# NicolaDM/MAPLE

Measured on AMD Instinct MI355X. Metric: candidate SPR placements/sec, higher is better.
Workload: dtype f64

## Files before the change

### __graft_entry__.py

```python
import os
import subprocess
import sys

ROOT = os.path.dirname(os.path.abspath(__file__))
if ROOT not in sys.path:
    sys.path.insert(0, ROOT)

CSRC = os.path.join(ROOT, "maple_amd", "csrc")
HIP_UNITS = ["maple_hip.hip", "append_queries.hip", "placement.hip", "update.hip", "spr_batch.hip", "frontier.hip", "frontier_upd.hip",
             "frontier_updw128.hip", "witness.hip", "em.hip"]
DEBUG_UNIT = "debug_abi.hip"
HIP_LIB = os.path.join(ROOT, "maple_amd", "libmaple_hip.so")
HIP_LIB_DEBUG = os.path.join(ROOT, "maple_amd", "libmaple_hip_debug.so")
HIP_FLAGS = ["--offload-arch=gfx950", "-O3", "-std=c++17", "-ffp-contract=off", "-fPIC"]
HIPCC = "hipcc" if subprocess.call(["which", "hipcc"], stdout=subprocess.DEVNULL) == 0 else "/opt/rocm/bin/hipcc"


def _stale(target, sources):
    if not os.path.exists(target):
        return True
    t = os.path.getmtime(target)
    return any(os.path.getmtime(s) > t for s in sources)


def compile_units(out_dir, extra_flags=(), only=None, force=True):
    sources = [os.path.join(CSRC, f) for f in os.listdir(CSRC) if not f.endswith((".o", ".c"))]
    sources.append(os.path.join(ROOT, "include", "maple_hip.h"))
    sources.append(os.path.join(ROOT, "include", "maple_hip_debug.h"))
    objs, jobs = [], []
    for unit in HIP_UNITS + [DEBUG_UNIT]:
        mine = only is None or unit in only
        obj = os.path.join(out_dir if mine else CSRC, unit[:-4] + ".o")
        objs.append(obj)
        deps = [x for x in sources if not (x.endswith(".hip") and os.path.basename(x) != unit)]
        if mine and (force or _stale(obj, deps)):
            jobs.append((unit, subprocess.Popen([HIPCC] + HIP_FLAGS + list(extra_flags) + ["-c", os.path.join(CSRC, unit), "-o", obj])))
    for unit, job in jobs:
        if job.wait() != 0:
            raise RuntimeError(f"hipcc failed on {unit}")
    return objs


def link(lib, objs):
    subprocess.check_call([HIPCC, "--offload-arch=gfx950", "-shared", "-fPIC"] + objs + ["-o", lib])


def build(force=False):
    extra = os.environ.get("MAPLE_HIP_EXTRA_FLAGS", "").split()
    objs = compile_units(CSRC, extra, force=force)
    for lib, parts in ((HIP_LIB, objs[:-1]), (HIP_LIB_DEBUG, objs)):
        if force or _stale(lib, parts):
            link(lib, parts)
    synth_src, synth_lib = os.path.join(CSRC, "synth_gen.c"), os.path.join(ROOT, "maple_amd", "libmaple_synth.so")
    if force or _stale(synth_lib, [synth_src]):
        subprocess.check_call(["gcc", "-O2", "-shared", "-fPIC", "-o", synth_lib, synth_src, "-lm"])
    subprocess.check_call(["make", "-C", os.path.join(ROOT, "oracle"), "-s"])
    import maple_amd
    from maple_amd import runtime
    runtime.load_library()


def smoke():
    import math
    import numpy as np
    from maple_amd.runtime import Device
    from maple_amd.synth import make_dataset
    from maple_amd.host import tip_genome_list, reference_tables
    from oracle.oracle_py import Oracle

    d = make_dataset(n_samples=64, l_ref=3000, seed=5, mean_diffs=12.0, frac_with_n=0.3, frac_ambig=0.3,
                     n_run_len=(5, 80))
    ref_idx, root_freqs = reference_tables(d.ref)
    lists = [tip_genome_list(x, ref_idx) for x in d.diffs]
    Q = [[-0.9, 0.2, 0.5, 0.2], [0.3, -1.4, 0.1, 1.0], [0.8, 0.1, -1.3, 0.4], [0.1, 0.6, 0.1, -0.8]]
    dev = Device(ref_idx, root_freqs, arena_bytes=64 << 20)
    orc = Oracle(ref_idx, root_freqs)
    dev.set_model(Q)
    orc.set_model(Q)
    ids = dev.upload(lists)
    n = len(lists)
    a = np.arange(n, dtype=np.int32)
    b = (a * 7 + 3) % n
    merged = dev.merge_batch(ids[a], 1e-4, True, ids[b], 2e-4, True, False)
    got_lists = dev.download(merged)
    ok_ids = [m for m in merged if m >= 0]
    scores = dev.append_batch(ok_ids, ids[: len(ok_ids)], True, 1.0 / dev.lRef)
    k = 0
    for i in range(n):
        want = orc.mergeVectors(lists[a[i]], 1e-4, True, lists[b[i]], 2e-4, True)
        if want is None:
            assert got_lists[i] is None
            continue
        assert len(want) == len(got_lists[i]) and all(x[0] == y[0] and x[1] == y[1] for x, y in zip(want, got_lists[i]))
        ws = orc.appendProbNode(want, lists[k], True, 1.0 / dev.lRef)
        gs = float(scores[k])
        assert (math.isinf(ws) and math.isinf(gs)) or abs(ws - gs) <= 1e-9 * max(1.0, abs(ws)), (ws, gs)
        k += 1
    import torch
    cu = torch.device("cuda", 0)
    t_q = torch.from_numpy(ids[:8].astype(np.int32)).to(cu)
    t_c = torch.from_numpy(np.asarray(ok_ids, dtype=np.int32)).to(cu)
    out = torch.empty(8 * len(ok_ids), dtype=torch.float64, device=cu)
    torch.cuda.synchronize()
    dev.append_queries_dev(8, t_q.data_ptr(), len(ok_ids), t_c.data_ptr(), True, 1.0 / dev.lRef, out.data_ptr(),
                           torch.cuda.current_stream().cuda_stream)
    torch.cuda.synchronize()
    got = out.cpu().numpy().reshape(8, len(ok_ids))
    ok_lists = [g for g in got_lists if g is not None]
    for qi in range(8):
        for ci in range(0, len(ok_ids), 5):
            ws = orc.appendProbNode(ok_lists[ci], lists[qi], True, 1.0 / dev.lRef)
            gs = float(got[qi, ci])
            assert (math.isinf(ws) and math.isinf(gs)) or abs(ws - gs) <= 1e-9 * max(1.0, abs(ws)), (qi, ci, ws, gs)
    dev.close()
    print(f"smoke ok: {n} merges, {k} + {8 * len(range(0, len(ok_ids), 5))} placements scored on the GPU and matched "
          "against the oracle")


if __name__ == "__main__":
    build()
    if len(sys.argv) > 1 and sys.argv[1] == "smoke":
        smoke()
```

### include/maple_hip_debug.h

```cpp
#ifndef MAPLE_HIP_DEBUG_H
#define MAPLE_HIP_DEBUG_H
#include "maple_hip.h"

#ifdef __cplusplus
extern "C" {
#endif

int maple_debug_frontier_levels(maple_ctx *ctx, int32_t cap, int64_t *itemsUpdating, int64_t *itemsCached, float *msUpdating,
                                float *msCached, int32_t *n, int64_t *waveItemsSmall , int64_t *waveItemsBig );

int maple_debug_wave_append_batch(maple_ctx *ctx, int32_t n, const int32_t *parentList, const int32_t *childList,
                                  const uint8_t *isTipC, const double *bLen, double *outLK, float *ms);
int maple_debug_trace_query(maple_ctx *ctx, int32_t query);
int maple_debug_calib_walk(maple_ctx *ctx, uint64_t bytes, int32_t repeats, float *ms);
int maple_debug_calib_write(maple_ctx *ctx, uint64_t bytes, int32_t mode, int32_t repeats, float *ms);
int maple_debug_trace_read(maple_ctx *ctx, int32_t *n, int32_t *items4 , double *vals2 );
int maple_debug_live_resources(int64_t *allocs, int64_t *bytes, int64_t *handles);
int maple_debug_gpv_batch(maple_ctx *ctx, int32_t n, const int32_t *i12, const double *totLen, const double *M16,
                          const double *errorRate, const double *vect4, const uint8_t *upNode, const uint8_t *flag,
                          double *out4);
int maple_debug_simplify_batch(maple_ctx *ctx, int32_t n, const double *vec4, const int32_t *refA, int32_t *out);
int maple_debug_frontier_pass_batch(maple_ctx *ctx, int32_t n, const int32_t *list, const int32_t *mutList, const uint8_t *dirIsUp,
                                    int32_t waveForm, int32_t *outList, uint8_t *grade, uint8_t *sameHandle);
int maple_debug_score_rows(maple_ctx *ctx, int32_t form, int32_t nQ, const int32_t *qList, const uint8_t *qTip, const double *qBLen,
                           int32_t nC, const int32_t *cand, const int32_t *outCol , int64_t ldOut, double fill, double *out,
                           uint64_t *finMask, int32_t *prefix, int64_t *pairsWalked );

#ifdef __cplusplus
}
#endif
#endif
```

### maple_amd/csrc/debug_abi.hip

```cpp
#include "../../include/maple_hip_debug.h"
#include "genome_dev.h"
#include "ctx_host.h"
#include "batch_host.h"
#include "frontier.h"
#include "frontier_dev.h"
#include "witness.h"

#include <algorithm>

using namespace frt;

__global__ __launch_bounds__(MAPLE_BLOCK) void k_calib_walk(const unsigned long long *buf, long long nLists, unsigned long long *sink)
{
    unsigned long long acc = 0;
    for (long long l = (long long)blockIdx.x * blockDim.x + threadIdx.x; l < nLists; l += (long long)gridDim.x * blockDim.x) {
        const unsigned long long *p = buf + l * 64;
        unsigned idx = 0;
        for (int k = 0; k < 64; k++) {
            unsigned long long w = p[idx];
            acc += w;
            idx = (idx + 1 + (unsigned)(w & 0)) & 63;
        }
    }
    if (acc == 0x123456789abcdefull) *sink = acc;
// ... 21 lines not shown
        hipLaunchKernelGGL(k_calib_write, dim3(4096), dim3(MAPLE_BLOCK), 0, c->stream, buf.p, (long long)(bytes / 8), mode == 1 ? 1 : 8);
    HIPCK(c, hipEventRecord(e1, c->stream));
    HIPCK(c, hipEventSynchronize(e1));
    if (ms) HIPCK(c, hipEventElapsedTime(ms, e0, e1));
    return MAPLE_OK;
}

extern "C" int maple_debug_calib_walk(maple_ctx *c, uint64_t bytes, int32_t repeats, float *ms)
{
    if (!c || bytes < 512 || repeats <= 0) return MAPLE_ERR_ARG;
    HIPCK(c, hipSetDevice(c->device));
    DevBuf<unsigned long long> buf, sink;
    HIPCK(c, buf.reserve_exact((size_t)((bytes + 7) / 8)));
    HIPCK(c, sink.reserve_exact(1));
    HIPCK(c, hipMemset(buf, 1, bytes));
    HIPCK(c, hipDeviceSynchronize());
    Event e0, e1;
    HIPCK(c, e0.create());
    HIPCK(c, e1.create());
    HIPCK(c, hipEventRecord(e0, c->stream));
    for (int r = 0; r < repeats; r++)
        hipLaunchKernelGGL(k_calib_walk, dim3(2048), dim3(MAPLE_BLOCK), 0, c->stream, buf.p, (long long)(bytes / 512), sink.p);
    HIPCK(c, hipEventRecord(e1, c->stream));
    HIPCK(c, hipEventSynchronize(e1));
    if (ms) HIPCK(c, hipEventElapsedTime(ms, e0, e1));
    return MAPLE_OK;
}

struct MatCtx {
    const double *M;
    __device__ inline double q(double, int i, int j) const { return M[i * 4 + j]; }
};
struct ThrCtx { struct { double thresholdProb, thresholdProb4; } m; };

__global__ __launch_bounds__(MAPLE_BLOCK) void k_debug_gpv(int n, int usingErrorRate, const int32_t *i12, const double *totLen,
                                                           const double *M16, const double *errorRate, const double *vect,
                                                           const uint8_t *upNode, const uint8_t *flag, double *out)
{
    for (int i = blockIdx.x * blockDim.x + threadIdx.x; i < n; i += gridDim.x * blockDim.x) {
        MatCtx c{M16 + 16 * (size_t)i};
        double o[4];
        if (i12[i] == 6) gpv_vec(c, 1.0, vect + 4 * (size_t)i, totLen[i], upNode[i] != 0, o);
        else if (usingErrorRate) gpv_nuc<MatCtx, true>(c, 1.0, i12[i], totLen[i], errorRate[i], upNode[i] != 0, flag[i] != 0, o);
        else gpv_nuc<MatCtx, false>(c, 1.0, i12[i], totLen[i], errorRate[i], upNode[i] != 0, false, o);
        for (int k = 0; k < 4; k++) out[4 * (size_t)i + k] = o[k];
    }
}

__global__ __launch_bounds__(MAPLE_BLOCK) void k_debug_simplify(int n, double thresholdProb, double thresholdProb4, const double *vec,
                                                                const int32_t *refA, int32_t *out)
{
    for (int i = blockIdx.x * blockDim.x + threadIdx.x; i < n; i += gridDim.x * blockDim.x) {
        ThrCtx c;
        c.m.thresholdProb = thresholdProb; c.m.thresholdProb4 = thresholdProb4;
        out[i] = simplify(c, vec + 4 * (size_t)i, refA[i]);
    }
}

extern "C" int maple_debug_gpv_batch(maple_ctx *c, int32_t n, const int32_t *i12, const double *totLen, const double *M16,
                                     const double *errorRate, const double *vect4, const uint8_t *upNode, const uint8_t *flag,
                                     double *out4)
{
    if (!c || n < 0 || !i12 || !totLen || !M16 || !errorRate || !vect4 || !upNode || !flag || !out4) return MAPLE_ERR_ARG;
    if (n == 0) return MAPLE_OK;
    HIPCK(c, hipSetDevice(c->device));
    TRY(need_model(c));
    TRY(h2d(c, c->s_i32[0], i12, (size_t)n));
    TRY(h2d(c, c->s_f64[0], totLen, (size_t)n));
    TRY(h2d(c, c->s_f64[1], M16, (size_t)16 * n));
    TRY(h2d(c, c->s_f64[2], errorRate, (size_t)n));
    TRY(h2d(c, c->s_f64[3], vect4, (size_t)4 * n));
    TRY(h2d(c, c->s_u8[0], upNode, (size_t)n));
    TRY(h2d(c, c->s_u8[1], flag, (size_t)n));
    HIPCK(c, c->s_aux.reserve((size_t)4 * n));
    hipLaunchKernelGGL(k_debug_gpv, dim3(grid_for(n)), dim3(MAPLE_BLOCK), 0, c->stream, n, c->dm.usingErrorRate, c->s_i32[0].p,
                       c->s_f64[0].p, c->s_f64[1].p, c->s_f64[2].p, c->s_f64[3].p, c->s_u8[0].p, c->s_u8[1].p, c->s_aux.p);
    HIPCK(c, hipGetLastError());
    HIPCK(c, hipMemcpyAsync(out4, c->s_aux.p, (size_t)4 * n * sizeof(double), hipMemcpyDeviceToHost, c->stream));
    HIPCK(c, hipStreamSynchronize(c->stream));
    return MAPLE_OK;
}

extern "C" int maple_debug_simplify_batch(maple_ctx *c, int32_t n, const double *vec4, const int32_t *refA, int32_t *out)
{
    if (!c || n < 0 || !vec4 || !refA || !out) return MAPLE_ERR_ARG;
    if (n == 0) return MAPLE_OK;
    HIPCK(c, hipSetDevice(c->device));
    TRY(h2d(c, c->s_f64[0], vec4, (size_t)4 * n));
    TRY(h2d(c, c->s_i32[0], refA, (size_t)n));
    HIPCK(c, c->s_i32[1].reserve(n));
    hipLaunchKernelGGL(k_debug_simplify, dim3(grid_for(n)), dim3(MAPLE_BLOCK), 0, c->stream, n, c->dm.thresholdProb,
                       c->dm.thresholdProb4, c->s_f64[0].p, c->s_i32[0].p, c->s_i32[1].p);
    HIPCK(c, hipGetLastError());
    HIPCK(c, hipMemcpyAsync(out, c->s_i32[1].p, n * sizeof(int32_t), hipMemcpyDeviceToHost, c->stream));
    HIPCK(c, hipStreamSynchronize(c->stream));
    return MAPLE_OK;
}

extern "C" int maple_debug_wave_append_batch(maple_ctx *c, int32_t n, const int32_t *pl, const int32_t *cl, const uint8_t *tip,
                                             const double *bl, double *out, float *ms)
{
    if (!c || n < 0 || !pl || !cl || !tip || !bl || !out) return MAPLE_ERR_ARG;
    if (n == 0) return MAPLE_OK;
    HIPCK(c, hipSetDevice(c->device));
    TRY(need_model(c));
    TRY(check_ids(c, n, pl, false, "parentList"));
    TRY(check_ids(c, n, cl, false, "childList"));
    TRY(stage_begin(c, (size_t)n * 32 + 256));
    STAGE(dpl, c, pl, n); STAGE(dcl, c, cl, n); STAGE(dtip, c, tip, n); STAGE(dbl, c, bl, n);
    TRY(stage_flush(c));
    HIPCK(c, c->s_f64[1].reserve(n));
    hipEvent_t e0, e1;
    TRY(ev_pair(c, &e0, &e1, MAPLE_K_OTHER, (double)n, 0.0));
    HIPCK(c, hipEventRecord(e0, c->stream));
    launch_wave_append(c, std::min(n, 256 * 16), n, dpl, dcl, dtip, dbl, c->s_f64[1].p);
    HIPCK(c, hipGetLastError());
    HIPCK(c, hipEventRecord(e1, c->stream));
    HIPCK(c, hipMemcpyAsync(out, c->s_f64[1].p, n * sizeof(double), hipMemcpyDeviceToHost, c->stream));
    HIPCK(c, hipStreamSynchronize(c->stream));
    if (ms) HIPCK(c, hipEventElapsedTime(ms, e0, e1));
    return MAPLE_OK;
}

extern "C" int maple_debug_live_resources(int64_t *allocs, int64_t *bytes, int64_t *handles)
{
    if (!allocs || !bytes || !handles) return MAPLE_ERR_ARG;
    const DevBufStats &s = devbuf_stats();
    *allocs = s.live_allocs; *bytes = s.live_bytes; *handles = s.live_handles;
    return MAPLE_OK;
}

extern "C" int maple_debug_trace_query(maple_ctx *c, int32_t query)
{
    if (!c) return MAPLE_ERR_ARG;
    c->trace_query = query;
    if (query >= 0) {
        HIPCK(c, c->s_trace_i.reserve(4 * 4096 + 4));
        HIPCK(c, c->s_trace_d.reserve(2 * 4096));
        HIPCK(c, hipMemset(c->s_trace_i.p, 0, (4 * 4096 + 4) * sizeof(int32_t)));
    }
    return MAPLE_OK;
}

extern "C" int maple_debug_trace_read(maple_ctx *c, int32_t *n, int32_t *items4, double *vals2)
{
    if (!c || !n || !items4 || !vals2 || !c->s_trace_i.p) return MAPLE_ERR_ARG;
    HIPCK(c, hipMemcpy(n, c->s_trace_i.p + 4 * 4096, sizeof(int32_t), hipMemcpyDeviceToHost));
    HIPCK(c, hipMemcpy(items4, c->s_trace_i.p, 4 * 4096 * sizeof(int32_t), hipMemcpyDeviceToHost));
    HIPCK(c, hipMemcpy(vals2, c->s_trace_d.p, 2 * 4096 * sizeof(double), hipMemcpyDeviceToHost));
    return MAPLE_OK;
}

extern "C" int maple_debug_frontier_levels(maple_ctx *c, int32_t cap, int64_t *itemsUpdating, int64_t *itemsCached, float *msUpdating,
                                           float *msCached, int32_t *n, int64_t *waveItemsSmall, int64_t *waveItemsBig)
{
    if (!c || cap < 0 || !itemsUpdating || !itemsCached || !msUpdating || !msCached || !n) return MAPLE_ERR_ARG;
    HIPCK(c, hipSetDevice(c->device));
    int nn = 0;
    const int rc = frontier_level_profile(c, cap, (long long *)itemsUpdating, (long long *)itemsCached, msUpdating, msCached, &nn,
                                          (long long *)waveItemsSmall, (long long *)waveItemsBig);
    *n = nn;
    return rc;
}

template <bool RV, bool U, bool SS>
__global__ __launch_bounds__(FR_BLOCK) void k_debug_fpass_lane(const DevModel *__restrict__ mp, ArenaViewS av, FPools fp, int n, const int32_t *l,
                                                               const int32_t *ml, const uint8_t *up, int32_t *handle)
{
    __shared__ Lds lds;
    const DevModel &m = *mp;
    stage_model(m, lds);
    Ctx<RV, U, SS> c(m, lds);
    const long long laneId = (long long)blockIdx.x * blockDim.x + threadIdx.x;
    for (long long i = laneId; i < n; i += (long long)gridDim.x * blockDim.x)
        handle[i] = fpass_removed(c, fp, av, laneId, ftree(l[i]), ml[i], up[i] != 0);
}

template <bool RV, bool U, bool SS>
__global__ __launch_bounds__(FR_BLOCK) void k_debug_fpass_wave(const DevModel *__restrict__ mp, ArenaViewS av, FPools fp, int n, const int32_t *l,
                                                               const int32_t *ml, const uint8_t *up, int32_t *handle)
{
    __shared__ Lds lds;
    const DevModel &m = *mp;
    stage_model(m, lds);
    Ctx<RV, U, SS> c(m, lds);
    const long long wave = ((long long)blockIdx.x * blockDim.x + threadIdx.x) >> 6, nWaves = ((long long)gridDim.x * blockDim.x) >> 6;
    const int lane = threadIdx.x & 63;
    for (long long i = wave; i < n; i += nWaves) {
        const int h = wave_pass(c, fp, av, ftree(l[i]), ml[i], up[i] != 0, true);
        if (lane == 0) handle[i] = h;
    }
}

__global__ __launch_bounds__(FR_BLOCK) void k_debug_fpass_out(FPools fp, int n, const int32_t *handle, int64_t *woff, int64_t *aoff, int32_t *nEnt,
                                                              int32_t *nAux, uint8_t *grade)
{
    for (int i = blockIdx.x * blockDim.x + threadIdx.x; i < n; i += gridDim.x * blockDim.x) {
        const int h = handle[i];
        if (h >= 0 && h < fp.capL) {
            const LRec r = fp.trec[h];
            woff[i] = LREC_OFF(r.x); aoff[i] = LREC_OFF(r.y); nEnt[i] = LREC_N(r.x); nAux[i] = LREC_N(r.y); grade[i] = fp.tflag[h];
        } else { woff[i] = 0; aoff[i] = 0; nEnt[i] = -1; nAux[i] = 0; grade[i] = 0; }
    }
}

extern "C" int maple_debug_frontier_pass_batch(maple_ctx *c, int32_t n, const int32_t *list, const int32_t *mutList, const uint8_t *dirIsUp,
                                               int32_t waveForm, int32_t *outList, uint8_t *grade, uint8_t *sameHandle)
{
    if (!c || n < 0 || n > (1 << 20) || !list || !mutList || !dirIsUp || !outList || !grade || !sameHandle) return MAPLE_ERR_ARG;
    if (n == 0) return MAPLE_OK;
    HIPCK(c, hipSetDevice(c->device));
    TRY(need_model(c));
    TRY(check_ids(c, n, list, false, "list"));
    TRY(settle(c));
    const int32_t nml = (int32_t)c->h_mut_cnt.size();
    long long capW = 0, capA = 0;
    int capE = 1;
    for (int i = 0; i < n; i++) {
        if (mutList[i] < -1 || mutList[i] >= nml) return fail(c, MAPLE_ERR_ARG, "mutList[%d] = %d is not a mutation-list id", i, mutList[i]);
        const long long cnt = mutList[i] < 0 ? 0 : c->h_mut_cnt[mutList[i]];
        const long long ne = c->h_n_ent[list[i]] + 2 * cnt, na = c->h_n_aux[list[i]] + 4 * cnt;
        capW += ne; capA += na;
        capE = std::max(capE, (int)ne);
    }
    const int threads = waveForm ? 64 * std::min(n, 1024) : std::min(1024, (n + FR_BLOCK - 1) / FR_BLOCK * FR_BLOCK);
    const int grid = (threads + FR_BLOCK - 1) / FR_BLOCK;
    const long long lanes = (long long)grid * FR_BLOCK;
    HIPCK(c, c->s_words.reserve((size_t)capW));
    HIPCK(c, c->s_aux.reserve((size_t)capA));
    auto up16 = [](size_t x) { return (x + 255) & ~(size_t)255; };
    const size_t oRec = 0, oCtr = up16(oRec + (size_t)n * sizeof(LRec)), oSw = up16(oCtr + sizeof(FCtr)),
                 oSa = up16(oSw + (waveForm ? 0 : (size_t)lanes * capE * sizeof(uint2))),
                 oWoff = up16(oSa + (waveForm ? 0 : (size_t)lanes * 5 * capE * sizeof(double))), oAoff = up16(oWoff + (size_t)n * 8),
                 oHandle = up16(oAoff + (size_t)n * 8), oNe = up16(oHandle + (size_t)n * 4), oNa = up16(oNe + (size_t)n * 4),
                 oFlag = up16(oNa + (size_t)n * 4), oGrade = up16(oFlag + (size_t)n), total = up16(oGrade + (size_t)n);
    DevBuf<uint8_t> own;
    HIPCK(c, own.reserve_exact(total));
    uint8_t *const buf = own.p;
    int rc = MAPLE_OK;
    std::vector<int32_t> handle(n);
    do {
        if (hipMemsetAsync(buf, 0, oSw, c->stream) != hipSuccess) { rc = fail(c, MAPLE_ERR_HIP, "hipMemsetAsync"); break; }
        FPools fp;
        memset(&fp, 0, sizeof fp);
        fp.tw = c->s_words.p; fp.ta = c->s_aux.p;
        fp.trec = (LRec *)(buf + oRec); fp.tflag = buf + oFlag;
        fp.capW = capW; fp.capA = capA; fp.capL = n;
        fp.sw = (uint2 *)(buf + oSw); fp.sa = (double *)(buf + oSa); fp.capE = capE;
        fp.ctr = (FCtr *)(buf + oCtr);
        fp.mat = 1;
        fp.mv = MutViewS{c->d_mut3, c->d_mut_off, c->d_mut_cnt};
        const ArenaViewS av{c->d_words, c->d_aux, c->d_ent_off, c->d_aux_off, c->d_n_ent, c->d_n_aux};
        if ((rc = stage_begin(c, (size_t)n * 64 + 256)) != MAPLE_OK) break;
        auto *dl = stage_put(c, list, (size_t)n);
        auto *dml = stage_put(c, mutList, (size_t)n);
        auto *dup = stage_put(c, dirIsUp, (size_t)n);
        if (!dl || !dml || !dup) { rc = fail(c, MAPLE_ERR_NOMEM, "argument staging overflow"); break; }
        if ((rc = stage_flush(c)) != MAPLE_OK) break;
        int32_t *dHandle = (int32_t *)(buf + oHandle), *dNe = (int32_t *)(buf + oNe), *dNa = (int32_t *)(buf + oNa);
        int64_t *dWoff = (int64_t *)(buf + oWoff), *dAoff = (int64_t *)(buf + oAoff);
        if (waveForm) DISPATCH3(c, k_debug_fpass_wave, <<<grid, FR_BLOCK, 0, c->stream>>>(c->d_model, av, fp, n, dl, dml, dup, dHandle));
        else DISPATCH3(c, k_debug_fpass_lane, <<<grid, FR_BLOCK, 0, c->stream>>>(c->d_model, av, fp, n, dl, dml, dup, dHandle));
        hipLaunchKernelGGL(k_debug_fpass_out, dim3(grid_for(n)), dim3(FR_BLOCK), 0, c->stream, fp, n, dHandle, dWoff, dAoff, dNe, dNa, buf + oGrade);
        if (hipGetLastError() != hipSuccess || hipMemcpyAsync(handle.data(), dHandle, (size_t)n * 4, hipMemcpyDeviceToHost, c->stream) != hipSuccess
            || hipMemcpyAsync(grade, buf + oGrade, (size_t)n, hipMemcpyDeviceToHost, c->stream) != hipSuccess
            || hipStreamSynchronize(c->stream) != hipSuccess) { rc = fail(c, MAPLE_ERR_HIP, "the frontier pass hook's launch failed"); break; }
        for (int i = 0; i < n && rc == MAPLE_OK; i++) {
            sameHandle[i] = handle[i] == -(list[i] + 10);
            if (!sameHandle[i] && handle[i] < 0) rc = fail(c, MAPLE_ERR_NOMEM, "item %d: no room for the new list (%d)", i, handle[i]);
        }
        if (rc != MAPLE_OK) break;
        if ((rc = commit_lists(c, n, dWoff, dAoff, dNe, dNa, outList, fp.tw, fp.ta)) != MAPLE_OK) break;
        if (hipStreamSynchronize(c->stream) != hipSuccess) { rc = fail(c, MAPLE_ERR_HIP, "hipStreamSynchronize"); break; }
        for (int i = 0; i < n; i++) if (sameHandle[i]) outList[i] = list[i];
    } while (0);
    return rc;
}

__global__ __launch_bounds__(MAPLE_BLOCK) void k_debug_fill(long long n, double v, double *out)
{
    for (long long i = (long long)blockIdx.x * blockDim.x + threadIdx.x; i < n; i += (long long)gridDim.x * blockDim.x) out[i] = v;
}

extern "C" int maple_debug_score_rows(maple_ctx *c, int32_t form, int32_t nQ, const int32_t *qList, const uint8_t *qTip, const double *qBLen,
                                      int32_t nC, const int32_t *cand, const int32_t *outCol, int64_t ldOut, double fill, double *out,
                                      uint64_t *finMask, int32_t *prefix, int64_t *pairsWalked)
{
    if (!c || form < 0 || form > 1 || nQ <= 0 || nC <= 0 || !qList || !qTip || !qBLen || !cand || ldOut < nC || !out || !finMask || !prefix)
        return MAPLE_ERR_ARG;
    if ((long long)nQ * ldOut > (1ll << 28)) return fail(c, MAPLE_ERR_ARG, "maple_debug_score_rows: a table of %lld scores", (long long)nQ * ldOut);
    HIPCK(c, hipSetDevice(c->device));
    TRY(need_model(c));
    TRY(check_ids(c, nQ, qList, false, "qList"));
    TRY(check_ids(c, nC, cand, true, "cand"));
    for (int k = 0; k < nC; k++) {
        if (cand[k] < -1) return fail(c, MAPLE_ERR_ARG, "cand[%d] = %d", k, cand[k]);
        if (outCol && (outCol[k] < 0 || outCol[k] >= ldOut)) return fail(c, MAPLE_ERR_ARG, "outCol[%d] = %d is outside a row of %lld", k, outCol[k], (long long)ldOut);
    }
    TRY(settle(c));
    const int nWords = (nC + 63) / 64;
    const size_t nOut = (size_t)nQ * (size_t)ldOut, nMask = (size_t)nQ * nWords, nPre = (size_t)nQ * (nWords + 1);
    DevBuf<double> dOut;
    DevBuf<unsigned long long> dMask;
    DevBuf<int32_t> dPre;
    HIPCK(c, dOut.reserve_exact(nOut));
    HIPCK(c, dMask.reserve_exact(nMask));
    HIPCK(c, dPre.reserve_exact(nPre));
    TRY(stage_begin(c, (size_t)nQ * 16 + (size_t)nC * 8 + 256));
    STAGE(dq, c, qList, nQ); STAGE(dtip, c, qTip, nQ); STAGE(dbl, c, qBLen, nQ); STAGE(dcand, c, cand, nC);
    const int32_t *dcol = nullptr;
    if (outCol) { STAGE(dc, c, outCol, nC); dcol = dc; }
    TRY(stage_flush(c));
    hipLaunchKernelGGL(k_debug_fill, dim3(grid_for((int)nOut)), dim3(MAPLE_BLOCK), 0, c->stream, (long long)nOut, fill, dOut.p);
    HIPCK(c, hipGetLastError());
    HIPCK(c, hipMemsetAsync(dMask.p, 0xA5, nMask * sizeof(unsigned long long), c->stream));
// ... 16 lines not shown
```

### maple_amd/csrc/fr_wave_items_body.inc

```
    __shared__ Lds lds;
    __shared__ WaveUpdLds<Class::wuIn> L;
    typedef WaveLds<Class::capW> WaveLdsC;
    const DevModel &m = *mp;
    stage_model(m, lds);
    Ctx<RV, U, SS> c(m, lds);
    const int lane = threadIdx.x;
    WaveLdsC &W = *reinterpret_cast<WaveLdsC *>(L.baux);
    static_assert(sizeof(WaveLdsC) <= sizeof(L.baux), "LDS alias");
    const long long lo = (long long)fp.ctr->loU;
    const long long nHeavy = (long long)(fp.ctr->*Class::count);
    (void)heavyMin;
    unsigned long long nU = 0, bU = 0;
    for (long long kk = blockIdx.x; kk < nHeavy; kk += gridDim.x) {
        nU++;
#ifdef MAPLE_SPR_PROFILE
        const long long tItem0 = wall_clock64();
        int profCls = Class::profCls;
        struct ProfEnd {
            const FPools &fp; const long long t0; int &cls;
            __device__ ~ProfEnd() {
                if ((threadIdx.x & 63) == 0) {
                    const unsigned long long dt = (unsigned long long)(wall_clock64() - t0);
                    atomicAdd(&fp.ctr->dbgWCnt[cls], 1ull); atomicAdd(&fp.ctr->dbgWT[cls], dt); atomicMax(&fp.ctr->dbgWMax[cls], dt);
                }
            }
        } profEnd{fp, tItem0, profCls};
#endif
        {
            const long long i = lo + (fp.*Class::perm)[kk];
            FItem &it = fp.U[i];
            FSearch &S = fp.S[it.q];
            if (!fs_live(S.state)) { if (lane == 0) it.flags |= FI_DEAD; continue; }
            const int q = it.q, t1 = it.t1, dir = it.dir;
            const NodeRec r1 = T.nd[t1];
            const int hPassed = it.hPassed, hRpr = it.hRpr;
            const double distance = it.distance, lastLK = it.lastLK;
            const bool rt = S.isRemovedTip != 0;
            const double rbl = S.removedBLen;
            const int other = dir == 0 ? -1 : (dir == 1 ? r1.c1 : r1.c0);
            const int upT = r1.up;
            const FList lp = fvalid(hPassed) ? flist(av, fp, hPassed) : FList{nullptr, nullptr, 0, 0};
            const FList lr = flist(av, fp, hRpr);
            const bool fits = fr_wave_fits(av, T, fp, it, Class::wuIn, Class::capW);
            if (!fits) {
#ifdef MAPLE_SPR_PROFILE
                profCls += 2;
#endif
                if (lane == 0) fr_upd_item_lane_call(c, av, T, P, fp, budget, laneBase + blockIdx.x, i, &bU);
                wave_sync();
                continue;
            }
            bool upd = true;
            double midProb = lastLK;
            int flagsAdd = 0;
            int nM = 0, naM = 0;
            auto merge = [&](const FList &l1, double b1, bool tp1, const FList &l2, double b2, bool tp2, bool upDown) -> int {
                if (l1.n > L.wuIn || l2.n > L.wuIn) return -2;
                wave_sync();
                const int r = wave_merge(c, fref(l1), l1.n, b1, tp1, fref(l2), l2.n, b2, tp2, upDown, L, naM);
                bU += 8ull * (unsigned long long)(l1.n + l1.na + l2.n + l2.na + (r > 0 ? r + naM : 0));
                if (r < 0) return r == -1 ? -1 : -2;
                nM = r;
                return 0;
            };
            auto differs = [&](int listId) -> bool {
                const FList tu = flist(av, fp, ftree(listId));
                const unsigned long long *tw = (const unsigned long long *)tu.w;
                for (int k = lane; k < tu.n; k += 64) L.old[k] = tw[k];
                wave_sync();
                return wave_differ(c, L.m, L.maux, nM, L.old, tu.aux, tu.n);
            };
            auto score = [&]() -> double {
                wave_sync();
                return wave_append(c, ListRef{(const uint2 *)L.m, L.maux}, nM, fref(lr), lr.n, rt, rbl, W);
            };
            auto push1 = [&](bool u, int node, int d, int h, double dst, double mp, int fails, double pb, int hr, bool needPass) -> int {
                int ref = FR_NONE;
                if (lane == 0) ref = fpush(fp, budget, q, u, node, d, h, dst, mp, fails, hr, pb, needPass);
                return __shfl(ref, 0, 64);
            };
            const bool matAdj = fp.mat && (r1.c0Frame != r1.frameOf || r1.c1Frame != r1.frameOf || r1.upFrame != r1.frameOf);
            auto passW = [&](int h, int mutId, bool up, bool removed) -> int {
                if (!matAdj) return h;
                return wave_pass(c, fp, av, h, mutId, up, removed);
            };
            bool dead = false, fallback = false;
            int child0 = FR_NONE, child1 = FR_NONE, hA = -1, hB = -1, hMid = -1;
            double recDist = 0.0;
            if (dir == 0) {
                const bool scored = !(upT == S.parent || upT < 0) && (r1.dist > P.effNon0 || r1.upIsRoot);
                if (scored) {
                    const FList ll = flist(av, fp, ftree(r1.lower));
                    if (merge(lp, distance / 2, false, ll, distance / 2, r1.isTip != 0, true) != 0) dead = true;
                    else {
                        if (r1.totUp >= 0 && !differs(r1.totUp)) upd = false;
                        midProb = score();
                        flagsAdd |= FI_SCORED;
                        if (upd && midProb >= it.pathBest - P.thrOptTopo) {
                            wave_sync();
                            hMid = fstore_wave(fp, L.m, L.maux, nM, naM);
                            if (hMid < 0) { fallback = true; dead = true; }
                            else { hA = hPassed; hB = ftree(r1.lower); recDist = distance; flagsAdd |= FI_REC_UPD; }
                        }
                    }
                }
                if (!dead) {
                    const PRule pr = p_rule(P, scored, midProb, lastLK, it.failsP, it.pathBest);
                    if (pr.go && r1.c0 >= 0) {
                        for (int k = 0; k < 2 && !fallback; k++) {
                            const int ch = k == 0 ? r1.c0 : r1.c1, oth = k == 0 ? r1.c1 : r1.c0;
                            int ref = FR_NONE;
                            const bool cross = matAdj && (k == 0 ? r1.c0Frame : r1.c1Frame) != r1.frameOf;
                            if (upd) {
                                const NodeRec ro = T.nd[oth];
                                const int hOther = passW(ftree(ro.lower), ro.mutId, true, false);
                                const FList lo2 = fvalid(hOther) ? flist(av, fp, hOther) : FList{nullptr, nullptr, 0, 0};
                                const int r = fvalid(hOther) ? merge(lp, distance, false, lo2, ro.dist, ro.isTip != 0, true) : -2;
                                if (r == -2) { fallback = true; break; }
                                if (r == 0) {
                                    wave_sync();
                                    int hv = fstore_wave(fp, L.m, L.maux, nM, naM), hr = hRpr;
                                    if (hv >= 0 && cross) {
                                        const int mId = T.nd[ch].mutId;
                                        hv = passW(hv, mId, false, false); hr = passW(hRpr, mId, false, true);
                                    }
                                    if (hv < 0 || !fvalid(hr)) { fallback = true; break; }
                                    ref = push1(true, ch, 0, hv, T.nd[ch].dist, midProb, pr.fails, pr.pathBest, hr, false);
                                }
                            } else if ((k == 0 ? r1.upRight : r1.upLeft) >= 0)
                                ref = push1(false, ch, 0, -1, 0.0, midProb, pr.fails, pr.pathBest, hRpr, cross);
                            if (k == 0) child0 = ref; else child1 = ref;
                        }
                    }
                }
            } else {
                const NodeRec ro = T.nd[other];
                const int vectUp = upT >= 0 ? passW(ftree(r1.whichChild ? T.nd[upT].upLeft : T.nd[upT].upRight), r1.mutId, false, false) : -1;
                const int hOther = passW(ftree(ro.lower), ro.mutId, true, false);
                const bool crossO = matAdj && ((dir == 1) ? r1.c1Frame : r1.c0Frame) != r1.frameOf, crossU = matAdj && r1.upFrame != r1.frameOf;
                const bool scored = upT >= 0 && (r1.dist > P.effNon0 || r1.upIsRoot);
                int hBottom = -1;
                if (vectUp == -2 || hOther == -2 || !fvalid(hOther)) {
                    if (lane == 0) { S.state = FS_FALLBACK; it.flags |= FI_DEAD; }
                    wave_sync();
                    continue;
                }
                const FList lo2 = flist(av, fp, hOther);
                const FList lvu = fvalid(vectUp) ? flist(av, fp, vectUp) : FList{nullptr, nullptr, 0, 0};
                if (scored) {
                    if (!fvalid(vectUp) || r1.totUp < 0) {
                        if (lane == 0) fr_upd_item_lane_call(c, av, T, P, fp, budget, laneBase + blockIdx.x, i, &bU);
                        wave_sync();
                        continue;
                    }
                    int r = merge(lp, distance, false, lo2, ro.dist, ro.isTip != 0, false);
                    if (r == -2) { fallback = true; dead = true; }
                    else if (r != 0) dead = true;
                    else {
                        wave_sync();
                        hBottom = fstore_wave(fp, L.m, L.maux, nM, naM);
                        if (hBottom < 0) { fallback = true; dead = true; }
                        else {
                            const FList lb = flist(av, fp, hBottom);
                            r = merge(lvu, r1.dist / 2, false, lb, r1.dist / 2, false, true);
                            if (r == -2) { fallback = true; dead = true; }
                            else if (r != 0) dead = true;
                            else {
                                if (!differs(r1.totUp)) upd = false;
                                midProb = score();
                                flagsAdd |= FI_SCORED;
                                if (upd && midProb >= it.pathBest - P.thrOptTopo) {
                                    wave_sync();
                                    hMid = fstore_wave(fp, L.m, L.maux, nM, naM);
                                    if (hMid < 0) { fallback = true; dead = true; }
                                    else { hA = vectUp; hB = hBottom; recDist = r1.dist; flagsAdd |= FI_REC_UPD; }
                                }
                            }
                        }
                    }
                }
                if (!dead) {
                    const PRule pr = p_rule(P, scored, midProb, lastLK, it.failsP, it.pathBest);
                    if (pr.go) {
                        if (upT >= 0) {
                            int hUp = -1;
                            bool stop = false;
                            if (upd) {
                                const int r = fvalid(vectUp) ? merge(lvu, r1.dist, false, lp, distance, false, true) : -2;
                                if (r == -2) { fallback = true; stop = true; }
                                else if (r == 0) { wave_sync(); hUp = fstore_wave(fp, L.m, L.maux, nM, naM); if (hUp < 0) { fallback = true; stop = true; } }
                            } else hUp = ftree(dir == 1 ? r1.upLeft : r1.upRight);
                            int hrO = hRpr, hrU = hRpr;
                            if (upd && crossO && !stop && hUp >= 0) {
                                hUp = passW(hUp, ro.mutId, false, false); hrO = passW(hRpr, ro.mutId, false, true);
                                if (hUp == -2 || !fvalid(hrO)) { fallback = true; stop = true; }
                            }
                            if (!stop && fvalid(hUp)) {
                                child0 = upd ? push1(true, other, 0, hUp, ro.dist, midProb, pr.fails, pr.pathBest, hrO, false)
                                             : push1(false, other, 0, -1, 0.0, midProb, pr.fails, pr.pathBest, hRpr, crossO);
// ... 32 lines not shown
```

### maple_amd/csrc/frontier.h

```cpp
#pragma once
#include "ctx_host.h"

#define FR_STATUS_FALLBACK (-8)

struct FrontierStats {
    int levels = 0, overflow = 0;
    long long itemsUpdating = 0, itemsCached = 0, tempLists = 0, tempWords = 0, tempAux = 0, records = 0;
};

struct FrontierWide {
    const int32_t *rowOf;
    const double *cacheS;
    FiniteRows fin;
    hipEvent_t rowsReady;
    int forceWide;
    const int32_t *frameParent = nullptr, *frameNode = nullptr;
    int nFrames = 0;
};

__attribute__((visibility("hidden")))
int frontier_search(maple_ctx *c, const SearchParams &P, int m, const int32_t *nodes, int budget, int zeroBudget, SearchOut *hostOut,
                    uint2 *poolW, double *poolA, unsigned long long *poolUsed, long long poolCapW, long long poolCapA,
                    FrontierStats *stats, long long itemsHint, const FrontierWide *wide = nullptr,
                    const uint8_t *overHint = nullptr);
__attribute__((visibility("hidden"))) int frontier_export(maple_ctx *c, long long cap, int32_t *q, int32_t *node, long long *n);
__attribute__((visibility("hidden")))
int frontier_level_profile(maple_ctx *c, int cap, long long *itemsU, long long *itemsC, float *msU, float *msC, int *n,
                           long long *waveSmall = nullptr, long long *waveBig = nullptr);
```

### maple_amd/csrc/frontier.hip

```cpp
#include "ctx_host.h"
#include "frontier_dev.h"
#include "search_plan.h"

#include <chrono>

using namespace frt;
namespace plan = maple::plan;

namespace {

__global__ __launch_bounds__(FR_BLOCK) void k_fr_arena_recs(ArenaViewS av, int n, LRec *out)
{
    for (int i = blockIdx.x * blockDim.x + threadIdx.x; i < n; i += gridDim.x * blockDim.x)
        out[i] = lrec_make(av.ent_off[i], av.n_ent[i], av.aux_off[i], av.n_aux[i]);
}

template <bool RV, bool U, bool SS>
__global__ __launch_bounds__(FR_BLOCK) void k_fr_begin(const DevModel *__restrict__ mp, ArenaViewS av, DevTree T, SearchParams P, int n,
                                                       const int32_t *nodes, FPools fp, SearchOut *out, int budget, int zeroBudget,
                                                       const int32_t *rowOf, int forceWide, const uint8_t *overHint)
{
    __shared__ Lds lds;
    const DevModel &m = *mp;
    stage_model(m, lds);
    Ctx<RV, U, SS> c(m, lds);
    for (int q = blockIdx.x * blockDim.x + threadIdx.x; q < n; q += gridDim.x * blockDim.x) {
        const int node = nodes[q];
        SearchOut &o = out[q];
        o.bestNode = -1; o.placement = -1; o.status = 0; o.nAppend = 0;
        o.bestScore = 0.0; o.improvement = 0.0; o.currentLK = 0.0;
        o.blen[0] = o.blen[1] = o.blen[2] = 0.0;
        o.rprWoff = o.rprAoff = -1; o.rprN = o.rprNA = 0;
        o.nShortList = o.nSteps = 0; o.tStep = o.tReplay = o.tRefine = 0;
        FSearch &S = fp.S[q];
        S.node = node; S.parent = -1; S.sibling = -1; S.hRpr0 = -1; S.seed0 = S.seed1 = FR_NONE; S.nItems = 0; S.state = FS_FINAL;
        S.slHead = FR_NONE; S.nApp = 0; S.recBase = 0; S.recCount = 0; S.isRemovedTip = 0; S.removedBLen = 0.0; S.curLK = 0.0;
        const NodeRec rn = T.nd[node];
        const int parent = rn.up;
        if (parent < 0) { o.status = 1; continue; }
        const NodeRec rp = T.nd[parent];
        const int childIdx = (rp.c0 == node) ? 0 : 1;
        const int vectUp = ftree(childIdx == 0 ? rp.upRight : rp.upLeft);
        if (!fvalid(vectUp) || rn.lower < 0) { o.status = -1; continue; }
        const FList lu = flist(av, fp, vectUp), ll = flist(av, fp, ftree(rn.lower));
        const long long laneId = (long long)blockIdx.x * blockDim.x + threadIdx.x;
        double curLK;
        if (fp.mat && rn.mutId >= 0 && fp.mv.cnt[rn.mutId] > 0) {
            const int cnt = fp.mv.cnt[rn.mutId];
            FScr scr{nullptr, nullptr};
            if (!fscratch(fp, laneId, lu.n + 2 * cnt, scr)) { S.state = FS_FALLBACK; continue; }
            Writer wr;
            wr.init(scr.w, scr.a);
            pass_walk(c.m.lRef, fref(lu), fp.mv.mut3 + 3 * fp.mv.off[rn.mutId], cnt, false, wr);
            curLK = append_walk(c, ListRef{scr.w, scr.a}, fref(ll), rn.isTip != 0, rn.dist);
        } else
        curLK = append_walk(c, fref(lu), fref(ll), rn.isTip != 0, rn.dist);
        o.currentLK = curLK;
        if (!(curLK < P.thrPlacement || rn.dist != 0.0)) { o.status = 2; continue; }
        if (overHint && overHint[q]) { S.state = FS_OVER; o.status = -5; continue; }
        S.parent = parent; S.sibling = childIdx == 0 ? rp.c1 : rp.c0;
        S.isRemovedTip = rn.isTip; S.removedBLen = rn.dist; S.curLK = curLK;
        const NodeRec rs = T.nd[S.sibling];
        int rpr = ftree(rn.lower);
        const int mergeLevel = shorten_would_merge(c, fref(ll), ll.n);
        const bool wouldMerge = mergeLevel != 0;
        S.rprMerge0 = mergeLevel;
        int hBest = rpr;
        if (fp.mat) {
            rpr = fpass_removed(c, fp, av, laneId, rpr, rn.mutId, true);
            hBest = fvalid(rpr) ? fpass_removed(c, fp, av, laneId, rpr, rs.mutId, false) : rpr;
            if (!fvalid(rpr) || !fvalid(hBest)) { S.state = FS_FALLBACK; continue; }
        }
        S.hRpr0 = hBest;
        bool wide = false;
        if (forceWide && rowOf && rowOf[q] >= 0) {
            if (wouldMerge) { S.state = FS_OVER; o.status = -5; o.nAppend = -1; continue; }
            wide = true;
        } else if (!U && budget > zeroBudget && rn.dist == 0.0) {
            wide = rowOf && rowOf[q] >= 0 && !wouldMerge;
            if (!wide) { S.state = FS_OVER; o.status = -5; o.nAppend = -1; continue; }
        } else if (U && rowOf && rowOf[q] >= 0) {
            if (wouldMerge) { S.state = FS_OVER; o.status = -5; o.nAppend = -1; continue; }
            wide = true;
        }
        S.state = wide ? FS_WIDE : FS_ACTIVE;
        if (rp.up < 0) {
            S.seed0 = fpush(fp, budget, q, true, S.sibling, 3, -1, 0.0, curLK, 0, S.hRpr0, curLK);
            continue;
        }
        const int pp = rp.up;
        const NodeRec rpp = T.nd[pp];
        const bool first = rpp.c0 == parent;
        const double d = rs.dist + rp.dist;
        int pv1 = ftree(rs.lower), rprUp = rpr, vUpUp = ftree(first ? rpp.upRight : rpp.upLeft), rprDown = rpr;
        if (fp.mat) {
            pv1 = fpass_store(fp, av, c.m.lRef, laneId, pv1, rs.mutId, true);
            if (rp.mutId >= 0) {
                pv1 = fvalid(pv1) ? fpass_store(fp, av, c.m.lRef, laneId, pv1, rp.mutId, true) : pv1;
                rprUp = fpass_removed(c, fp, av, laneId, rpr, rp.mutId, true);
            }
            vUpUp = fpass_store(fp, av, c.m.lRef, laneId, vUpUp, rp.mutId, false);
            if (rs.mutId >= 0) {
                vUpUp = fvalid(vUpUp) ? fpass_store(fp, av, c.m.lRef, laneId, vUpUp, rs.mutId, false) : vUpUp;
                rprDown = hBest;
            }
            if (pv1 == -2 || vUpUp == -2 || !fvalid(rprUp) || !fvalid(rprDown)) { S.state = FS_FALLBACK; continue; }
        }
        S.seed0 = fpush(fp, budget, q, true, pp, first ? 1 : 2, pv1, d, curLK, 0, rprUp, curLK);
        S.seed1 = fpush(fp, budget, q, true, S.sibling, 0, vUpUp, d, curLK, 0, rprDown, curLK);
    }
}

#define FR_LVL 8
__global__ void k_fr_snap_u(FCtr *ctr, long long capU, long long capR, long long capPassR, unsigned long long *lvl, int maxLevels)
{
    if (threadIdx.x == 0 && blockIdx.x == 0) {
        ctr->loU = ctr->hiU; ctr->hiU = min(ctr->usedU, (unsigned long long)capU);
        atomicExch(&ctr->safePassR, min(ctr->nPassR, (unsigned long long)capPassR));
        __threadfence();
        atomicExch(&ctr->safeR, min(ctr->usedR, (unsigned long long)capR));
        ctr->bigUsed = 0;
        const unsigned long long heavySmall = ctr->permHeavy, heavyBig = ctr->permHeavy2;
        ctr->permDown = ctr->permUp = ctr->permDownB = ctr->permUpB = ctr->permHeavy = ctr->permHeavy2 = 0;
        if (lvl) {
            const int l = ctr->nLevels++;
            if (l < maxLevels) { lvl[FR_LVL * l] = ctr->loU; lvl[FR_LVL * l + 1] = ctr->hiU; lvl[FR_LVL * l + 6] = lvl[FR_LVL * l + 7] = 0; }
            if (l > 0 && l - 1 < maxLevels) { lvl[FR_LVL * (l - 1) + 6] = heavySmall; lvl[FR_LVL * (l - 1) + 7] = heavyBig; }
        }
    }
}
__global__ void k_fr_snap_c(FCtr *ctr, long long capCC, long long capPass, long long capDeferred, unsigned long long *lvl, int maxLevels)
{
    if (threadIdx.x == 0 && blockIdx.x == 0) {
        ctr->loC = ctr->hiC; ctr->hiC = min(ctr->usedC, (unsigned long long)capCC);
        ctr->loR = ctr->hiR; ctr->hiR = atomicAdd(&ctr->safeR, 0ull);
        __threadfence();
        ctr->loP = ctr->hiP; ctr->hiP = min(ctr->nPass, (unsigned long long)capPass);
        ctr->loPR = ctr->hiPR; ctr->hiPR = atomicAdd(&ctr->safePassR, 0ull);
        ctr->bigUsedC = 0;
        ctr->loD = ctr->hiD; ctr->hiD = min(ctr->nDeferred, (unsigned long long)capDeferred);
        if (lvl) {
            const int k = ctr->nLevelsC++;
            if (k < maxLevels) {
                lvl[FR_LVL * k + 2] = ctr->loC; lvl[FR_LVL * k + 3] = ctr->hiC;
                lvl[FR_LVL * k + 4] = (unsigned long long)capCC + ctr->loR; lvl[FR_LVL * k + 5] = (unsigned long long)capCC + ctr->hiR;
            }
        }
    }
}

#define FR_PASS_WAVE_BELOW 8192
template <bool RV, bool U, bool SS>
__global__ __launch_bounds__(FR_BLOCK) void k_fr_pass_wave(const DevModel *__restrict__ mp, ArenaViewS av, DevTree T, FPools fp)
{
    __shared__ Lds lds;
    const DevModel &m = *mp;
    stage_model(m, lds);
    Ctx<RV, U, SS> c(m, lds);
    const long long wave = ((long long)blockIdx.x * blockDim.x + threadIdx.x) >> 6, nWaves = ((long long)gridDim.x * blockDim.x) >> 6;
    const int lane = threadIdx.x & 63;
    const long long loA = (long long)fp.ctr->loP, nA = (long long)fp.ctr->hiP - loA, loB = (long long)fp.ctr->loPR, nB = (long long)fp.ctr->hiPR - loB;
    if (nA + nB > FR_PASS_WAVE_BELOW) return;
    for (long long i = wave; i < nA + nB; i += nWaves) {
        FItem &it = item_of(fp, i < nA ? fp.passList[loA + i] : fp.passListR[loB + (i - nA)]);
        FSearch &S = fp.S[it.q];
        if (!fs_live(S.state)) continue;
        const NodeRec r1 = T.nd[it.t1];
        const int mutId = it.dir == 0 ? r1.mutId : T.nd[it.dir == 1 ? r1.c0 : r1.c1].mutId;
        const int h = wave_pass(c, fp, av, it.hRpr, mutId, it.dir != 0, true);
        if (lane == 0) {
            if (!fvalid(h)) S.state = FS_FALLBACK;
            else {
                it.hRpr = h;
                const unsigned long long k = atomicAdd(&fp.ctr->nDeferred, 1ull);
                if ((long long)k < fp.capDeferred) fp.deferred[k] = (int32_t)(&it - fp.C);
                else { S.state = FS_FALLBACK; fp.ctr->overflow = 1; }
            }
        }
    }
}

template <bool RV, bool U, bool SS>
__global__ __launch_bounds__(FR_BLOCK) void k_fr_pass(const DevModel *__restrict__ mp, ArenaViewS av, DevTree T, FPools fp, long long slabBase)
{
    __shared__ Lds lds;
    const DevModel &m = *mp;
    stage_model(m, lds);
    Ctx<RV, U, SS> c(m, lds);
    const long long laneId = (long long)blockIdx.x * blockDim.x + threadIdx.x;
    const long long slab = slabBase + laneId;
    const long long loA = (long long)fp.ctr->loP, nA = (long long)fp.ctr->hiP - loA, loB = (long long)fp.ctr->loPR, nB = (long long)fp.ctr->hiPR - loB;
    if (nA + nB <= FR_PASS_WAVE_BELOW) return;
    for (long long i = laneId; i < nA + nB; i += (long long)gridDim.x * blockDim.x) {
        FItem &it = item_of(fp, i < nA ? fp.passList[loA + i] : fp.passListR[loB + (i - nA)]);
        FSearch &S = fp.S[it.q];
        if (!fs_live(S.state)) continue;
        const NodeRec r1 = T.nd[it.t1];
        const int mutId = it.dir == 0 ? r1.mutId : T.nd[it.dir == 1 ? r1.c0 : r1.c1].mutId;
        const int h = fpass_removed(c, fp, av, slab, it.hRpr, mutId, it.dir != 0);
        if (!fvalid(h)) { S.state = FS_FALLBACK; continue; }
        it.hRpr = h;
        const unsigned long long k = atomicAdd(&fp.ctr->nDeferred, 1ull);
        if ((long long)k < fp.capDeferred) fp.deferred[k] = (int32_t)(&it - fp.C);
        else { S.state = FS_FALLBACK; fp.ctr->overflow = 1; }
    }
}

__global__ __launch_bounds__(FR_BLOCK) void k_fr_sort_level(ArenaViewS av, DevTree T, FPools fp, int heavyMin, int bigMin)
{
    const long long lo = (long long)fp.ctr->loU, hi = (long long)fp.ctr->hiU;
    const long long n = hi - lo;
    const int lane = threadIdx.x & 63;
    heavyMin = fr_level_heavy_min(fp, heavyMin);
    auto bc = [](unsigned long long x) {
        return ((unsigned long long)(uint32_t)__shfl((int)(x >> 32), 0, 64) << 32) | (uint32_t)__shfl((int)x, 0, 64);
    };
    for (long long base = (long long)blockIdx.x * blockDim.x; base < n; base += (long long)gridDim.x * blockDim.x) {
        const long long i = base + threadIdx.x;
        int kind = -1;
        bool small = false;
        if (i < n) {
            const FItem &it = fp.U[lo + i];
            const int sz = fr_upd_size(av, T, fp, it);
            if (!(heavyMin > 0 && it.dir != 3 && sz >= heavyMin)) kind = (it.dir == 0 ? 0 : 1) + (sz >= bigMin ? 2 : 0);
            else {
                small = fr_wave_fits(av, T, fp, it, WaveSmall::wuIn, WaveSmall::capW);
                if (!small && !fr_wave_fits(av, T, fp, it, WaveBig::wuIn, WaveBig::capW)) kind = (it.dir == 0 ? 2 : 3);
            }
        }
        const unsigned long long below = (1ull << lane) - 1ull;
        {
            const bool hv = i < n && kind == -1;
            for (int cls = 0; cls < 2; cls++) {
                const bool mine = hv && (small == (cls == 0));
                const unsigned long long mh = __ballot(mine);
                if (!mh) continue;
                unsigned long long b0 = 0;
                if (lane == 0) b0 = atomicAdd(cls == 0 ? &fp.ctr->permHeavy : &fp.ctr->permHeavy2, (unsigned long long)__popcll(mh));
                b0 = bc(b0);
                if (mine) (cls == 0 ? fp.perm3 : fp.perm4)[(long long)(b0 + __popcll(mh & below))] = (int32_t)i;
            }
        }
        for (int k = 0; k < 4; k++) {
            const unsigned long long mk = __ballot(kind == k);
            if (!mk) continue;
            unsigned long long *ctr = k == 0 ? &fp.ctr->permDown : (k == 1 ? &fp.ctr->permUp : (k == 2 ? &fp.ctr->permDownB : &fp.ctr->permUpB));
            unsigned long long b0 = 0;
            if (lane == 0) b0 = atomicAdd(ctr, (unsigned long long)__popcll(mk));
            b0 = bc(b0);
            if (kind == k) {
                int32_t *pm = k < 2 ? fp.perm : fp.perm2;
                const long long at = (long long)(b0 + __popcll(mk & below));
                pm[(k & 1) ? n - 1 - at : at] = (int32_t)i;
            }
        }
    }
}

#ifndef FR_CACHED_WAVES
#define FR_CACHED_WAVES 4
#endif
template <bool RV, bool U, bool SS>
__global__ __launch_bounds__(FR_BLOCK) __attribute__((amdgpu_waves_per_eu(FR_CACHED_WAVES, FR_CACHED_WAVES)))
void k_fr_cached(const DevModel *__restrict__ mp, ArenaViewS av, DevTree T, SearchParams P, FPools fp, int budget,
                 const int32_t *rowOf, FiniteRows fin)
{
    __shared__ Lds lds;
    const DevModel &m = *mp;
    stage_model(m, lds);
    Ctx<RV, U, SS> c(m, lds);
    const int lane = threadIdx.x & 63;
    const long long loC = (long long)fp.ctr->loC, nC = (long long)fp.ctr->hiC - loC, loR = fp.capCC + (long long)fp.ctr->loR,
                    nCR = nC + (long long)fp.ctr->hiR - (long long)fp.ctr->loR, loD = (long long)fp.ctr->loD,
                    hi = nCR + (long long)fp.ctr->hiD - loD;
    unsigned long long nSc = 0, bSc = 0;
    for (long long i0 = (long long)blockIdx.x * blockDim.x; i0 < hi; i0 += (long long)gridDim.x * blockDim.x) {
        const long long i = i0 + threadIdx.x;
#ifdef MAPLE_SPR_PROFILE
        const long long tp0 = wall_clock64();
#endif
        int mode = 0;
        FItem *itp = nullptr;
        const FSearch *Sp = nullptr;
        NodeRec r1{};
        FList lp{nullptr, nullptr, 0, 0}, lr{nullptr, nullptr, 0, 0};
        bool rt = false;
        double rbl = 0.0;
        if (i < hi) {
            FItem &it = fp.C[i < nC ? loC + i : (i < nCR ? loR + (i - nC) : (long long)fp.deferred[loD + (i - nCR)])];
            FSearch &S = fp.S[it.q];
            itp = &it; Sp = &S;
            const int st = S.state;
            if (i < nCR && (it.flags & FI_NEEDPASS)) { }
            else if (!fs_live(st)) it.flags |= FI_DEAD;
            else if (st == FS_WIDE && it.dir == 0) {
                int fl = FI_SEED;
                if (fin.mask && rowOf) {
                    const NodeRec r1s = T.nd[it.t1];
                    const SScan rec = T.scan[r1s.preRank];
                    const size_t row = (size_t)rowOf[it.q];
                    const unsigned long long *fm = fin.mask + row * fin.nWords;
                    const int32_t *fpx = fin.prefix + row * (fin.nWords + 1);
                    const int clo = T.candBefore[r1s.preRank], chi = T.candBefore[r1s.preRank + rec.size];
                    if (fin_count_before(fm, fpx, chi) == fin_count_before(fm, fpx, clo)) {
                        const bool firstScored = !(r1s.up == S.parent || r1s.up < 0) && (r1s.dist > P.effNon0 || r1s.upIsRoot);
                        const bool dropped = firstScored && !(rec.ff & SS_TOTUP);
                        fl |= FI_SEED_EMPTY;
                        it.hA = (firstScored && !dropped) ? 1 : 0;
                        it.hB = T.cladeVisits[r1s.preRank];
                        it.hMid = ((rec.ff & SS_INNER) && !dropped) ? 1 : 0;
                    }
                }
                it.flags |= (uint8_t)fl;
            } else {
                r1 = T.nd[it.t1];
                const int upT = r1.up;
                const bool scored = (it.dir == 0) ? (!(upT == S.parent || upT < 0) && (r1.dist > P.effNon0 || r1.upIsRoot))
                                                  : (upT >= 0 && (r1.dist > P.effNon0 || r1.upIsRoot));
                mode = 1;
                if (scored) {
                    if (r1.totUp < 0) { it.flags |= FI_DEAD; mode = 0; }
                    else {
                        lp = flist(av, fp, ftree(r1.totUp)); lr = flist(av, fp, it.hRpr);
                        rt = S.isRemovedTip != 0; rbl = S.removedBLen;
                        mode = 2;
                    }
                }
            }
        }
#ifdef MAPLE_SPR_PROFILE
        __builtin_amdgcn_s_waitcnt(0);
        const long long tp1 = wall_clock64();
#endif
        double scoreV = 0.0;
        if (mode == 2) scoreV = append_walk(c, fref(lp), fref(lr), rt, rbl);
        const int nS = __popcll(__ballot(mode == 2));
        (void)nS;
#ifdef MAPLE_SPR_PROFILE
        const long long tp2 = wall_clock64();
#endif
        if (mode != 0) {
            FItem &it = *itp;
            const FSearch &S = *Sp;
            const int q = it.q, hRpr = it.hRpr, upT = r1.up;
            const double lastLK = it.lastLK;
            double midProb = lastLK;
            const bool scored = mode == 2;
            if (scored) {
                midProb = scoreV;
                it.flags |= FI_SCORED;
                nSc++; bSc += 8ull * (unsigned long long)(lp.n + lp.na) + 8ull;
            }
            it.midProb = midProb;
            const PRule pr = p_rule(P, scored, midProb, lastLK, it.failsP, it.pathBest);
            if (pr.go) {
                const bool x0 = fp.mat && r1.c0Frame != r1.frameOf, x1 = fp.mat && r1.c1Frame != r1.frameOf, xu = fp.mat && r1.upFrame != r1.frameOf;
                if (it.dir == 0) {
                    if (r1.c0 >= 0) {
                        if (r1.upRight >= 0) it.child0 = fpush(fp, budget, q, false, r1.c0, 0, -1, 0.0, midProb, pr.fails, hRpr, pr.pathBest, x0, true);
                        if (r1.upLeft >= 0) it.child1 = fpush(fp, budget, q, false, r1.c1, 0, -1, 0.0, midProb, pr.fails, hRpr, pr.pathBest, x1, true);
                    }
                } else {
                    const int other = (it.dir == 1) ? r1.c1 : r1.c0;
                    const bool xo = (it.dir == 1) ? x1 : x0;
                    if (upT >= 0) {
                        if (((it.dir == 1) ? r1.upLeft : r1.upRight) >= 0) {
                            it.child0 = fpush(fp, budget, q, false, other, 0, -1, 0.0, midProb, pr.fails, hRpr, pr.pathBest, xo, true);
                            it.child1 = fpush(fp, budget, q, false, upT, (int)r1.whichChild + 1, -1, 0.0, midProb, pr.fails, hRpr, pr.pathBest, xu, true);
                        }
                    } else
                        it.child0 = fpush(fp, budget, q, false, other, 0, -1, 0.0, midProb, pr.fails, hRpr, pr.pathBest, xo, true);
                }
            }
            (void)S;
        }
#ifdef MAPLE_SPR_PROFILE
        {
            __builtin_amdgcn_s_waitcnt(0);
            const long long tp3 = wall_clock64();
            int len = mode == 2 ? lp.n + lr.n : 0, tot = len;
            for (int off = 32; off > 0; off >>= 1) { len = max(len, __shfl_down(len, off, 64)); tot += __shfl_down(tot, off, 64); }
            if (lane == 0) {
                atomicAdd(&fp.ctr->dbgC[0], 1ull); atomicAdd(&fp.ctr->dbgC[1], (unsigned long long)(tp1 - tp0));
                atomicAdd(&fp.ctr->dbgC[2], (unsigned long long)(tp2 - tp1)); atomicAdd(&fp.ctr->dbgC[3], (unsigned long long)(tp3 - tp2));
                atomicAdd(&fp.ctr->dbgC[4], (unsigned long long)len); atomicAdd(&fp.ctr->dbgC[5], (unsigned long long)nS);
                atomicAdd(&fp.ctr->dbgC[6], (unsigned long long)tot);
            }
        }
#endif
    }
    for (int off = 32; off > 0; off >>= 1) {
        nSc += ((unsigned long long)(uint32_t)__shfl_down((int)(nSc >> 32), off, 64) << 32) | (uint32_t)__shfl_down((int)nSc, off, 64);
        bSc += ((unsigned long long)(uint32_t)__shfl_down((int)(bSc >> 32), off, 64) << 32) | (uint32_t)__shfl_down((int)bSc, off, 64);
// ... 416 lines not shown
    }
}

template <bool RV, bool U, bool SS>
__global__ __launch_bounds__(FR_BLOCK) __attribute__((amdgpu_waves_per_eu(4, 4)))
void k_fr_refine(const DevModel *__restrict__ mp, ArenaViewS av, DevTree T, FPools fp)
{
    __shared__ Lds lds;
    const DevModel &m = *mp;
    stage_model(m, lds);
    Ctx<RV, U, SS> c(m, lds);
    const long long laneId = (long long)blockIdx.x * blockDim.x + threadIdx.x;
    double *ais = fp.sais + laneId * 2ll * fp.capE;
    const long long nRecs = min((long long)fp.ctr->nRecs, fp.capRecs);
    for (long long i = laneId; i < nRecs; i += (long long)gridDim.x * blockDim.x) {
        FRec &R = fp.recs[i];
        const FItem &it = item_of(fp, R.ref);
        FSearch &S = fp.S[R.q];
        R.ok = 0;
        if (!fs_live(S.state)) continue;
        const int t1 = it.t1;
        const NodeRec r1 = T.nd[t1];
        int hUp, hDown, hMid;
        double distance;
        if (it.flags & FI_REC_UPD) { hUp = it.hA; hDown = it.hB; hMid = it.hMid; distance = it.recDist; }
        else {
            hUp = r1.up >= 0 ? ftree(r1.whichChild ? T.nd[r1.up].upLeft : T.nd[r1.up].upRight) : -1;
            if (fp.mat && fvalid(hUp)) {
                hUp = fpass_store(fp, av, c.m.lRef, laneId, hUp, r1.mutId, false);
                if (hUp == -2) { S.state = FS_FALLBACK; continue; }
            }
            hDown = ftree(r1.lower); hMid = ftree(r1.totUp); distance = r1.dist;
        }
        if (!fvalid(hUp) || !fvalid(hDown) || !fvalid(hMid)) { R.ok = -1; continue; }
        int hRem = it.hRpr;
        if (R.hRprS == FR_SHORTEN) {
            const FList l0 = flist(av, fp, hRem);
            FScr scrS;
            if (!fscratch(fp, laneId, l0.n, scrS)) { S.state = FS_FALLBACK; continue; }
            Writer ws;
            ws.init(scrS.w, scrS.a);
            shorten_walk(c, fref(l0), l0.n, ws);
            hRem = fstore(fp, ws);
            if (hRem < 0) { S.state = FS_FALLBACK; continue; }
            R.hRprS = hRem;
        }
        const FList lUp = flist(av, fp, hUp), lDown = flist(av, fp, hDown), lMid = flist(av, fp, hMid), lRem = flist(av, fp, hRem);
        const bool ft = r1.isTip != 0, rt = S.isRemovedTip != 0;
        const int need = max(lDown.n + lRem.n, max(lUp.n + lRem.n, lUp.n + lDown.n));
        FScr scr0;
        if (lMid.n + lRem.n > 2 * fp.capE || lUp.n + need > 2 * fp.capE || !fscratch(fp, laneId, need, scr0)) { S.state = FS_FALLBACK; continue; }
        uint2 *sw = scr0.w;
        double *sa = scr0.a;
        bool f;
        Writer w;
        const double app = blen_walk(c, fref(lMid), fref(lRem), rt, ais, 1, &f);
        w.init(sw, sa);
        int r = merge_walk(c, fref(lDown), distance / 2, ft, fref(lRem), app, rt, false, false, 0, 0, w, nullptr);
        if (r < 0) { R.ok = -1; continue; }
        const ListRef scr{sw, sa};
        double top = blen_walk(c, fref(lUp), scr, false, ais, 1, &f);
        w.init(sw, sa);
        r = merge_walk(c, fref(lUp), top, false, fref(lRem), app, rt, true, false, 0, 0, w, nullptr);
        if (r == -1) {
            top = m.defaultBLen * 0.1;
            w.init(sw, sa);
            r = merge_walk(c, fref(lUp), top, false, fref(lRem), app, rt, true, false, 0, 0, w, nullptr);
        }
        if (r < 0) { R.ok = -1; continue; }
        const double bottom = blen_walk(c, scr, fref(lDown), ft, ais, 1, &f);
        w.init(sw, sa);
        r = merge_walk(c, fref(lUp), top, false, fref(lDown), bottom, ft, true, false, 0, 0, w, nullptr);
        if (r < 0) { R.ok = -1; continue; }
        const double cost = append_walk(c, scr, fref(lRem), rt, app);
        const double initialCost = append_walk(c, fref(lUp), fref(lDown), ft, distance);
        const double newPartialCost = append_walk(c, fref(lUp), fref(lDown), ft, bottom + top);
        R.optimized = cost + newPartialCost - initialCost;
        R.top = top; R.bottom = bottom; R.app = app;
        R.ok = 1;
    }
}

__global__ __launch_bounds__(FR_BLOCK) void k_fr_finish(ArenaViewS av, DevTree T, SearchParams P, int n, FPools fp, SearchOut *out,
                                                        uint2 *poolW, double *poolA, unsigned long long *poolUsed, long long poolCapW,
                                                        long long poolCapA)
{
    for (int q = blockIdx.x * blockDim.x + threadIdx.x; q < n; q += gridDim.x * blockDim.x) {
        FSearch &S = fp.S[q];
        SearchOut &o = out[q];
        if (S.state == FS_FALLBACK) { o.status = FR_STATUS_FALLBACK; continue; }
        if (!fs_live(S.state)) continue;
        const int node = S.node;
        const NodeRec rp = T.nd[S.parent];
        double bestScore = S.curLK;
        int bestNode = S.sibling, hBestRpr = S.hRpr0, nApp = S.nApp;
        double bl0 = rp.up >= 0 ? rp.dist : 0.0, bl1 = T.nd[S.sibling].dist, bl2 = S.removedBLen;
        bool failed = false;
        for (int k = 0; k < S.recCount; k++) {
            const FRec &R = fp.recs[S.recBase + k];
            if (R.ok != 1) { failed = true; break; }
            nApp += 3;
            if (R.optimized >= bestScore) {
                const FItem &it = item_of(fp, R.ref);
                bestNode = it.t1; bestScore = R.optimized; bl0 = R.top; bl1 = R.bottom; bl2 = R.app; hBestRpr = R.hRprS >= 0 ? R.hRprS : it.hRpr;
            }
        }
        o.nAppend = nApp;
        o.nShortList = S.recCount;
        if (failed) { o.status = -1; continue; }
        o.bestNode = bestNode; o.bestScore = bestScore;
        o.blen[0] = bl0; o.blen[1] = bl1; o.blen[2] = bl2;
        if (poolW) {
            const FList rp2 = flist(av, fp, hBestRpr);
            const long long ow = (long long)atomicAdd(&poolUsed[0], (unsigned long long)rp2.n);
            const long long oa = (long long)atomicAdd(&poolUsed[1], (unsigned long long)rp2.na);
            if (ow + rp2.n <= poolCapW && oa + rp2.na <= poolCapA) {
                for (int k = 0; k < rp2.n; k++) poolW[ow + k] = rp2.w[k];
                for (int k = 0; k < rp2.na; k++) poolA[oa + k] = rp2.aux[k];
                o.rprWoff = ow; o.rprAoff = oa; o.rprN = rp2.n; o.rprNA = rp2.na;
            } else o.status = -4;
        }
        const double curLK = S.curLK;
        if (bestScore + P.thrPlacement > curLK) {
            bool updated = true;
            int topNode = T.nd[node].up;
            if (bestNode == topNode) updated = false;
            while (T.nd[topNode].dist == 0.0 && T.nd[topNode].up >= 0) topNode = T.nd[topNode].up;
            if (bestNode == topNode && bl1 == 0.0) updated = false;
            if (bestNode == S.sibling) updated = false;
            if (T.nd[bestNode].up == S.sibling && bl0 == 0.0) updated = false;
            if (updated) { o.improvement = bestScore - curLK; o.placement = bestNode; }
        }
    }
}

__global__ __launch_bounds__(FR_BLOCK) void k_fr_export(FPools fp, long long nU, long long nC, long long nR, int32_t *outQ, int32_t *outNode)
{
    const long long n = nU + nC + nR;
    for (long long i = (long long)blockIdx.x * blockDim.x + threadIdx.x; i < n; i += (long long)gridDim.x * blockDim.x) {
        const FItem &it = i < nU ? fp.U[i] : (i < nU + nC ? fp.C[i - nU] : fp.C[fp.capCC + (i - nU - nC)]);
        outQ[i] = it.q; outNode[i] = it.t1;
    }
}

struct FrontierScratch : ScratchBase {
    Stream side, side2;
    Event evFork, evJoin, evFork2, evJoin2;
    DevBuf<uint8_t> itemsU, itemsC, srch, recs, ctr;
    DevBuf<uint2> tw, sw, bw;
    DevBuf<double> ta, sa, sais, ba;
    DevBuf<LRec> trec, arec;
    DevBuf<int32_t> nodes, expQ, expNode;
    DevBuf<uint8_t> out, wideBr, tflag, overHint;
    DevBuf<int32_t> wideRow, wideQ, wideCtr, perm, perm2, perm3, perm4, tot, lsize, lpos, lpar, passList, passListR, deferred;
    DevBuf<uint2> bw2; DevBuf<double> ba2;
    DevBuf<uint8_t> visit;
    DevBuf<unsigned long long> lvl;
    DevBuf<long long> vbase;
    std::vector<unsigned long long> lastLvl;
    std::vector<size_t> lastSlotsU, lastSlotsC;
    long long lastU = -1, lastC = -1, lastR = 0;
    plan::FrontierNeeds need;
    FPools lastPools{};
    int capE = 0;
    plan::FrontierCaps caps() const
    {
        plan::FrontierCaps k;
        k.itemsU = itemsU.cap; k.itemsC = itemsC.cap; k.tw = tw.cap; k.ta = ta.cap; k.trec = trec.cap; k.tflag = tflag.cap; k.arec = arec.cap;
        k.sw = sw.cap; k.sa = sa.cap; k.sais = sais.cap; k.bw = bw.cap; k.bw2 = bw2.cap; k.recs = recs.cap;
        k.perm = perm.cap; k.perm2 = perm2.cap; k.perm3 = perm3.cap; k.perm4 = perm4.cap; k.visit = visit.cap; k.lsize = lsize.cap;
        k.lpos = lpos.cap; k.lpar = lpar.cap; k.passList = passList.cap; k.passListR = passListR.cap;
        return k;
    }
};

struct QuiesceOnExit {
    hipStream_t s[3];
    bool armed = true;
    ~QuiesceOnExit() { if (armed) for (hipStream_t x : s) (void)hipStreamSynchronize(x); }
    void disarm() { armed = false; }
};

}

int frontier_search(maple_ctx *c, const SearchParams &P, int m, const int32_t *nodes, int budget, int zeroBudget, SearchOut *hostOut,
                    uint2 *poolW, double *poolA, unsigned long long *poolUsed, long long poolCapW, long long poolCapA,
                    FrontierStats *stats, long long itemsHint, const FrontierWide *wide, const uint8_t *overHint)
{
    if (!c->frontier) c->frontier.reset(new FrontierScratch());
    FrontierScratch &F = *static_cast<FrontierScratch *>(c->frontier.get());
    if (budget < 1) budget = 1 << 30;
    const auto tEnter = std::chrono::steady_clock::now();
    auto sinceEnter = [&] { return std::chrono::duration_cast<std::chrono::microseconds>(std::chrono::steady_clock::now() - tEnter).count() * 1e-3; };
    const bool dbgTime = c->tuning.verbose != 0;
    plan::FrontierPlanIn in;
    size_t totalB = 0;
    if (hipMemGetInfo(&in.freeBytes, &totalB) != hipSuccess) in.freeBytes = (size_t)8 << 30;
    const size_t allocs0 = devbuf_stats().allocs, allocBytes0 = devbuf_stats().bytes;
    struct PoolCap { const char *name; const size_t *cap; size_t elem, before; };
    PoolCap poolCaps[] = {{"itemsU", &F.itemsU.cap, 1, 0}, {"itemsC", &F.itemsC.cap, 1, 0}, {"tw", &F.tw.cap, 8, 0}, {"ta", &F.ta.cap, 8, 0},
                          {"trec", &F.trec.cap, 16, 0}, {"sw", &F.sw.cap, 8, 0}, {"sa", &F.sa.cap, 8, 0}, {"sais", &F.sais.cap, 8, 0},
                          {"bw", &F.bw.cap, 8, 0}, {"bw2", &F.bw2.cap, 8, 0}, {"visit", &F.visit.cap, 1, 0}, {"recs", &F.recs.cap, 1, 0},
                          {"perm", &F.perm.cap, 4, 0}, {"passList", &F.passList.cap, 4, 0}};
    for (PoolCap &pc : poolCaps) pc.before = *pc.cap;
    in.m = m; in.budget = budget; in.itemsHint = itemsHint;
    in.usingErrorRate = c->dm.usingErrorRate; in.forceWide = wide && wide->forceWide; in.matTree = c->tree_has_mut;
    in.nLists = c->h_n_ent.size(); in.usedEnt = c->used_ent; in.treeMaxEnt = c->tree_max_ent; in.waveAllBelow = c->tuning.waveAllBelow;
    static_assert(sizeof(FItem) == 96 && sizeof(FVisit) == 32 && sizeof(FRec) == 48 && FR_BLOCK == 256, "tests/search_plan_main.cpp");
    in.szItem = sizeof(FItem); in.szVisit = sizeof(FVisit); in.szRec = sizeof(FRec);
    in.frBlock = FR_BLOCK; in.heavyMult = FR_HEAVY_MULT; in.bigMin = FR_BIG_MIN;
    in.cap = F.caps(); in.capE = F.capE; in.need = F.need;
    const plan::FrontierPlan pl = plan::plan_frontier(in);
    F.capE = pl.capE;
    HIPCK(c, F.itemsU.reserve_exact(pl.resItemsU));
    HIPCK(c, F.itemsC.reserve_exact(pl.resItemsC));
    HIPCK(c, F.srch.reserve((size_t)m * sizeof(FSearch)));
    HIPCK(c, F.recs.reserve_exact(pl.resRecs));
    HIPCK(c, F.ctr.reserve(sizeof(FCtr)));
    HIPCK(c, F.tw.reserve_exact(pl.resTw));
    HIPCK(c, F.ta.reserve_exact(pl.resTa));
    HIPCK(c, F.trec.reserve_exact(pl.resTrec));
    HIPCK(c, F.arec.reserve_exact(pl.resArec));
    HIPCK(c, F.tflag.reserve_exact(pl.resTflag));
    HIPCK(c, F.sw.reserve_exact(pl.resSw));
    HIPCK(c, F.sa.reserve_exact(pl.resSa));
    HIPCK(c, F.sais.reserve_exact(pl.resSais));
    HIPCK(c, F.bw.reserve_exact(pl.resBw));
    HIPCK(c, F.ba.reserve_exact(pl.resBa));
    HIPCK(c, F.bw2.reserve_exact(pl.resBw2));
    HIPCK(c, F.ba2.reserve_exact(pl.resBa2));
    HIPCK(c, F.nodes.reserve((size_t)m));
    HIPCK(c, F.out.reserve((size_t)m * sizeof(SearchOut)));
    const plan::FrontierBound bd = plan::bind_frontier(in, pl, F.caps());
    FPools fp;
    fp.U = (FItem *)F.itemsU.p; fp.C = (FItem *)F.itemsC.p;
    fp.capU = bd.capU; fp.capC = bd.capC; fp.capCC = bd.capCC;
    fp.tw = F.tw.p; fp.ta = F.ta.p; fp.trec = F.trec.p; fp.arec = F.arec.p; fp.nArec = (int32_t)c->h_n_ent.size();
    fp.capW = bd.capW; fp.capA = bd.capA;
    fp.tflag = F.tflag.p;
    fp.capL = bd.capL;
    HIPCK(c, F.perm.reserve_exact(bd.resPerm));
    HIPCK(c, F.perm2.reserve_exact(bd.resPerm2));
    HIPCK(c, F.perm3.reserve_exact(bd.resPerm3));
    HIPCK(c, F.perm4.reserve_exact(bd.resPerm4));
    fp.perm = F.perm.p; fp.perm2 = F.perm2.p; fp.perm3 = F.perm3.p; fp.perm4 = F.perm4.p;
    fp.waveAllBelow = pl.waveAllBelow;
    fp.maxLevels = 4096;
    fp.capVisit = bd.capVisit;
    HIPCK(c, F.visit.reserve_exact(bd.resVisit));
    HIPCK(c, F.lsize.reserve_exact(bd.resLsize));
    HIPCK(c, F.lpos.reserve_exact(bd.resLpos));
    HIPCK(c, F.lpar.reserve_exact(bd.resLpar));
    fp.lsize = F.lsize.p; fp.lpos = F.lpos.p; fp.lpar = F.lpar.p;
    HIPCK(c, F.lvl.reserve((size_t)fp.maxLevels * FR_LVL));
    HIPCK(c, F.tot.reserve((size_t)m));
    HIPCK(c, F.vbase.reserve((size_t)m + 1));
    fp.visit = bd.layoutOK ? (FVisit *)F.visit.p : nullptr; fp.lvl = F.lvl.p; fp.tot = F.tot.p; fp.vbase = F.vbase.p;
    fp.sw = F.sw.p; fp.sa = F.sa.p; fp.sais = F.sais.p; fp.capE = pl.capE;
    fp.bw = F.bw.p; fp.ba = F.ba.p; fp.capBig = bd.capBig; fp.bigSide = 0;
    fp.ctr = (FCtr *)F.ctr.p; fp.S = (FSearch *)F.srch.p; fp.recs = (FRec *)F.recs.p;
    fp.capRecs = bd.capRecs;
    fp.mat = c->tree_has_mut ? 1 : 0;
    fp.mv = mview(c);
    fp.passList = nullptr; fp.capPass = 0; fp.passListR = nullptr; fp.capPassR = 0; fp.deferred = nullptr; fp.capDeferred = 0;
    if (fp.mat) {
        HIPCK(c, F.passList.reserve_exact(bd.resPassList));
        fp.passList = F.passList.p; fp.capPass = (long long)F.passList.cap;
        HIPCK(c, F.passListR.reserve_exact(bd.resPassListR));
        fp.passListR = F.passListR.p; fp.capPassR = (long long)F.passListR.cap;
        HIPCK(c, F.deferred.reserve_exact(bd.resDeferred));
        fp.deferred = F.deferred.p; fp.capDeferred = (long long)F.deferred.cap;
    }
    if (dbgTime) fprintf(stderr, "[maple]   frontier +%.1f ms: pools reserved (%zu allocations, %.2f GB; free %.1f GB, room %.1f GB; per-lane scratch %lld x %d entries, shared %lld + %lld)\n", sinceEnter(),
                         devbuf_stats().allocs - allocs0, 1e-9 * (double)(devbuf_stats().bytes - allocBytes0), 1e-9 * (double)in.freeBytes, 1e-9 * pl.room,
                         pl.scratchLanes + pl.extraSlabs, pl.capE, pl.capBig, pl.capBig2);
    if (dbgTime)
        for (const PoolCap &pc : poolCaps)
            if (*pc.cap != pc.before) fprintf(stderr, "[maple]     %s: %.3f -> %.3f GB\n", pc.name, 1e-9 * (double)(pc.before * pc.elem), 1e-9 * (double)(*pc.cap * pc.elem));
    hipStream_t s = c->stream;
    const bool dbgSync = c->tuning.verbose > 2;
    auto stage = [&](const char *what) -> int {
        if (!dbgSync) return MAPLE_OK;
        HIPCK(c, hipDeviceSynchronize());
        fprintf(stderr, "[maple] frontier: %s done\n", what);
        return MAPLE_OK;
    };
    HIPCK(c, hipMemsetAsync(fp.ctr, 0, sizeof(FCtr), s));
    HIPCK(c, hipMemcpyAsync(F.nodes.p, nodes, (size_t)m * sizeof(int32_t), hipMemcpyHostToDevice, s));
    if (overHint) {
        HIPCK(c, F.overHint.reserve((size_t)m));
        HIPCK(c, hipMemcpyAsync(F.overHint.p, overHint, (size_t)m, hipMemcpyHostToDevice, s));
    }
    SearchOut *dout = (SearchOut *)F.out.p;
    DevTree T = c->dtree;
    const ArenaViewS av = view(c);
    hipEvent_t e0, e1, er0, er1;
    size_t slotEv;
    TRY(maple_internal_ev_pair(c, &e0, &e1, MAPLE_K_SPR_SEARCH, (double)m, 0.0, &slotEv));
    HIPCK(c, hipEventRecord(e0, s));
    std::vector<int32_t> wideIdx;
    const bool useWide = wide && wide->rowOf && wide->cacheS && (wide->forceWide || budget > zeroBudget) && c->scan_valid && !c->tuning.noCladeScan
                         && (size_t)(c->tree_max_depth + 2) * 16 <= (48u << 10);
    DevTree Tw = T;
    if (useWide) {
        Tw.scan = c->t_scan.p; Tw.scanParent = c->t_scan_parent.p; Tw.scanDepthCap = c->tree_max_depth + 2;
        Tw.candBefore = c->t_cand_before.p; Tw.cladeVisits = c->t_clade_visits.p;
    }
    if (useWide) {
        for (int k = 0; k < m; k++) if (wide->rowOf[k] >= 0) wideIdx.push_back(k);
        if ((int)c->h_clade.size() == T.n)
            std::stable_sort(wideIdx.begin(), wideIdx.end(), [&](int a, int b) { return c->h_clade[nodes[a]] > c->h_clade[nodes[b]]; });
        HIPCK(c, F.wideRow.reserve((size_t)m));
        HIPCK(c, F.wideQ.reserve(std::max<size_t>(1, wideIdx.size())));
        HIPCK(c, F.wideCtr.reserve(4));
        HIPCK(c, hipMemcpyAsync(F.wideRow.p, wide->rowOf, (size_t)m * sizeof(int32_t), hipMemcpyHostToDevice, s));
        if (!wideIdx.empty())
            HIPCK(c, hipMemcpyAsync(F.wideQ.p, wideIdx.data(), wideIdx.size() * sizeof(int32_t), hipMemcpyHostToDevice, s));
        HIPCK(c, hipMemsetAsync(F.wideCtr.p, 0, 4 * sizeof(int32_t), s));
        HIPCK(c, hipStreamSynchronize(s));
    }
    const bool anyWide = useWide && !wideIdx.empty();
    if (fp.nArec > 0) {
        k_fr_arena_recs<<<std::min(4096, (fp.nArec + FR_BLOCK - 1) / FR_BLOCK), FR_BLOCK, 0, s>>>(av, fp.nArec, F.arec.p);
        HIPCK(c, hipGetLastError());
    }
    DISPATCH3(c, k_fr_begin, <<<std::min(pl.gridN, pl.gridUpd), FR_BLOCK, 0, s>>>(c->d_model, av, T, P, m, F.nodes.p, fp, dout, budget, zeroBudget,
                                                            anyWide ? F.wideRow.p : nullptr, anyWide ? wide->forceWide : 0,
                                                            overHint ? F.overHint.p : nullptr));
    HIPCK(c, hipGetLastError());
    FCtr hc;
    std::memset(&hc, 0, sizeof hc);
    int levels = 0;
    std::vector<size_t> slotsC, slotsU;
    if (!F.side) {
        {
            int prLow = 0, prHigh = 0;
            if (hipDeviceGetStreamPriorityRange(&prLow, &prHigh) != hipSuccess) prLow = 0;
            HIPCK(c, F.side.create(&prLow));
            HIPCK(c, F.side2.create(&prLow));
        }
        HIPCK(c, F.evFork2.create(hipEventDisableTiming));
        HIPCK(c, F.evJoin2.create(hipEventDisableTiming));
        HIPCK(c, F.evFork.create(hipEventDisableTiming));
        HIPCK(c, F.evJoin.create(hipEventDisableTiming));
    }
    const hipStream_t s2 = F.side, s3 = F.side2;
    FPools fpC = fp;
    fpC.bw = F.bw2.p; fpC.ba = F.ba2.p; fpC.capBig = (long long)F.bw2.cap; fpC.bigSide = 1;
    int launchesC = 0;
    auto u_level = [&]() -> int {
        hipEvent_t a0, a1;
        size_t slot;
        TRY(maple_internal_ev_pair(c, &a0, &a1, MAPLE_K_FR_UPDATING, 0.0, 0.0, &slot));
        slotsU.push_back(slot);
        HIPCK(c, hipEventRecord(a0, s));
        k_fr_sort_level<<<512, FR_BLOCK, 0, s>>>(av, T, fp, pl.heavyMin, pl.bigMin);
        TRY(stage("k_fr_sort_level"));
        TRY(fr_launch_updating(c, s, pl.gridUpd, av, T, P, fp, budget, pl.heavyMin));
        TRY(stage("k_fr_updating"));
        if (pl.heavyMin > 0) {
            TRY(fr_launch_updating_wave_small(c, s, pl.gridWaveSmall, av, T, P, fp, budget, pl.heavyMin, pl.scratchLanes + 256));
            TRY(fr_launch_updating_wave(c, s, pl.gridWave, av, T, P, fp, budget, pl.heavyMin, pl.scratchLanes));
        }
        TRY(stage("k_fr_updating_wave"));
        HIPCK(c, hipEventRecord(a1, s));
        k_fr_snap_u<<<1, 64, 0, s>>>(fp.ctr, fp.capU, fp.capC - fp.capCC, fp.capPassR, fp.lvl, fp.maxLevels);
        HIPCK(c, hipEventRecord(F.evFork, s));
        HIPCK(c, hipStreamWaitEvent(s2, F.evFork, 0));
        levels++;
        return MAPLE_OK;
    };
    bool passQueued = false;
    auto c_launch = [&]() -> int {
        hipEvent_t b0, b1;
        size_t slot;
        TRY(maple_internal_ev_pair(c, &b0, &b1, MAPLE_K_FR_CACHED, 0.0, 0.0, &slot));
        slotsC.push_back(slot);
        if (fp.mat && passQueued) HIPCK(c, hipStreamWaitEvent(s2, F.evJoin2, 0));
        k_fr_snap_c<<<1, 64, 0, s2>>>(fp.ctr, fp.capCC, fp.capPass, fp.capDeferred, fp.lvl, fp.maxLevels);
        HIPCK(c, hipEventRecord(b0, s2));
        if (fp.mat) {
            HIPCK(c, hipEventRecord(F.evFork2, s2));
            HIPCK(c, hipStreamWaitEvent(s3, F.evFork2, 0));
            DISPATCH3(c, k_fr_pass_wave, <<<1024, FR_BLOCK, 0, s3>>>(c->d_model, av, T, fp));
            DISPATCH3(c, k_fr_pass, <<<256, FR_BLOCK, 0, s3>>>(c->d_model, av, T, fpC, pl.scratchLanes + 2048));
            HIPCK(c, hipEventRecord(F.evJoin2, s3));
            passQueued = true;
            TRY(stage("k_fr_pass"));
        }
        DISPATCH3(c, k_fr_cached, <<<pl.gridCached, FR_BLOCK, 0, s2>>>(c->d_model, av, anyWide ? Tw : T, P, fp, budget,
                                                                        anyWide ? F.wideRow.p : nullptr,
                                                                        anyWide ? wide->fin : FiniteRows{nullptr, nullptr, 0}));
        HIPCK(c, hipEventRecord(b1, s2));
        TRY(stage("k_fr_cached"));
        launchesC++;
        return MAPLE_OK;
    };
    QuiesceOnExit quiesce{{s, s2, s3}};
    k_fr_snap_u<<<1, 64, 0, s>>>(fp.ctr, fp.capU, fp.capC - fp.capCC, fp.capPassR, fp.lvl, fp.maxLevels);
    HIPCK(c, hipGetLastError());
    HIPCK(c, hipEventRecord(F.evFork, s));
    HIPCK(c, hipStreamWaitEvent(s2, F.evFork, 0));
    if (anyWide && wide->rowsReady) HIPCK(c, hipStreamWaitEvent(s2, wide->rowsReady, 0));
    for (;;) {
        for (int g = 0; g < pl.groupLevels; g++) {
            TRY(u_level());
            for (int k2 = 0; k2 < 2; k2++) TRY(c_launch());
        }
        HIPCK(c, hipGetLastError());
        HIPCK(c, hipMemcpyAsync(&hc, fp.ctr, sizeof(FCtr), hipMemcpyDeviceToHost, s));
        HIPCK(c, hipStreamSynchronize(s));
        if (hc.hiU == hc.loU) break;
        if (levels > 100000) return fail(c, MAPLE_ERR_FATAL, "frontier search did not terminate");
    }
    for (;;) {
        for (int g = 0; g < pl.groupLevels; g++) TRY(c_launch());
        if (passQueued) HIPCK(c, hipStreamWaitEvent(s2, F.evJoin2, 0));
        HIPCK(c, hipGetLastError());
        HIPCK(c, hipMemcpyAsync(&hc, fp.ctr, sizeof(FCtr), hipMemcpyDeviceToHost, s2));
        HIPCK(c, hipStreamSynchronize(s2));
        const unsigned long long haveC = std::min<unsigned long long>(hc.usedC, (unsigned long long)fp.capCC),
                                 haveR = std::min<unsigned long long>(hc.usedR, (unsigned long long)(fp.capC - fp.capCC));
        if (hc.hiC == haveC && hc.hiR == haveR && hc.hiD == std::min<unsigned long long>(hc.nDeferred, (unsigned long long)fp.capDeferred)) break;
        if (launchesC > 200000) return fail(c, MAPLE_ERR_FATAL, "frontier search did not terminate");
    }
    HIPCK(c, hipEventRecord(F.evJoin, s2));
    HIPCK(c, hipStreamWaitEvent(s, F.evJoin, 0));
    if (dbgTime) fprintf(stderr, "[maple]   frontier +%.1f ms: expansion done (%d updating levels, %d cached launches)\n", sinceEnter(), levels, launchesC);
    size_t slotWide = (size_t)-1;
    if (anyWide) {
        hipEvent_t w0, w1;
        TRY(maple_internal_ev_pair(c, &w0, &w1, MAPLE_K_FR_WIDE, 0.0, 0.0, &slotWide));
        const int capB = 512, gridW = (int)std::min<size_t>(8192, wideIdx.size());
        HIPCK(c, F.wideBr.reserve_exact(std::max(F.wideBr.cap, (size_t)gridW * capB * sizeof(BestRec))));
        HIPCK(c, hipEventRecord(F.evFork, s));
        HIPCK(c, hipStreamWaitEvent(s2, F.evFork, 0));
        HIPCK(c, hipEventRecord(w0, s2));
        const size_t dyn = (size_t)Tw.scanDepthCap * (sizeof(double) + sizeof(int) + sizeof(unsigned));
        k_fr_replay_wide<<<gridW, 64, dyn, s2>>>(Tw, P, (int)wideIdx.size(), F.wideQ.p, F.wideRow.p, wide->cacheS, wide->fin, fp, dout,
                                                  (BestRec *)F.wideBr.p, capB, F.wideCtr.p);
        HIPCK(c, hipGetLastError());
        HIPCK(c, hipEventRecord(w1, s2));
        HIPCK(c, hipEventRecord(F.evJoin, s2));
    }
    TRY(maple_internal_ev_pair(c, &er0, &er1, MAPLE_K_FR_REPLAY, (double)m, 0.0));
    HIPCK(c, hipEventRecord(er0, s));
    if (levels <= fp.maxLevels && launchesC <= fp.maxLevels && fp.visit) {
        HIPCK(c, hipMemsetAsync(fp.lpos, 0xFF, (size_t)fp.capVisit * sizeof(int32_t), s));
        for (int l = launchesC - 1; l >= 0; l--) k_fr_layout_sizes<<<pl.gridLayout, FR_BLOCK, 0, s>>>(fp, l, 1);
        for (int l = levels - 1; l >= 0; l--) k_fr_layout_sizes<<<pl.gridLayout, FR_BLOCK, 0, s>>>(fp, l, 0);
        k_fr_layout_totals<<<pl.gridN, FR_BLOCK, 0, s>>>(m, fp);
        k_fr_layout_scan<<<1, 1024, 0, s>>>(m, fp.tot, fp.vbase);
        k_fr_layout_seeds<<<pl.gridN, FR_BLOCK, 0, s>>>(m, fp);
        for (int l = 0; l < levels; l++) k_fr_layout_place<<<pl.gridLayout, FR_BLOCK, 0, s>>>(fp, l, 0);
        for (int l = 0; l < launchesC; l++) k_fr_layout_place<<<pl.gridLayout, FR_BLOCK, 0, s>>>(fp, l, 1);
        HIPCK(c, hipGetLastError());
        TRY(stage("k_fr_layout"));
    } else fp.visit = nullptr;
    k_fr_replay<<<pl.gridN, FR_BLOCK, 0, s>>>(P, m, fp, dout);
    TRY(stage("k_fr_replay"));
    if (anyWide) HIPCK(c, hipStreamWaitEvent(s, F.evJoin, 0));
    if (anyWide && fp.mat && wide->nFrames > 0) {
        DISPATCH3(c, k_fr_wide_frames, <<<std::min(pl.gridUpd, 512), FR_BLOCK, 0, s>>>(c->d_model, av, T, fp, wide->frameParent, wide->frameNode));
        TRY(stage("k_fr_wide_frames"));
    }
    DISPATCH3(c, k_fr_refine, <<<pl.gridUpd, FR_BLOCK, 0, s>>>(c->d_model, av, T, fp));
    TRY(stage("k_fr_refine"));
    k_fr_finish<<<pl.gridN, FR_BLOCK, 0, s>>>(av, T, P, m, fp, dout, poolW, poolA, poolUsed, poolCapW, poolCapA);
    HIPCK(c, hipGetLastError());
    HIPCK(c, hipEventRecord(er1, s));
    HIPCK(c, hipEventRecord(e1, s));
    HIPCK(c, hipMemcpyAsync(hostOut, dout, (size_t)m * sizeof(SearchOut), hipMemcpyDeviceToHost, s));
    HIPCK(c, hipMemcpyAsync(&hc, fp.ctr, sizeof(FCtr), hipMemcpyDeviceToHost, s));
    HIPCK(c, hipStreamSynchronize(s));
    quiesce.disarm();
    if (dbgTime) fprintf(stderr, "[maple]   frontier +%.1f ms: replay, refinement, final selection done; results on the host\n", sinceEnter());
    if (dbgTime && (hc.fbReason[0] | hc.fbReason[1] | hc.fbReason[2] | hc.fbReason[3] | hc.fbReason[4] | hc.fbReason[5] | hc.fbReason[6] | hc.fbReason[7]))
        fprintf(stderr, "[maple]   exact walk handed searches to the one-lane kernel: %d a merge within tolerance, %d a list re-expressed from a shortened one, "
                        "%d a fifth shortened list, %d the search's own first list shortened, %d marked list without a layout, %d other; whole-tree searches: "
                        "%d short list / scan slots / marked item list, %d a scanned branch whose list shorten() would change\n",
                hc.fbReason[1], hc.fbReason[2], hc.fbReason[3], hc.fbReason[4], hc.fbReason[5], hc.fbReason[0], hc.fbReason[6], hc.fbReason[7]);
    if (dbgTime && hc.overflow)
        fprintf(stderr, "[maple]   frontier pools, asked / capacity: updating items %llu / %lld, cached items %llu / %lld, roots %llu / %lld, temporary lists %llu / %lld "
                        "(words %llu / %lld, aux %llu / %lld), pass entries %llu / %lld, of roots %llu / %lld, records %llu / %lld\n",
                hc.usedU, fp.capU, hc.usedC, fp.capCC, hc.usedR, fp.capC - fp.capCC, hc.nLists, fp.capL, hc.usedW, fp.capW, hc.usedA, fp.capA,
                hc.nPass, fp.capPass, hc.nPassR, fp.capPassR, hc.nRecs, fp.capRecs);
    {
        const double meanCand = c->n_scored ? c->scored_bytes_total / c->n_scored : 0.0;
        double units = 0.0, bytes = 0.0;
        double unitsW = 0.0, bytesW = 0.0;
        for (int k = 0; k < m; k++) {
            if (hostOut[k].status != 0 && hostOut[k].status != -1) continue;
            if (anyWide && wide->rowOf[k] >= 0) {
                const int32_t l = c->h_tree_lower[nodes[k]];
                unitsW += hostOut[k].nAppend;
                bytesW += 8.0 * hostOut[k].nAppend + (l >= 0 ? 8.0 * c->h_n_ent[l] + 8.0 * c->h_n_aux[l] : 0.0);
                continue;
            }
            units += hostOut[k].nAppend;
            const int32_t l = c->h_tree_lower[nodes[k]];
            bytes += meanCand * hostOut[k].nAppend + (l >= 0 ? 8.0 * c->h_n_ent[l] + 8.0 * c->h_n_aux[l] : 0.0);
        }
        c->ev_units[slotEv] = units; c->ev_bytes[slotEv] = bytes;
        if (slotWide != (size_t)-1) { c->ev_units[slotWide] = unitsW; c->ev_bytes[slotWide] = bytesW; }
        if (!slotsC.empty()) { c->ev_units[slotsC[0]] = (double)hc.scoredC; c->ev_bytes[slotsC[0]] = (double)hc.bytesC; }
        if (!slotsU.empty()) { c->ev_units[slotsU[0]] = (double)hc.itemsU; c->ev_bytes[slotsU[0]] = (double)hc.bytesU; }
    }
#ifdef MAPLE_SPR_PROFILE
    {
        const char *nm[8] = {"<64", "<96", "<128", "<192", "<256", "<384", "<512", ">=512"};
        for (int b = 0; b < 8; b++)
            if (hc.dbgCnt[b]) fprintf(stderr, "[maple] one-lane updating items, lists of %s entries: %llu items, mean %.3f ms, slowest %.3f ms\n", nm[b],
                                      hc.dbgCnt[b], hc.dbgT[b] * 1e-5 / hc.dbgCnt[b], hc.dbgMax[b] * 1e-5);
    }
    if (hc.dbgC[0])
        fprintf(stderr, "[maple] k_fr_cached, per wavefront-iteration (%llu of them, %.1f scored items each): %.2f us before the scores (item, search, node, "
                        "list table), %.2f us in the scores (%.1f entries per scored item in its two lists, the longest of an iteration %.1f), %.2f us "
                        "after them (rule, pushes)\n",
                hc.dbgC[0], (double)hc.dbgC[5] / hc.dbgC[0], hc.dbgC[1] * 1e-2 / hc.dbgC[0], hc.dbgC[2] * 1e-2 / hc.dbgC[0],
                (double)hc.dbgC[6] / std::max(1.0, (double)hc.dbgC[5]), (double)hc.dbgC[4] / hc.dbgC[0], hc.dbgC[3] * 1e-2 / hc.dbgC[0]);
    {
        const char *nm[4] = {"small class", "512 class", "small class, one lane (a list does not fit)", "512 class, one lane (a list does not fit)"};
        for (int b = 0; b < 4; b++)
            if (hc.dbgWCnt[b]) fprintf(stderr, "[maple] wavefront-wide updating items, %s: %llu items, mean %.3f ms, slowest %.3f ms\n", nm[b],
                                       hc.dbgWCnt[b], hc.dbgWT[b] * 1e-5 / hc.dbgWCnt[b], hc.dbgWMax[b] * 1e-5);
    }
    if (anyWide) {
        double tw = 0, ts = 0, mw = 0, ms = 0; long long ns = 0, mxn = 0;
        for (int k : wideIdx) {
            tw += hostOut[k].tStep * 1e-5; ts += hostOut[k].tReplay * 1e-5; ns += hostOut[k].nSteps;
            mw = std::max(mw, hostOut[k].tStep * 1e-5); ms = std::max(ms, hostOut[k].tReplay * 1e-5); mxn = std::max<long long>(mxn, hostOut[k].nSteps);
        }
        fprintf(stderr, "[maple] wide replay profile over %zu searches: item walk %.1f ms total (max %.2f), scans %.1f ms total (max %.2f), %lld scans (max %lld)\n",
                wideIdx.size(), tw, mw, ts, ms, ns, mxn);
    }
#endif
    F.need = plan::remember_frontier(F.need, m, anyWide && wide->forceWide, hc.usedU, hc.usedC, hc.usedR, hc.nLists, hc.usedW, hc.usedA, hc.overflow != 0);
    F.lastU = std::min((long long)hc.usedU, fp.capU); F.lastC = std::min((long long)hc.usedC, fp.capCC);
    F.lastR = std::min((long long)hc.usedR, fp.capC - fp.capCC); F.lastPools = fp;
    {
        const int nl = std::min(std::max(levels, launchesC), fp.maxLevels);
        F.lastLvl.assign((size_t)nl * FR_LVL, 0ull);
        if (nl) HIPCK(c, hipMemcpy(F.lastLvl.data(), fp.lvl, (size_t)nl * FR_LVL * sizeof(unsigned long long), hipMemcpyDeviceToHost));
        for (int l = 0; l < nl; l++) {
            unsigned long long *L = F.lastLvl.data() + (size_t)FR_LVL * l;
            if (l >= levels) L[0] = L[1] = L[6] = L[7] = 0;
            if (l >= launchesC) L[2] = L[3] = L[4] = L[5] = 0;
        }
        F.lastSlotsU = slotsU; F.lastSlotsC = slotsC;
    }
    if (hc.overflow) F.lastU = F.lastC = -1;
    if (stats) {
        stats->levels = levels; stats->itemsUpdating = (long long)hc.usedU; stats->itemsCached = (long long)(hc.usedC + hc.usedR);
        stats->tempLists = (long long)hc.nLists; stats->tempWords = (long long)hc.usedW; stats->tempAux = (long long)hc.usedA;
        stats->records = (long long)hc.nRecs; stats->overflow = hc.overflow;
    }
    return MAPLE_OK;
}

int frontier_export(maple_ctx *c, long long cap, int32_t *q, int32_t *node, long long *n)
{
    FrontierScratch *F = static_cast<FrontierScratch *>(c->frontier.get());
    if (!F || F->lastU < 0) return fail(c, MAPLE_ERR_STATE, "no complete frontier search to export");
    const long long tot = F->lastU + F->lastC + F->lastR;
    *n = tot;
    if (tot > cap) return fail(c, MAPLE_ERR_ARG, "%lld expanded items do not fit in %lld", tot, cap);
    if (tot == 0) return MAPLE_OK;
    HIPCK(c, F->expQ.reserve((size_t)tot));
    HIPCK(c, F->expNode.reserve((size_t)tot));
    k_fr_export<<<(int)std::min<long long>(1024, (tot + FR_BLOCK - 1) / FR_BLOCK), FR_BLOCK, 0, c->stream>>>(F->lastPools, F->lastU, F->lastC, F->lastR,
                                                                                                          F->expQ.p, F->expNode.p);
    HIPCK(c, hipGetLastError());
    HIPCK(c, hipMemcpyAsync(q, F->expQ.p, (size_t)tot * sizeof(int32_t), hipMemcpyDeviceToHost, c->stream));
    HIPCK(c, hipMemcpyAsync(node, F->expNode.p, (size_t)tot * sizeof(int32_t), hipMemcpyDeviceToHost, c->stream));
    HIPCK(c, hipStreamSynchronize(c->stream));
    return MAPLE_OK;
}

int frontier_level_profile(maple_ctx *c, int cap, long long *itemsU, long long *itemsC, float *msU, float *msC, int *n, long long *waveSmall,
                           long long *waveBig)
{
    FrontierScratch *F = static_cast<FrontierScratch *>(c->frontier.get());
    if (!F) return fail(c, MAPLE_ERR_STATE, "no frontier search to report on");
    const int nl = (int)(F->lastLvl.size() / FR_LVL);
    *n = nl;
    for (int l = 0; l < nl && l < cap; l++) {
        const unsigned long long *L = F->lastLvl.data() + (size_t)FR_LVL * l;
        itemsU[l] = (long long)(L[1] - L[0]);
        itemsC[l] = (long long)(L[3] - L[2]) + (long long)(L[5] - L[4]);
        if (waveSmall) waveSmall[l] = (long long)L[6];
        if (waveBig) waveBig[l] = (long long)L[7];
        msU[l] = msC[l] = 0.f;
        const size_t su = l < (int)F->lastSlotsU.size() ? F->lastSlotsU[l] : (size_t)-1 / 4, sc = l < (int)F->lastSlotsC.size() ? F->lastSlotsC[l] : (size_t)-1 / 4;
        if (2 * su + 1 < c->ev_used) { HIPCK(c, hipEventSynchronize(c->evs[2 * su + 1])); HIPCK(c, hipEventElapsedTime(&msU[l], c->evs[2 * su], c->evs[2 * su + 1])); }
        if (2 * sc + 1 < c->ev_used) { HIPCK(c, hipEventSynchronize(c->evs[2 * sc + 1])); HIPCK(c, hipEventElapsedTime(&msC[l], c->evs[2 * sc], c->evs[2 * sc + 1])); }
    }
    return MAPLE_OK;
}
```

### maple_amd/csrc/frontier_dev.h

```cpp
#pragma once
#include "ctx_host.h"
#include "frontier.h"

#include <algorithm>
#include <cstring>

namespace frt {

#define FR_BLOCK 256
#ifndef FR_HEAVY_MULT
#define FR_HEAVY_MULT 24
#endif
#ifndef FR_BIG_MIN
#define FR_BIG_MIN 176
#endif

enum { FI_UPD_IN = 1, FI_UPD_OUT = 2, FI_SCORED = 4, FI_DEAD = 8, FI_REC_UPD = 16, FI_SEED = 32, FI_SEED_EMPTY = 64,
       FI_NEEDPASS = 128 };
enum { FS_ACTIVE = 0, FS_FINAL = 1, FS_OVER = 2, FS_FALLBACK = 3, FS_WIDE = 4 };
__device__ __forceinline__ bool fs_live(int st) { return st == FS_ACTIVE || st == FS_WIDE; }
#define FR_NONE (-1)

typedef ulonglong2 LRec;
#define LREC_OFF(x) ((long long)((x) & ((1ull << 40) - 1)))
#define LREC_N(x) ((int32_t)((x) >> 40))
__device__ __host__ __forceinline__ LRec lrec_make(long long offW, int n, long long offA, int na)
{
    LRec r;
    r.x = (unsigned long long)offW | ((unsigned long long)(uint32_t)n << 40);
    r.y = (unsigned long long)offA | ((unsigned long long)(uint32_t)na << 40);
    return r;
}

struct alignas(32) FItem {
    int8_t dir;
    uint8_t flags;
    int16_t failsA;
    int32_t next;
    int32_t child0, child1;
    double midProb, lastLK;
    int32_t q, t1;
    int32_t hPassed, hRpr;
    double distance, pathBest;
    int16_t failsP, pad;
    int32_t hA, hB, hMid;
    double recDist;
    int32_t pad2[2];
};
static_assert(sizeof(FItem) == 96, "FItem");

struct alignas(32) FVisit {
    double midProb, lastLK;
    int32_t ref, size;
    int32_t parent;
    uint8_t flags; int8_t dir; int16_t failsOut;
};
static_assert(sizeof(FVisit) == 32, "FVisit");

struct FSearch {
    int32_t node, parent, sibling;
    int32_t hRpr0;
    int32_t seed0, seed1;
    int32_t nItems;
    int32_t state;
    int32_t slHead, nApp, recBase, recCount;
    int32_t isRemovedTip;
    int32_t rprMerge0;
    double removedBLen, curLK;
};

struct FRec { int32_t q, ref; double optimized, top, bottom, app; int32_t ok;
              int32_t hRprS; };
#define FR_SHORTEN (-3)
#define FR_FRAMES_EVENT (-4)
#define FR_FRAMES (-2)

struct FCtr {
    alignas(128) unsigned long long loU;
    unsigned long long hiU;
    alignas(128) unsigned long long loC;
    unsigned long long hiC, loR, hiR, loPR, hiPR;
    alignas(128) unsigned long long safeR;
    unsigned long long safePassR;
    alignas(128) unsigned long long usedU;
    alignas(128) unsigned long long usedC;
    alignas(128) unsigned long long usedR;
    alignas(128) unsigned long long nPassR;
    alignas(128) unsigned long long bigUsedC;
    alignas(128) unsigned long long nDeferred;
    unsigned long long loD, hiD;
    alignas(128) unsigned long long permDown;
    alignas(128) unsigned long long permUp;
    alignas(128) unsigned long long permDownB;
    alignas(128) unsigned long long permUpB;
    alignas(128) unsigned long long permHeavy;
    alignas(128) unsigned long long permHeavy2;
    alignas(128) unsigned long long nLists;
    alignas(128) unsigned long long usedW;
    alignas(128) unsigned long long usedA;
    alignas(128) unsigned long long nRecs;
    alignas(128) unsigned long long nPass;
    unsigned long long loP, hiP;
    unsigned long long bigUsed;
    alignas(128) unsigned long long itemsU;
    unsigned long long bytesU;
    alignas(128) unsigned long long scoredC;
    unsigned long long bytesC;
    int32_t overflow, nLevels, nLevelsC;
    int32_t fbReason[8];
#ifdef MAPLE_SPR_PROFILE
    unsigned long long dbgCnt[8], dbgT[8], dbgMax[8];
    unsigned long long dbgC[8];
    unsigned long long dbgWCnt[4], dbgWT[4], dbgWMax[4];
#endif
};

struct FPools {
    FItem *U, *C;
    long long capU, capC;
    long long capCC;
    uint2 *tw; double *ta;
    LRec *trec;
    const LRec *arec; int32_t nArec;
    uint8_t *tflag;
    long long capW, capA, capL;
    FVisit *visit; long long capVisit;
    int32_t *lsize, *lpos, *lpar;
    unsigned long long *lvl;
    int32_t maxLevels;
    int32_t *tot; long long *vbase;
    int32_t *perm, *perm2;
    int32_t *perm3, *perm4;
    int32_t waveAllBelow;
    uint2 *sw; double *sa; double *sais;
    int32_t capE;
    uint2 *bw; double *ba;
    long long capBig;
    int32_t bigSide;
    FCtr *ctr;
    FSearch *S;
    FRec *recs;
    long long capRecs;
    int32_t mat;
    MutViewS mv;
    int32_t *passList; long long capPass;
    int32_t *passListR; long long capPassR;
    int32_t *deferred; long long capDeferred;
};

__device__ __forceinline__ FItem &item_of(const FPools &fp, int ref) { return ref >= 0 ? fp.C[ref] : fp.U[-(ref + 2)]; }

struct FList { const uint2 *w; const double *aux; int32_t n, na; };

__device__ __forceinline__ bool fvalid(int h) { return h >= 0 || h <= -10; }
__device__ __forceinline__ int ftree(int listId) { return listId < 0 ? -1 : -(listId + 10); }
__device__ __forceinline__ FList flist(const ArenaViewS &av, const FPools &fp, int h)
{
    if (h >= 0) { const LRec r = fp.trec[h]; return FList{fp.tw + LREC_OFF(r.x), fp.ta + LREC_OFF(r.y), LREC_N(r.x), LREC_N(r.y)}; }
    const int id = -h - 10;
    if (id < fp.nArec) { const LRec r = fp.arec[id]; return FList{av.words + LREC_OFF(r.x), av.aux + LREC_OFF(r.y), LREC_N(r.x), LREC_N(r.y)}; }
    return FList{av.words + av.ent_off[id], av.aux + av.aux_off[id], av.n_ent[id], av.n_aux[id]};
}
__device__ __forceinline__ int flen(const ArenaViewS &av, const FPools &fp, int h)
{
    if (h >= 0) return LREC_N(fp.trec[h].x);
    const int id = -h - 10;
    return id < fp.nArec ? LREC_N(fp.arec[id].x) : av.n_ent[id];
}
__device__ __forceinline__ ListRef fref(const FList &l) { return ListRef{l.w, l.aux}; }

struct FScr { uint2 *w; double *a; };
__device__ inline bool fscratch(const FPools &fp, long long laneId, int need, FScr &o)
{
    if (need <= fp.capE) { o.w = fp.sw + laneId * fp.capE; o.a = fp.sa + laneId * 5ll * fp.capE; return true; }
    const unsigned long long off = atomicAdd(fp.bigSide ? &fp.ctr->bigUsedC : &fp.ctr->bigUsed, (unsigned long long)need);
    if ((long long)(off + need) > fp.capBig) return false;
    o.w = fp.bw + off; o.a = fp.ba + 5ull * off;
    return true;
}

__device__ inline int fstore(const FPools &fp, const Writer &wr)
{
    const unsigned long long act = __ballot(1);
    const int lane = threadIdx.x & 63, leader = (int)__ffsll((long long)act) - 1;
    int preN = 0, preA = 0, totN = 0, totA = 0, rank = 0, cnt = 0;
    for (unsigned long long mm = act; mm; mm &= mm - 1) {
        const int j = (int)__ffsll((long long)mm) - 1;
        const int nj = __builtin_amdgcn_readlane(wr.n, j), aj = __builtin_amdgcn_readlane(wr.na, j);
        if (j < lane) { preN += nj; preA += aj; rank++; }
        totN += nj; totA += aj; cnt++;
    }
    unsigned long long id0 = 0, ow0 = 0, oa0 = 0;
    if (lane == leader) {
        id0 = atomicAdd(&fp.ctr->nLists, (unsigned long long)cnt);
        ow0 = atomicAdd(&fp.ctr->usedW, (unsigned long long)totN);
        oa0 = atomicAdd(&fp.ctr->usedA, (unsigned long long)totA);
    }
    auto bc = [&](unsigned long long x) {
        return ((unsigned long long)(uint32_t)__builtin_amdgcn_readlane((int)(x >> 32), leader) << 32)
               | (uint32_t)__builtin_amdgcn_readlane((int)x, leader);
    };
    const unsigned long long id = bc(id0) + (unsigned long long)rank, ow = bc(ow0) + (unsigned long long)preN,
                             oa = bc(oa0) + (unsigned long long)preA;
    if ((long long)id >= fp.capL || (long long)(ow + wr.n) > fp.capW || (long long)(oa + wr.na) > fp.capA) {
        fp.ctr->overflow = 1;
        return -2;
    }
    uint2 *dw = fp.tw + ow;
    double *da = fp.ta + oa;
    for (int k = 0; k < wr.n; k++) dw[k] = wr.w[k];
    for (int k = 0; k < wr.na; k++) da[k] = wr.aux[k];
    fp.trec[id] = lrec_make((long long)ow, wr.n, (long long)oa, wr.na); fp.tflag[id] = 0;
    return (int)id;
}

__device__ inline int wave_excl_sum_f(int v, int lane, int &total)
{
    int incl = v;
    for (int off = 1; off < 64; off <<= 1) {
        const int t = __shfl_up(incl, off);
        incl += (lane >= off) ? t : 0;
    }
    total = __shfl(incl, 63);
    return incl - v;
}

template <class C> __device__ inline int shorten_would_merge(const C &c, ListRef L, int nEnt)
{
    const double thr = c.m.thresholdProb;
    Cursor a;
    a.init(L);
    Ent head = a.e;
    int level = 0;
    bool exact = true;
    for (int k = 1; k < nEnt; k++) {
        a.next();
        const Ent &nw = a.e;
        bool absorb = false;
        if (nw.type == 4 && head.type == 4 && nw.hasD0 == head.hasD0 && nw.hasD1 == head.hasD1) {
            if (!nw.hasD0) absorb = true;
            else if (fabs(nw.d0 - head.d0) > thr) absorb = false;
            else if (nw.hasD1 && fabs(nw.d1 - head.d1) > thr) absorb = false;
            else absorb = (nw.flag == head.flag);
        }
        if (absorb) {
            if (nw.hasD0 && (nw.d0 != head.d0 || (nw.hasD1 && nw.d1 != head.d1))) exact = false;
            level = max(level, exact ? 1 : 2);
        } else { head = nw; exact = true; }
    }
    return level;
}

__device__ inline int fpass_store(const FPools &fp, const ArenaViewS &av, const int lRef, const long long laneId, const int h, const int mutId,
                                  const bool dirUp)
{
    if (!fvalid(h) || mutId < 0) return h;
    const int cnt = fp.mv.cnt[mutId];
    if (cnt == 0) return h;
    const FList l = flist(av, fp, h);
    FScr scr{nullptr, nullptr};
    if (!fscratch(fp, laneId, l.n + 2 * cnt, scr)) return -2;
    Writer wr;
    wr.init(scr.w, scr.a);
    pass_walk(lRef, fref(l), fp.mv.mut3 + 3 * fp.mv.off[mutId], cnt, dirUp, wr);
    return fstore(fp, wr);
}
template <class C>
__device__ inline int fpass_removed(const C &c, const FPools &fp, const ArenaViewS &av, const long long laneId, const int h, const int mutId,
                                    const bool dirUp)
{
    const int r = fpass_store(fp, av, c.m.lRef, laneId, h, mutId, dirUp);
    if (r == h || r < 0) return r;
    const FList l = flist(av, fp, r);
    fp.tflag[r] = (uint8_t)shorten_would_merge(c, fref(l), l.n);
    return r;
}
template <class C>
__device__ inline int wave_pass(const C &c, const FPools &fp, const ArenaViewS &av, const int h, const int mutId, const bool dirUp, const bool removed)
{
    if (!fvalid(h) || mutId < 0) return h;
    const int cnt = fp.mv.cnt[mutId];
    if (cnt == 0) return h;
    const int lane = threadIdx.x & 63;
    const FList l = flist(av, fp, h);
    const int32_t *mut = fp.mv.mut3 + 3 * fp.mv.off[mutId];
// ... 48 lines not shown
        int idx = nOut + wave_excl_sum_f(cntOut, lane, totN);
        int ao = nAux + wave_excl_sum_f(auxOut, lane, totA);
        if (i < l.n) {
            auto put = [&](int type, int pos, int ref, bool tails, bool vec) {
                const uint32_t meta = (uint32_t)type | ((uint32_t)ref << 3) | ((tails && e.hasD0) ? 1u << 5 : 0u) | ((tails && e.hasD1) ? 1u << 6 : 0u)
                                      | ((tails && e.flag) ? 1u << 7 : 0u) | ((uint32_t)ao << 8);
                dw[idx++] = make_uint2((uint32_t)pos, meta);
                if (tails && e.hasD0) da[ao++] = e.d0;
                if (tails && e.hasD1) da[ao++] = e.d1;
                if (vec) { da[ao] = e.vec[0]; da[ao + 1] = e.vec[1]; da[ao + 2] = e.vec[2]; da[ao + 3] = e.vec[3]; ao += 4; }
            };
            if (e.type == 5) put(5, e.pos, 0, false, false);
            else if (e.type == 4) {
                int last = prevEnd;
                for (int k = a; k < b; k++) {
                    const int mp = mut[3 * k], from = mut[3 * k + 1], to = mut[3 * k + 2];
                    if (mp > last + 1) put(4, mp - 1, 0, true, false);
                    put(dirUp ? to : from, mp, dirUp ? from : to, true, false);
                    last = mp;
                }
                if (last < e.pos) put(4, e.pos, 0, true, false);
            } else if (a < b) {
                const int newRef = dirUp ? mut[3 * a + 1] : mut[3 * a + 2];
                if (e.type == 6) put(6, e.pos, newRef, true, true);
                else if (e.type == newRef) put(4, e.pos, 0, true, false);
                else put(e.type, e.pos, newRef, true, false);
            } else put(e.type, e.pos, e.ref, true, e.type == 6);
        }
        nOut += totN; nAux += totA;
    }
    __threadfence();
    sync();
    int level = 0;
    if (removed) {
        bool plain = false, tails = false;
        for (int j = 1 + lane; j < nOut; j += 64) {
            const uint32_t m1 = dw[j].y, m0 = dw[j - 1].y;
            if ((m1 & 7u) == 4u && (m0 & 7u) == 4u && ((m1 ^ m0) & 0x60u) == 0u) { if (m1 & 0x20u) tails = true; else plain = true; }
        }
        if (__ballot(tails)) {
            if (lane == 0) level = shorten_would_merge(c, ListRef{dw, da}, nOut);
            level = __shfl(level, 0, 64);
        } else level = __ballot(plain) ? 1 : 0;
    }
    if (lane == 0) {
        fp.trec[id] = lrec_make((long long)ow, nOut, (long long)oa, nAux); fp.tflag[id] = (uint8_t)level;
    }
    __threadfence();
    sync();
    return (int)id;
}

__device__ __forceinline__ int frpr_marked(const FPools &fp, const FSearch &S, const int h)
{
    return h >= 0 ? (int)fp.tflag[h] : (h <= -10 ? S.rprMerge0 : 0);
}

__device__ inline int fpush(const FPools &fp, const int budget, const int q, const bool upd, const int t1, const int dir,
                            const int hPassed, const double distance, const double lastLK, const int fails, const int hRpr,
                            const double pathBest, const bool needPass = false, const bool fromC = false)
{
    FSearch &S = fp.S[q];
    if (S.state != FS_WIDE && atomicAdd(&S.nItems, 1) >= budget) { S.state = FS_OVER; return FR_NONE; }
    FItem *it;
    int ref;
    unsigned long long *ctrp = upd ? &fp.ctr->usedU : (fromC ? &fp.ctr->usedC : &fp.ctr->usedR);
    const unsigned long long act = __ballot(1);
    const int lane = threadIdx.x & 63, leader = (int)__ffsll((long long)act) - 1;
    const unsigned long long same = __ballot(upd);
    const unsigned long long mine = upd ? (act & same) : (act & ~same);
    const int lead2 = (int)__ffsll((long long)mine) - 1;
    unsigned long long base = 0;
    if (lane == lead2) base = atomicAdd(ctrp, (unsigned long long)__popcll(mine));
    base = ((unsigned long long)(uint32_t)__shfl((int)(base >> 32), lead2, 64) << 32) | (uint32_t)__shfl((int)base, lead2, 64);
    (void)leader;
    const unsigned long long i = base + (unsigned long long)__popcll(mine & ((1ull << lane) - 1ull));
    if (upd) {
        if ((long long)i >= fp.capU) { S.state = FS_FALLBACK; fp.ctr->overflow = 1; return FR_NONE; }
        it = &fp.U[i]; ref = -((int)i + 2);
    } else if (fromC) {
        if ((long long)i >= fp.capCC) { S.state = FS_FALLBACK; fp.ctr->overflow = 1; return FR_NONE; }
        it = &fp.C[i]; ref = (int)i;
    } else {
        if ((long long)i >= fp.capC - fp.capCC) { S.state = FS_FALLBACK; fp.ctr->overflow = 1; return FR_NONE; }
        it = &fp.C[fp.capCC + i]; ref = (int)(fp.capCC + i);
    }
    it->q = q; it->t1 = t1; it->dir = (int8_t)dir; it->flags = upd ? FI_UPD_IN : 0; it->failsP = (int16_t)fails;
    it->hPassed = hPassed; it->hRpr = hRpr; it->distance = distance; it->lastLK = lastLK; it->pathBest = pathBest;
    it->child0 = it->child1 = FR_NONE; it->hA = it->hB = it->hMid = -1; it->next = FR_NONE; it->failsA = 0;
    it->midProb = lastLK; it->recDist = 0.0;
    if (needPass) {
        it->flags |= FI_NEEDPASS;
        const unsigned long long k = atomicAdd(fromC ? &fp.ctr->nPass : &fp.ctr->nPassR, 1ull);
        if ((long long)k >= (fromC ? fp.capPass : fp.capPassR)) { S.state = FS_FALLBACK; fp.ctr->overflow = 1; }
        else (fromC ? fp.passList : fp.passListR)[k] = ref;
    }
    return ref;
}

struct PRule { int fails; double pathBest; bool go; };
__device__ __forceinline__ PRule p_rule(const SearchParams &P, bool scored, double midProb, double lastLK, int fails, double pathBest)
{
    PRule r;
    r.fails = fails; r.pathBest = pathBest;
    if (scored) {
        if (midProb > pathBest) { r.pathBest = midProb; r.fails = 0; }
        else if (midProb < (lastLK - P.thrConsec)) r.fails = fails + 1;
    }
    const bool within = midProb > (r.pathBest - P.thrLKtopology);
    r.go = P.strict ? (r.fails <= P.allowedFails && within) : (r.fails <= P.allowedFails || within);
    return r;
}

__device__ __forceinline__ int fr_upd_size(const ArenaViewS &av, const DevTree &T, const FPools &fp, const FItem &it)
{
    if (it.dir == 3) return 0;
    const NodeRec &r1 = T.nd[it.t1];
    const int other = it.dir == 0 ? it.t1 : (it.dir == 1 ? r1.c1 : r1.c0);
    const int lw = T.nd[other].lower;
    const int nTree = lw >= 0 ? flen(av, fp, ftree(lw)) : 0;
    const int nPass = fvalid(it.hPassed) ? flen(av, fp, it.hPassed) : 0;
    return nPass + nTree;
}
__device__ __forceinline__ bool fr_upd_heavy(const ArenaViewS &av, const DevTree &T, const FPools &fp, const FItem &it, int heavyMin)
{
    return heavyMin > 0 && it.dir != 3 && fr_upd_size(av, T, fp, it) >= heavyMin;
}
__device__ inline bool fr_wave_fits(const ArenaViewS &av, const DevTree &T, const FPools &fp, const FItem &it, const int wuIn, const int capW)
{
    const int dir = it.dir;
    if (dir == 3 || !fvalid(it.hPassed)) return false;
    const NodeRec r1 = T.nd[it.t1];
    const int nP = flen(av, fp, it.hPassed), nR = flen(av, fp, it.hRpr);
    if (nP > wuIn || nR > capW) return false;
    const int other = dir == 0 ? -1 : (dir == 1 ? r1.c1 : r1.c0);
    const int upT = r1.up;
    const bool mat = fp.mat && (r1.c0Frame != r1.frameOf || r1.c1Frame != r1.frameOf || r1.upFrame != r1.frameOf);
    auto grow = [&](int mutId) { return (mat && mutId >= 0) ? 2 * fp.mv.cnt[mutId] : 0; };
    const int g0 = (dir == 0 && r1.c0 >= 0) ? grow(T.nd[r1.c0].mutId) : 0, g1 = (dir == 0 && r1.c1 >= 0) ? grow(T.nd[r1.c1].mutId) : 0;
    const int gO = other >= 0 ? grow(T.nd[other].mutId) : 0, gU = (dir != 0 && upT >= 0) ? grow(r1.mutId) : 0;
    const int ids[6] = {r1.lower, r1.totUp, dir == 0 && r1.c0 >= 0 ? T.nd[r1.c0].lower : -1, dir == 0 && r1.c1 >= 0 ? T.nd[r1.c1].lower : -1,
                        other >= 0 ? T.nd[other].lower : -1,
                        (dir != 0 && upT >= 0) ? (r1.whichChild ? T.nd[upT].upLeft : T.nd[upT].upRight) : -1};
    const int add[6] = {0, 0, g0, g1, gO, gU};
    for (int k = 0; k < 6; k++) if (ids[k] >= 0 && av.n_ent[ids[k]] + add[k] > wuIn) return false;
    if (dir != 0 && ids[4] >= 0 && nP + av.n_ent[ids[4]] + gO > wuIn) return false;
    return true;
}
struct WaveSmall {
    static constexpr int wuIn = 128, capW = 256, profCls = 0;
    static constexpr int32_t *FPools::*perm = &FPools::perm3;
    static constexpr unsigned long long FCtr::*count = &FCtr::permHeavy;
};
struct WaveBig {
    static constexpr int wuIn = 512, capW = 512, profCls = 1;
    static constexpr int32_t *FPools::*perm = &FPools::perm4;
    static constexpr unsigned long long FCtr::*count = &FCtr::permHeavy2;
};

__device__ __forceinline__ int fr_level_heavy_min(const FPools &fp, int heavyMin)
{
    const long long n = (long long)(fp.ctr->hiU - fp.ctr->loU);
    return (heavyMin > 0 && n <= fp.waveAllBelow) ? 1 : heavyMin;
}

}

__attribute__((visibility("hidden")))
int fr_launch_updating(maple_ctx *c, hipStream_t s, int grid, const ArenaViewS &av, const DevTree &T, const SearchParams &P, const frt::FPools &fp,
                       int budget, int heavyMin);
__attribute__((visibility("hidden")))
int fr_launch_updating_wave(maple_ctx *c, hipStream_t s, int grid, const ArenaViewS &av, const DevTree &T, const SearchParams &P,
                            const frt::FPools &fp, int budget, int heavyMin, long long laneBase);
__attribute__((visibility("hidden")))
int fr_launch_updating_wave_small(maple_ctx *c, hipStream_t s, int grid, const ArenaViewS &av, const DevTree &T, const SearchParams &P,
                                  const frt::FPools &fp, int budget, int heavyMin, long long laneBase);
```

### maple_amd/csrc/frontier_upd_wave.h

```cpp
#pragma once
#include "frontier_upd_lane.h"
#include "wave_dev.h"
#include "wave_update.h"

namespace frt {

__device__ inline int fstore_wave(const FPools &fp, const unsigned long long *w, const double *a, int n, int na)
{
    const int lane = threadIdx.x & 63;
    unsigned long long id = 0, ow = 0, oa = 0;
    if (lane == 0) {
        id = atomicAdd(&fp.ctr->nLists, 1ull);
        ow = atomicAdd(&fp.ctr->usedW, (unsigned long long)n);
        oa = atomicAdd(&fp.ctr->usedA, (unsigned long long)na);
    }
    auto bc = [](unsigned long long x) {
        return ((unsigned long long)(uint32_t)__shfl((int)(x >> 32), 0, 64) << 32) | (uint32_t)__shfl((int)x, 0, 64);
    };
    id = bc(id); ow = bc(ow); oa = bc(oa);
    if ((long long)id >= fp.capL || (long long)(ow + n) > fp.capW || (long long)(oa + na) > fp.capA) {
        if (lane == 0) fp.ctr->overflow = 1;
        return -2;
    }
    unsigned long long *dw = (unsigned long long *)(fp.tw + ow);
    double *da = fp.ta + oa;
    for (int k = lane; k < n; k += 64) dw[k] = w[k];
    for (int k = lane; k < na; k += 64) da[k] = a[k];
    if (lane == 0) { fp.trec[id] = lrec_make((long long)ow, n, (long long)oa, na); fp.tflag[id] = 0; }
    __threadfence();
    wave_sync();
    return (int)id;
}

static_assert(sizeof(WaveUpdLds<WaveSmall::wuIn>) == 27680 && sizeof(WaveUpdLds<WaveBig::wuIn>) == 110720 && sizeof(Lds) == 160, "LDS per wavefront");

}
```

### maple_amd/csrc/search_plan.h

```cpp
#pragma once
#include <algorithm>
#include <cstddef>
#include <cstdint>
#include <vector>

namespace maple {
namespace plan {


struct FrontierNeeds {
    long long needU = 0, needC = 0, needR = 0, needL = 0, needW = 0, needA = 0, needM = 0;
    bool lastOverflow = false;
};

struct FrontierCaps {
    size_t itemsU = 0, itemsC = 0, tw = 0, ta = 0, trec = 0, tflag = 0, arec = 0, sw = 0, sa = 0, sais = 0, bw = 0, bw2 = 0, recs = 0;
    size_t perm = 0, perm2 = 0, perm3 = 0, perm4 = 0, visit = 0, lsize = 0, lpos = 0, lpar = 0, passList = 0, passListR = 0;
};

struct FrontierPlanIn {
    int m = 0, budget = 0;
    long long itemsHint = 0;
    bool usingErrorRate = false, forceWide = false, matTree = false;
    size_t nLists = 0;
    long long usedEnt = 0;
    int treeMaxEnt = 0;
    size_t freeBytes = 0;
    int waveAllBelow = 0;
    size_t szItem = 0, szVisit = 0, szRec = 0;
    int frBlock = 0, heavyMult = 0, bigMin = 0;
    FrontierCaps cap;
    int capE = 0;
    FrontierNeeds need;
};

struct FrontierPlan {
    size_t resItemsU, resItemsC, resRecs, resTw, resTa, resTrec, resArec, resTflag, resSw, resSa, resSais, resBw, resBa, resBw2, resBa2;
    long long capU, capC, capR, capL, capW, capA;
    bool growthCut;
    int capE;
    long long scratchLanes, extraSlabs;
    int gridUpd;
    long long capBig, capBig2, capRecs;
    double room;
    int gridN, gridCached, heavyMin, bigMin, gridWave, gridWaveSmall, groupLevels, gridLayout, waveAllBelow;
};

static inline size_t grow(size_t want, size_t cap) { return want <= cap ? cap : std::max(want, cap + cap / 2); }

static inline FrontierPlan plan_frontier(const FrontierPlanIn &in)
{
    FrontierPlan p;
    const FrontierCaps &F = in.cap;
    const int m = in.m, budget = in.budget;
    const size_t held = F.itemsU + F.itemsC + F.tw * 8 + F.ta * sizeof(double)
                        + F.sw * 8 + F.sa * sizeof(double) + F.sais * sizeof(double) + F.bw * 48 + F.bw2 * 48;
    const double room = 0.5 * (double)(in.freeBytes + held);
    p.room = room;
    const bool longSearches = in.usingErrorRate && !in.forceWide;
    const long long perSearchC = longSearches ? std::min<long long>(budget, std::max<long long>(768, budget / 4)) : std::min<long long>(budget, 768);
    long long capC = std::max<long long>(1 << 16, std::max((long long)m * perSearchC, in.itemsHint));
    long long capU = std::max<long long>(1 << 14, (long long)m * std::min<long long>(budget, 16));
    long long capR = std::max<long long>(1 << 16, std::min(capC, (long long)m * std::min<long long>(budget, 32)));
    const long long meanEnt = std::max<long long>(16, in.nLists == 0 ? 64 : in.usedEnt / (long long)in.nLists);
    long long capL = (longSearches ? 6 : 2) * capU;
    long long capW = 2 * capL * meanEnt, capA = capW;
    if (in.need.needM > 0 && !in.forceWide) {
        const double f = (in.need.lastOverflow ? 2.0 : 1.25) * std::min(16.0, (double)m / (double)in.need.needM);
        capU = std::max(capU, (long long)(f * in.need.needU)); capC = std::max(capC, (long long)(f * in.need.needC)); capR = std::max(capR, (long long)(f * in.need.needR));
        capL = std::max(capL, (long long)(f * in.need.needL));
        capW = std::max<long long>(1 << 20, (long long)(f * in.need.needW)); capA = std::max<long long>(1 << 20, (long long)(f * in.need.needA));
    }
    const int capE = std::max(in.capE, std::max(256, std::min(1024, (6 * (int)meanEnt + 31) / 32 * 32)));
    p.capE = capE;
    long long scratchLanes = m <= 64 ? 16384 : 256ll * 4 * 4 * 64;
    const long long extraSlabs = 2048 + (in.matTree ? 256ll * in.frBlock : 0);
    while (scratchLanes > 16384 && (double)(scratchLanes + extraSlabs) * capE * 64 > 0.25 * room) scratchLanes /= 2;
    p.scratchLanes = scratchLanes; p.extraSlabs = extraSlabs;
    p.gridUpd = (int)(scratchLanes / in.frBlock);
    const long long capBig = std::max<long long>(1 << 20, 64ll * 1024 * std::max(1, in.treeMaxEnt));
    const long long capBig2 = in.matTree ? std::max<long long>(1 << 20, capBig / 4) : 0;
    p.capBig = capBig; p.capBig2 = capBig2;
    {
        const long long curU = (long long)(F.itemsU / in.szItem), curCR = (long long)(F.itemsC / in.szItem);
        const long long curL = (long long)std::min(F.trec, F.tflag);
        const long long curW = (long long)F.tw, curA = (long long)F.ta;
        const double perItem = (double)(in.szItem + in.szVisit + 12);
        const double fixed = (double)(scratchLanes + extraSlabs) * capE * 64 + (double)(capBig + capBig2) * 48;
        const double base = (double)(curCR + curU) * perItem + (double)(curW + curA) * 8 + (double)curL * 24 + fixed;
        const double gCR = std::max<double>(0.0, (double)(capC + capR - curCR)), gU = std::max<double>(0.0, (double)(capU - curU));
        const double gL = std::max<double>(0.0, (double)(capL - curL)), gW = std::max<double>(0.0, (double)(capW - curW)), gA = std::max<double>(0.0, (double)(capA - curA));
        const double growth = (gCR + gU) * perItem + (gW + gA) * 8 + gL * 24;
        double f = 1.0;
        if (base + growth > room && growth > 0) f = std::max(0.0, (room - base) / growth);
        p.growthCut = f < 1.0;
        const double wantCR = std::max<double>((double)curCR, (double)curCR + f * gCR);
        const double shareR = (double)capR / (double)(capC + capR);
        capR = std::max<long long>(1 << 16, (long long)(wantCR * shareR)); capC = std::max<long long>(1 << 16, (long long)wantCR - capR);
        capU = std::max<long long>(1 << 14, std::max(curU, (long long)(curU + f * gU)));
        capL = std::max<long long>(2 * (1 << 14), std::max(curL, (long long)(curL + f * gL)));
        capW = std::max<long long>(1 << 20, std::max(curW, (long long)(curW + f * gW)));
        capA = std::max<long long>(1 << 20, std::max(curA, (long long)(curA + f * gA)));
    }
    p.capU = capU; p.capC = capC; p.capR = capR; p.capL = capL; p.capW = capW; p.capA = capA;
    const long long capRecs = std::max<long long>(1 << 14, (long long)m * 16);
    p.capRecs = capRecs;
    p.resItemsU = grow((size_t)capU * in.szItem, F.itemsU);
    p.resItemsC = grow((size_t)(capC + capR) * in.szItem, F.itemsC);
    p.resRecs = grow((size_t)capRecs * in.szRec, F.recs);
    p.resTw = grow((size_t)capW, F.tw);
    p.resTa = grow((size_t)capA, F.ta);
    p.resTrec = grow((size_t)capL, F.trec);
    p.resArec = grow(in.nLists, F.arec);
    p.resTflag = grow((size_t)capL, F.tflag);
    p.resSw = (size_t)(scratchLanes + extraSlabs) * capE;
    p.resSa = (size_t)(scratchLanes + extraSlabs) * capE * 5;
    p.resSais = (size_t)(scratchLanes + extraSlabs) * capE * 2;
    p.resBw = (size_t)capBig;
    p.resBa = (size_t)capBig * 5;
    p.resBw2 = (size_t)capBig2;
    p.resBa2 = (size_t)capBig2 * 5;
    p.gridN = std::max(1, std::min(2048, (m + in.frBlock - 1) / in.frBlock));
    p.gridCached = (int)std::min<long long>(16384, std::max<long long>(512, (long long)m / 12));
    p.heavyMin = m <= 64 ? 1 : std::max(256, in.heavyMult * (int)meanEnt / 4); p.gridWave = 256; p.gridWaveSmall = 1280;
    p.bigMin = m <= 64 ? (1 << 30) : in.bigMin;
    p.groupLevels = m <= 64 ? 2 : 8;
    p.gridLayout = (int)std::min<long long>(1024, std::max<long long>(64, (long long)m / 64));
    p.waveAllBelow = in.waveAllBelow > 0 ? in.waveAllBelow : (in.waveAllBelow < 0 ? 0 : 49152);
    return p;
}

struct FrontierBound {
    long long capU, capC, capCC, capW, capA, capL, capBig, capRecs, capVisit;
    bool layoutOK;
    size_t resPerm, resPerm2, resPerm3, resPerm4, resVisit, resLsize, resLpos, resLpar, resPassList, resPassListR, resDeferred;
};

static inline FrontierBound bind_frontier(const FrontierPlanIn &in, const FrontierPlan &p, const FrontierCaps &after)
{
    FrontierBound b;
    b.capU = (long long)(after.itemsU / in.szItem); b.capC = (long long)(after.itemsC / in.szItem);
    b.capCC = b.capC - std::max(p.capR, (long long)((double)b.capC * p.capR / (double)(p.capC + p.capR)));
    b.capW = (long long)after.tw; b.capA = (long long)after.ta;
    b.capL = (long long)std::min(after.trec, after.tflag);
    b.resPerm = std::max(after.perm, (size_t)b.capU);
    b.resPerm2 = std::max(after.perm2, (size_t)b.capU);
    b.resPerm3 = std::max(after.perm3, (size_t)b.capU);
    b.resPerm4 = std::max(after.perm4, (size_t)b.capU);
    b.capVisit = b.capU + b.capC;
    b.layoutOK = in.m > 64 && b.capVisit < (1ll << 31) - 64;
    b.resVisit = b.resLsize = b.resLpos = b.resLpar = 0;
    if (b.layoutOK) {
        b.resVisit = std::max(after.visit, (size_t)b.capVisit * in.szVisit);
        b.resLsize = std::max(after.lsize, (size_t)b.capVisit);
        b.resLpos = std::max(after.lpos, (size_t)b.capVisit);
        b.resLpar = std::max(after.lpar, (size_t)b.capVisit);
    }
    b.capBig = (long long)after.bw;
    b.capRecs = (long long)(after.recs / in.szRec);
    b.resPassList = b.resPassListR = b.resDeferred = 0;
    if (in.matTree) {
        b.resPassList = std::max(after.passList, (size_t)std::max<long long>(1 << 16, b.capC / 8));
        b.resPassListR = std::max(after.passListR, (size_t)std::max<long long>(1 << 16, (b.capC - b.capCC) / 4));
        b.resDeferred = b.resPassList + b.resPassListR;
    }
    return b;
}

static inline FrontierNeeds remember_frontier(const FrontierNeeds &before, int m, bool wideOnly, unsigned long long usedU, unsigned long long usedC,
                                       unsigned long long usedR, unsigned long long nLists, unsigned long long usedW, unsigned long long usedA,
                                       bool overflow)
{
    FrontierNeeds n = before;
    if (!wideOnly && (m >= 1024 || m >= before.needM)) {
        n.needU = (long long)usedU; n.needC = (long long)usedC; n.needR = (long long)usedR; n.needL = (long long)nLists; n.needW = (long long)usedW;
        n.needA = (long long)usedA; n.needM = m; n.lastOverflow = overflow;
    }
    return n;
}


static inline int lane_cap_w0(int wsEntriesPerLane, int treeMaxEnt) { return wsEntriesPerLane > 0 ? wsEntriesPerLane : std::max(16384, 64 * treeMaxEnt); }
static inline int lane_start_cap_w(int capW0, bool cached, bool heavyQueries) { return cached ? (heavyQueries ? 8 : 4) * capW0 : capW0; }

struct LanePlanIn {
    int m = 0, attempt = 0, capW = 0;
    bool cached = false, strict = false, assist = false;
    bool freeKnown = false;
    size_t freeBytes = 0, wsCap = 0;
    size_t szList = 0, szStack = 0, szBest = 0;
};

struct LanePlan {
    int32_t capW, capA, capH, capS, capB, capAis;
    size_t w, aux, h, st, best, ais, total;
    long long wsBudget, maxLanes;
    int lanesWanted, activeLanes, nWaves, lanes;
    size_t reserve;
};

static inline LanePlan plan_lane_launch(const LanePlanIn &in)
{
    LanePlan p;
    const int m = in.m, attempt = in.attempt;
    p.capW = in.capW;
    p.capA = 5 * p.capW;
    p.capH = p.capW / 8 + 256;
    p.capS = 1024 * (attempt + 1);
    p.capB = (in.cached ? 4096 : 1024) * (attempt + 1);
    p.capAis = 8192 * (attempt + 1);
    auto al = [](size_t x) { return (x + 63) & ~(size_t)63; };
    p.w = al((size_t)p.capW * 8);
    p.aux = al((size_t)p.capA * sizeof(double));
    p.h = al((size_t)p.capH * in.szList);
    p.st = al((size_t)p.capS * in.szStack);
    p.best = al((size_t)p.capB * in.szBest);
    p.ais = al((size_t)p.capAis * sizeof(double));
    p.total = p.w + p.aux + p.h + p.st + p.best + p.ais;
    long long wsBudget = 96ll << 30;
    if (in.freeKnown) {
        const long long avail = (long long)((double)(in.freeBytes + in.wsCap) * 0.7);
        if (avail < wsBudget) wsBudget = avail;
    }
    long long maxLanes = wsBudget / (long long)p.total;
    if (maxLanes > 4096 * 64) maxLanes = 4096 * 64;
    if (in.cached && maxLanes > 8192) maxLanes = 8192;
    if (maxLanes < 64) maxLanes = 64;
    const int lanesWanted = (int)(m < maxLanes ? m : maxLanes);
    const int lanesDiv = in.strict ? 32768 : (lanesWanted > 65536 ? 8192 : 16384);
    int activeLanes = (lanesWanted + lanesDiv - 1) / lanesDiv;
    if (activeLanes < 1) activeLanes = 1;
    if (activeLanes > 64) activeLanes = 64;
    if (!in.cached && in.assist && activeLanes > 4) activeLanes = 4;
    int nWaves = (lanesWanted + activeLanes - 1) / activeLanes;
    if (nWaves > 8192) nWaves = 8192;
    const int lanes = nWaves * activeLanes;
    p.wsBudget = wsBudget; p.maxLanes = maxLanes; p.lanesWanted = lanesWanted; p.activeLanes = activeLanes; p.nWaves = nWaves; p.lanes = lanes;
    {
        size_t need = (size_t)lanes * p.total;
        if (need > in.wsCap) {
            const size_t top = (size_t)maxLanes * p.total;
            need = std::min(std::max(need, 2 * in.wsCap), std::max(top, need));
        }
        p.reserve = need;
    }
    return p;
}


static inline bool patched_only(bool nodesCurrent, bool matTree, int n, int searchTier, bool tracing, bool wantsLists, int requested,
                                bool usingErrorRate, bool anyZeroLength)
{
    if (!(nodesCurrent && !matTree && n <= 64 && searchTier == 0 && !tracing && !wantsLists)) return false;
    return !(requested >= 0 && !usingErrorRate && anyZeroLength);
}

static inline int wide_budget(int requested, int nScored, bool usingErrorRate, bool patchedOnly, int budgetDefault)
{
    int wideBudget = requested == 0 ? std::max(budgetDefault, std::min(8192, nScored / 64)) : requested;
    if (patchedOnly) wideBudget = -1;
    if (requested == 0) wideBudget = usingErrorRate ? std::min(2 * wideBudget, std::max(wideBudget, 8192)) : 2 * wideBudget;
    return wideBudget;
}

static inline int frontier_budget(int wideBudget, int requested, int nScored, bool usingErrorRate)
{
    if (wideBudget <= 0) return 0;
    return usingErrorRate ? wideBudget : std::max(wideBudget, requested == 0 ? nScored / 2 : 0);
}

static inline size_t score_rows_max(bool freeKnown, size_t freeBytes, size_t cacheCapBytes, int nNodes)
{
    size_t budget = (size_t)4ull << 30;
    if (freeKnown) budget = std::max(budget, std::min((freeBytes + cacheCapBytes) / 2, (size_t)96ull << 30));
    return std::max<size_t>(1, budget / ((size_t)nNodes * sizeof(double)));
}

struct RouteIn {
    int wideBudget = 0;
    bool usingErrorRate = false, matTree = false, useFrontier = false;
    bool scanValid = false, havePlace = false;
    bool hintsCoverTree = false;
    bool noCladeScan = false, denseWideScoring = false, wideOutsideFrontier = false, noOverHint = false;
};

enum PreRowsKind { PRE_NONE = 0, PRE_WITNESS = 1, PRE_HINTED = 2 };
static inline PreRowsKind pre_rows_kind(const RouteIn &r)
{
    const bool hybrid = r.wideBudget > 0;
    if (hybrid && !r.usingErrorRate && r.wideBudget > 16
        && (!r.matTree || (r.scanValid && r.havePlace && !r.noCladeScan && !r.denseWideScoring && !r.wideOutsideFrontier)))
        return PRE_WITNESS;
    if (hybrid && r.usingErrorRate && r.useFrontier && !r.noOverHint && r.hintsCoverTree && r.wideBudget > 16 && r.scanValid && r.havePlace
        && !r.noCladeScan && !r.wideOutsideFrontier)
        return PRE_HINTED;
    return PRE_NONE;
}
static inline bool pre_rows_fit(size_t nCand, size_t rowsMax) { return nCand >= 64 && nCand <= rowsMax; }
static inline int pre_rows_spare(size_t nCand, size_t rowsMax, bool witness) { return witness ? (int)std::min<size_t>(4096, rowsMax - nCand) : 0; }

static inline bool root_rows_ok(const RouteIn &r, int nF, size_t nWide)
// ... 45 lines not shown
```

### maple_amd/runtime.py

```python
from __future__ import annotations

import ctypes as C
import os

import numpy as np

from .genome_list import PackedLists, pack_lists, pack_mutations, unpack_list

HERE = os.path.dirname(os.path.abspath(__file__))
LIB_PATH = os.path.join(HERE, "libmaple_hip.so")

EXPORTS = [
    "maple_abi_version", "maple_create", "maple_destroy", "maple_set_tuning", "maple_last_error", "maple_set_model", "maple_get_model",
    "maple_lists_upload", "maple_lists_update", "maple_lists_sizes", "maple_lists_download", "maple_arena_mark", "maple_arena_release",
    "maple_arena_stats", "maple_mutations_upload", "maple_append_batch", "maple_merge_batch", "maple_blen_batch",
    "maple_differ_batch", "maple_pass_branch_batch", "maple_shorten_batch", "maple_root_vector_batch",
    "maple_evaluate_placement_batch", "maple_update_partials", "maple_update_partials_touched", "maple_tree_patch", "maple_append_batch_dev", "maple_append_queries_dev", "maple_timing_reset", "maple_timing_read", "maple_timing_read_each",
    "maple_append_algorithmic_bytes", "maple_tree_upload", "maple_spr_search_batch", "maple_minor_batch", "maple_root_prob_batch", "maple_candset_create", "maple_append_candset",
    "maple_minor_candset", "maple_placement_search_batch", "maple_placement_prepare", "maple_placement_ahead", "maple_placement_ahead_stats", "maple_set_fatal_policy",
    "maple_timing_read_kind", "maple_placement_supports_batch",
    "maple_candset_destroy", "maple_spr_search_visited", "maple_arena_compact", "maple_append_queries_argmax_dev", "maple_comm_unique_id", "maple_comm_init", "maple_argmax_allreduce_dev", "maple_tree_rebuild_lists",
    "maple_em_expectation", "maple_em_rates",
]


DEBUG_EXPORTS = ["maple_debug_wave_append_batch", "maple_debug_trace_query", "maple_debug_trace_read", "maple_debug_calib_walk",
                 "maple_debug_calib_write", "maple_debug_gpv_batch", "maple_debug_simplify_batch", "maple_debug_frontier_levels",
                 "maple_debug_frontier_pass_batch", "maple_debug_live_resources", "maple_debug_score_rows"]
LIB_PATH_DEBUG = os.path.join(HERE, "libmaple_hip_debug.so")


class MapleParams(C.Structure):
    _fields_ = [("thresholdProb", C.c_double), ("minBLenSensitivity", C.c_double),
                ("thresholdDiffForUpdate", C.c_double), ("thresholdFoldChangeUpdate", C.c_double),
                ("defaultBLen", C.c_double)]


class MapleSearchParams(C.Structure):
    _fields_ = [("strictTopologyStopRules", C.c_int32), ("allowedFailsTopology", C.c_int32),
                ("thresholdLogLKtopology", C.c_double), ("thresholdTopologyPlacement", C.c_double),
                ("thresholdLogLKoptimizationTopology", C.c_double), ("thresholdLogLKconsecutivePlacement", C.c_double),
                ("effectivelyNon0BLen", C.c_double), ("wideSearchBudget", C.c_int32), ("searchTier", C.c_int32)]


class MapleTuning(C.Structure):
    _fields_ = [("structSize", C.c_uint32), ("wavePerItemMax", C.c_int32), ("placementChunkMax", C.c_int32), ("noCladeScan", C.c_int32), ("verbose", C.c_int32),
                ("wideOutsideFrontier", C.c_int32), ("denseWideScoring", C.c_int32), ("waveAllBelow", C.c_int32), ("noOverHint", C.c_int32), ("noAheadExpansion", C.c_int32), ("noAheadSpeculation", C.c_int32)]


class MaplePlacementParams(C.Structure):
    _fields_ = [("oneMutBLen", C.c_double), ("effectivelyNon0BLen", C.c_double), ("thresholdLogLK", C.c_double),
                ("thresholdLogLKoptimization", C.c_double), ("thresholdLogLKconsecutivePlacement", C.c_double),
                ("allowedFails", C.c_int32), ("strictStopRules", C.c_int32), ("onlyFindIdentical", C.c_int32)]


class MapleEmTotals(C.Structure):
    _fields_ = [("counts", C.c_double * 16), ("waitingTimes", C.c_double * 4), ("errorCount", C.c_double), ("totTreeLength", C.c_double),
                ("observedTotNucsSites", C.c_int64), ("numTips", C.c_int64)]


EM_MODELS = {"UNREST": 0, "GTR": 1}


class MapleError(RuntimeError):
    ERR_ARG, ERR_HIP, ERR_NOMEM, ERR_STATE, ERR_FATAL = -1, -2, -3, -4, -5

    def __init__(self, msg, code=None):
        super().__init__(msg)
        self.code = code


_lib = None
_lib_debug = None


def load_library(debug=False):
    global _lib, _lib_debug
    if (_lib_debug if debug else _lib) is None:
        default = LIB_PATH_DEBUG if debug else LIB_PATH
        lib_path = os.environ.get("MAPLE_HIP_LIB_DEBUG" if debug else "MAPLE_HIP_LIB", default)
        if not os.path.exists(lib_path):
            raise MapleError(f"{lib_path} is missing: run `python -c 'import __graft_entry__ as g; g.build()'`; "
                             "there is no CPU fallback for the placement path")
        try:
            import torch
        except ImportError:
            pass
        lib = C.CDLL(lib_path)
        lib.maple_last_error.restype = C.c_char_p
        for name in EXPORTS + (DEBUG_EXPORTS if debug else []):
            if not hasattr(lib, name):
                raise MapleError(f"{lib_path} does not export {name} (include/maple_hip{'_debug' if name in DEBUG_EXPORTS else ''}.h): "
                                 "rebuild it with __graft_entry__.build()")
        if debug:
            _lib_debug = lib
        else:
            _lib = lib
    return _lib_debug if debug else _lib


def _ptr(a):
    return None if a is None else a.ctypes.data_as(C.c_void_p)


def _i32(x):
    return np.ascontiguousarray(x, dtype=np.int32)


def _u8(x):
    return np.ascontiguousarray(x, dtype=np.uint8)


def _f64(x):
    return np.ascontiguousarray(x, dtype=np.float64)


def debug_live_resources():
    a, b, h = C.c_int64(), C.c_int64(), C.c_int64()
    rc = load_library(debug=True).maple_debug_live_resources(C.byref(a), C.byref(b), C.byref(h))
    if rc != 0:
        raise MapleError(f"maple_debug_live_resources failed ({rc})", rc)
    return a.value, b.value, h.value


class Device:

    def __init__(self, ref_idx, root_freqs, *, device=0, thresholdProb=1e-8, minBLenSensitivity=None,
                 thresholdDiffForUpdate=1e-5, thresholdFoldChangeUpdate=1.01, defaultBLen=0.000033,
                 arena_bytes=0, lib=None, debug=False):
        self.lib = lib if lib is not None else load_library(debug)
        self.ref_idx = _u8(ref_idx)
        self.lRef = int(len(self.ref_idx))
        if minBLenSensitivity is None:
            minBLenSensitivity = 0.001 / self.lRef
        p = MapleParams(thresholdProb, minBLenSensitivity, thresholdDiffForUpdate, thresholdFoldChangeUpdate, defaultBLen)
        rf = _f64(root_freqs)
        h = C.c_void_p()
        rc = self.lib.maple_create(C.byref(h), int(device), self.lRef, _ptr(self.ref_idx), _ptr(rf), C.byref(p),
                                   C.c_uint64(arena_bytes))
        if rc != 0:
            raise MapleError(f"maple_create failed ({rc}): no usable MI355X / HIP runtime; the placement path has no "
                             "CPU fallback")
        self.h = h
        self.device = int(device)
        self.u = False

    def _ck(self, rc):
        if rc != 0:
            msg = self.lib.maple_last_error(self.h)
            raise MapleError(f"libmaple_hip error {rc}: {msg.decode() if msg else ''}", rc)

    def close(self):
        if getattr(self, "h", None):
            self.lib.maple_destroy(self.h)
            self.h = None

    def __del__(self):
        try:
            self.close()
        except Exception:
            pass

    def set_tuning(self, *, wave_per_item_max=0, placement_chunk_max=0, no_clade_scan=False, verbose=0, wide_outside_frontier=False,
                   dense_wide_scoring=False, wave_all_below=0, no_over_hint=False, no_ahead_expansion=False, no_ahead_speculation=False):
        t = MapleTuning(C.sizeof(MapleTuning), int(wave_per_item_max), int(placement_chunk_max), int(bool(no_clade_scan)), int(verbose),
                        int(bool(wide_outside_frontier)), int(bool(dense_wide_scoring)), int(wave_all_below), int(bool(no_over_hint)),
                        int(no_ahead_expansion), int(bool(no_ahead_speculation)))
        self._ck(self.lib.maple_set_tuning(self.h, C.byref(t)))

    def set_model(self, Q, siteRates=None, usingErrorRate=False, errorRateGlobal=0.0, errorRates=None):
        Qf = _f64(np.asarray(Q, dtype=np.float64).reshape(16))
        sr = None if siteRates is None else _f64(siteRates)
        er = None if (errorRates is None or not usingErrorRate) else _f64(errorRates)
        self._ck(self.lib.maple_set_model(self.h, _ptr(Qf), _ptr(sr), int(bool(usingErrorRate)),
                                          C.c_double(errorRateGlobal or 0.0), _ptr(er)))
        self.u = bool(usingErrorRate)
        self.rv, self.ss = sr is not None, er is not None

    def get_model(self):
        cr = np.zeros(self.lRef + 1)
        ce = np.zeros(self.lRef + 1)
# ... 281 lines not shown
    def placement_ahead(self, q_lists, *, oneMutBLen, effectivelyNon0BLen, thresholdLogLK, thresholdLogLKoptimization,
                        thresholdLogLKconsecutivePlacement, allowedFails=5, strictStopRules=True, onlyFindIdentical=False):
        q = _i32(q_lists)
        pp = MaplePlacementParams(oneMutBLen, effectivelyNon0BLen, thresholdLogLK, thresholdLogLKoptimization,
                                  thresholdLogLKconsecutivePlacement, int(allowedFails), int(bool(strictStopRules)),
                                  int(bool(onlyFindIdentical)))
        taken = C.c_int32(0)
        self._ck(self.lib.maple_placement_ahead(self.h, len(q), _ptr(q), C.byref(pp), C.byref(taken)))
        return taken.value

    def placement_ahead_stats(self):
        out = np.zeros(5, dtype=np.int64)
        self._ck(self.lib.maple_placement_ahead_stats(self.h, _ptr(out)))
        return dict(zip(("searches", "fallbacks", "expanded_items", "traversals_ahead_used", "traversals_ahead_dropped"), (int(x) for x in out)))

    def placement_search_batch(self, q_lists, *, oneMutBLen, effectivelyNon0BLen, thresholdLogLK,
                               thresholdLogLKoptimization, thresholdLogLKconsecutivePlacement, allowedFails=5,
                               strictStopRules=True, onlyFindIdentical=False):
        q = _i32(q_lists)
        n = len(q)
        pp = MaplePlacementParams(oneMutBLen, effectivelyNon0BLen, thresholdLogLK, thresholdLogLKoptimization,
                                  thresholdLogLKconsecutivePlacement, int(allowedFails), int(bool(strictStopRules)),
                                  int(bool(onlyFindIdentical)))
        out = dict(bestNode=np.zeros(n, np.int32), bestScore=np.zeros(n), blen=np.zeros((n, 3)),
                   bestDiffs=np.zeros(n, np.int32), nAppend=np.zeros(n, np.int32), status=np.zeros(n, np.int32))
        self._ck(self.lib.maple_placement_search_batch(self.h, n, _ptr(q), C.byref(pp), _ptr(out["bestNode"]),
                                                       _ptr(out["bestScore"]), _ptr(out["blen"]), _ptr(out["bestDiffs"]),
                                                       _ptr(out["nAppend"]), _ptr(out["status"])))
        return out

    def placement_supports_batch(self, q_lists, *, oneMutBLen, effectivelyNon0BLen, thresholdLogLK,
                                 thresholdLogLKoptimization, thresholdLogLKconsecutivePlacement,
                                 thresholdLogLKoptimizationTopology, minBranchSupport=0.01, allowedFails=5,
                                 strictStopRules=True, onlyFindIdentical=False):
        q = _i32(q_lists)
        n = len(q)
        pp = MaplePlacementParams(oneMutBLen, effectivelyNon0BLen, thresholdLogLK, thresholdLogLKoptimization,
                                  thresholdLogLKconsecutivePlacement, int(allowedFails), int(bool(strictStopRules)),
                                  int(bool(onlyFindIdentical)))
        cap = 128 * max(1, n)
        off = np.zeros(n + 1, np.int64)
        node, supp, bl = np.zeros(cap, np.int32), np.zeros(cap), np.zeros((cap, 3))
        best, status = np.zeros(n, np.int32), np.zeros(n, np.int32)
        self._ck(self.lib.maple_placement_supports_batch(self.h, n, _ptr(q), C.byref(pp),
                                                         C.c_double(thresholdLogLKoptimizationTopology),
                                                         C.c_double(minBranchSupport), C.c_int64(cap), _ptr(off), _ptr(node),
                                                         _ptr(supp), _ptr(bl), _ptr(best), _ptr(status)))
        out = []
        for g in range(n):
            a, b = off[g], off[g + 1]
            out.append(([(int(node[i]), float(supp[i]), tuple(float(x) for x in bl[i])) for i in range(a, b)], int(best[g])))
        return out, status

    def debug_gpv_batch(self, i12, totLen, mutMatrix, errorRate, vect, upNode, flag):
        i12 = _i32(i12)
        n = len(i12)
        M = _f64(np.asarray(mutMatrix, dtype=np.float64).reshape(n, 16))
        v = _f64(np.asarray(vect, dtype=np.float64).reshape(n, 4))
        out = np.zeros((n, 4))
        self._ck(self.lib.maple_debug_gpv_batch(self.h, n, _ptr(i12), _ptr(_f64(totLen)), _ptr(M), _ptr(_f64(errorRate)), _ptr(v),
                                                _ptr(_u8(upNode)), _ptr(_u8(flag)), _ptr(out)))
        return out

    def debug_simplify_batch(self, vec, refA):
        v = _f64(np.asarray(vec, dtype=np.float64).reshape(-1, 4))
        out = np.zeros(len(v), dtype=np.int32)
        self._ck(self.lib.maple_debug_simplify_batch(self.h, len(v), _ptr(v), _ptr(_i32(refA)), _ptr(out)))
        return out

    def debug_frontier_pass_batch(self, lists, mutLists, dirIsUp, wave_form=False):
        lists, mutLists = _i32(lists), _i32(mutLists)
        n = len(lists)
        up = _u8(np.broadcast_to(dirIsUp, n))
        out = np.zeros(n, dtype=np.int32)
        grade, same = np.zeros(n, dtype=np.uint8), np.zeros(n, dtype=np.uint8)
        self._ck(self.lib.maple_debug_frontier_pass_batch(self.h, n, _ptr(lists), _ptr(mutLists), _ptr(up), int(bool(wave_form)),
                                                          _ptr(out), _ptr(grade), _ptr(same)))
        return out, grade, same.astype(bool)

    def debug_score_rows(self, form, q_lists, qTip, qBLen, cands, out_col=None, ld_out=None, fill=float("nan")):
        q_lists, cands = _i32(q_lists), _i32(cands)
        nQ, nC = len(q_lists), len(cands)
        ld = nC if ld_out is None else int(ld_out)
        nW = (nC + 63) // 64
        tip, bl = _u8(np.broadcast_to(qTip, nQ)), _f64(np.broadcast_to(qBLen, nQ))
        col = None if out_col is None else _i32(out_col)
        assert col is None or len(col) == nC
        out = np.zeros((nQ, max(ld, 1)))
        mask = np.zeros((nQ, nW), dtype=np.uint64)
        prefix = np.zeros((nQ, nW + 1), dtype=np.int32)
        pairs = C.c_int64(-1)
        self._ck(self.lib.maple_debug_score_rows(self.h, int(form), nQ, _ptr(q_lists), _ptr(tip), _ptr(bl), nC, _ptr(cands), _ptr(col),
                                                 C.c_int64(ld), C.c_double(fill), _ptr(out), _ptr(mask), _ptr(prefix), C.byref(pairs)))
        return out, mask, prefix, pairs.value

    def debug_calib_walk(self, nbytes, repeats=1):
        ms = C.c_float()
        self._ck(self.lib.maple_debug_calib_walk(self.h, C.c_uint64(nbytes), int(repeats), C.byref(ms)))
        return ms.value

    def debug_calib_write(self, nbytes, mode, repeats=1):
        ms = C.c_float()
        self._ck(self.lib.maple_debug_calib_write(self.h, C.c_uint64(nbytes), int(mode), int(repeats), C.byref(ms)))
        return ms.value

    def debug_trace_query(self, q):
        self._ck(self.lib.maple_debug_trace_query(self.h, int(q)))

    def debug_trace_read(self):
        n = C.c_int32()
        it = np.zeros(4 * 4096, dtype=np.int32)
        va = np.zeros(2 * 4096, dtype=np.float64)
        self._ck(self.lib.maple_debug_trace_read(self.h, C.byref(n), _ptr(it), _ptr(va)))
        k = min(n.value, 4096)
        return it[: 4 * k].reshape(k, 4), va[: 2 * k].reshape(k, 2)

    def append_batch_dev(self, n, parent_ptr, child_ptr, tip_ptr, blen_ptr, out_ptr, stream=0):
        self._ck(self.lib.maple_append_batch_dev(self.h, int(n), C.c_void_p(parent_ptr), C.c_void_p(child_ptr),
                                                 C.c_void_p(tip_ptr), C.c_void_p(blen_ptr), C.c_void_p(out_ptr),
                                                 C.c_void_p(stream)))

    def append_queries_dev(self, nQ, qlist_ptr, nC, cand_ptr, isTipC, bLen, out_ptr, stream=0):
        self._ck(self.lib.maple_append_queries_dev(self.h, int(nQ), C.c_void_p(qlist_ptr), int(nC), C.c_void_p(cand_ptr),
                                                   int(bool(isTipC)), C.c_double(bLen), C.c_void_p(out_ptr),
                                                   C.c_void_p(stream)))

    def append_queries_argmax_dev(self, nQ, qlist_ptr, nC, cand_ptr, rank_ptr, isTipC, bLen, best_score_ptr, best_idx_ptr, stream=0):
        self._ck(self.lib.maple_append_queries_argmax_dev(self.h, int(nQ), C.c_void_p(qlist_ptr), int(nC), C.c_void_p(cand_ptr),
                                                          C.c_void_p(rank_ptr), int(bool(isTipC)), C.c_double(bLen),
                                                          C.c_void_p(best_score_ptr), C.c_void_p(best_idx_ptr), C.c_void_p(stream)))

    def comm_unique_id(self):
        buf = np.zeros(128, dtype=np.uint8)
        self._ck(self.lib.maple_comm_unique_id(self.h, _ptr(buf)))
        return buf

    def comm_init(self, world, rank, unique_id):
        self._ck(self.lib.maple_comm_init(self.h, int(world), int(rank), _ptr(_u8(unique_id))))

    def argmax_allreduce_dev(self, n, score_ptr, idx_ptr, stream=0):
        self._ck(self.lib.maple_argmax_allreduce_dev(self.h, int(n), C.c_void_p(score_ptr), C.c_void_p(idx_ptr), C.c_void_p(stream)))

    def timing_reset(self):
        self._ck(self.lib.maple_timing_reset(self.h))

    def timing_read_each(self, cap=256):
        ms = np.zeros(cap, dtype=np.float32)
        n = C.c_int32()
        self._ck(self.lib.maple_timing_read_each(self.h, int(cap), _ptr(ms), C.byref(n)))
        return ms[: n.value].tolist()

    def frontier_levels(self, cap=4096):
        iu, ic = np.zeros(cap, np.int64), np.zeros(cap, np.int64)
        ws, wb = np.zeros(cap, np.int64), np.zeros(cap, np.int64)
        mu, mc = np.zeros(cap, np.float32), np.zeros(cap, np.float32)
        n = C.c_int32()
        self._ck(self.lib.maple_debug_frontier_levels(self.h, int(cap), _ptr(iu), _ptr(ic), _ptr(mu), _ptr(mc), C.byref(n), _ptr(ws), _ptr(wb)))
        k = min(cap, n.value)
        self.last_wave_items = (ws[:k], wb[:k])
        return iu[:k], ic[:k], mu[:k], mc[:k]

    def tree_rebuild_lists(self, root, up, c0, c1, tip, mut, dist, lower, bump_len=0.0):
        n = len(up)
        up, c0, c1 = _i32(up), _i32(c0), _i32(c1)
        tip = np.ascontiguousarray(np.asarray(tip, np.uint8))
        mutp = None if mut is None else _i32(mut)
        assert dist.dtype == np.float64 and dist.flags.c_contiguous
        lower = _i32(lower).copy()
        ur, ul, tu = (np.full(n, -1, np.int32) for _ in range(3))
        bad = np.zeros(max(64, n), np.int32)
        nbad = C.c_int32()
        self._ck(self.lib.maple_tree_rebuild_lists(self.h, n, int(root), _ptr(up), _ptr(c0), _ptr(c1), _ptr(tip), _ptr(mutp), _ptr(dist),
                                                   _ptr(lower), _ptr(ur), _ptr(ul), _ptr(tu), C.c_double(bump_len), len(bad), _ptr(bad),
                                                   C.byref(nbad)))
        return lower, ur, ul, tu, np.unique(bad[: min(nbad.value, len(bad))])

    def em_expectation(self, n_minor=None):
        L = self.lRef
        nm = None if n_minor is None else _i32(n_minor)
        tot = MapleEmTotals()
        wts, cs, tn, on, ecs = np.zeros(4 * L), np.zeros(L), np.zeros(L + 1), np.zeros(L + 1), np.zeros(L)
        self._ck(self.lib.maple_em_expectation(self.h, _ptr(nm), C.byref(tot), _ptr(wts), _ptr(cs), _ptr(tn), _ptr(on), _ptr(ecs)))
        return dict(counts=np.array(tot.counts).reshape(4, 4), waitingTimes=np.array(tot.waitingTimes), errorCount=tot.errorCount,
                    totTreeLength=tot.totTreeLength, observedTotNucsSites=int(tot.observedTotNucsSites), numTips=int(tot.numTips),
                    waitingTimesSites=wts.reshape(L, 4), countsSites=cs, trackingNs=tn, observedNucsSites=on, errorCountSites=ecs)

    def em_rates(self, n_minor=None, model="UNREST"):
        L = self.lRef
        nm = None if n_minor is None else _i32(n_minor)
        code = model if isinstance(model, int) else EM_MODELS.get(model, 2)
        Q = np.zeros(16)
        sr = np.zeros(L) if getattr(self, "rv", False) else None
        se = np.zeros(L) if getattr(self, "ss", False) else None
        er = C.c_double()
        self._ck(self.lib.maple_em_rates(self.h, _ptr(nm), int(code), _ptr(Q), _ptr(sr), C.byref(er), _ptr(se)))
        return Q.reshape(4, 4), sr, (er.value if self.u else None), se

    def timing_read(self):
        n, ms = C.c_int32(), C.c_double()
        self._ck(self.lib.maple_timing_read(self.h, C.byref(n), C.byref(ms)))
        return n.value, ms.value

    KIND_SPR_SCORE, KIND_SPR_SEARCH, KIND_SPR_REPLAY, KIND_APPEND_QUERIES, KIND_APPEND_PAIRS, KIND_PLACE_SCORE = 1, 2, 3, 4, 5, 6
    KIND_FR_UPDATING, KIND_FR_CACHED, KIND_FR_REPLAY, KIND_FR_WIDE = 7, 8, 9, 10

    def timing_read_kind(self, kind):
        n, ms, u, b = C.c_int32(), C.c_double(), C.c_double(), C.c_double()
        self._ck(self.lib.maple_timing_read_kind(self.h, int(kind), C.byref(n), C.byref(ms), C.byref(u), C.byref(b)))
        return n.value, ms.value, u.value, b.value

    def append_algorithmic_bytes(self, parent, child=None, child_once=False):
        parent = _i32(parent)
        ch = None if child is None else _i32(child)
        b = C.c_uint64()
        self._ck(self.lib.maple_append_algorithmic_bytes(self.h, len(parent), _ptr(parent), _ptr(ch),
                                                         int(bool(child_once)), C.byref(b)))
        return b.value
```

Before: 42.53 billion.

## Add mid-size wavefront update class between small and big LDS tiers

```diff
diff --git a/__graft_entry__.py b/__graft_entry__.py
--- a/__graft_entry__.py
+++ b/__graft_entry__.py
@@ -8,7 +8,7 @@
 
 CSRC = os.path.join(ROOT, "maple_amd", "csrc")
 HIP_UNITS = ["maple_hip.hip", "append_queries.hip", "placement.hip", "update.hip", "spr_batch.hip", "frontier.hip", "frontier_upd.hip",
-             "frontier_updw128.hip", "witness.hip", "em.hip"]
+             "frontier_updw128.hip", "frontier_updw256.hip", "witness.hip", "em.hip"]
 DEBUG_UNIT = "debug_abi.hip"
 HIP_LIB = os.path.join(ROOT, "maple_amd", "libmaple_hip.so")
 HIP_LIB_DEBUG = os.path.join(ROOT, "maple_amd", "libmaple_hip_debug.so")
diff --git a/include/maple_hip_debug.h b/include/maple_hip_debug.h
--- a/include/maple_hip_debug.h
+++ b/include/maple_hip_debug.h
@@ -7,7 +7,10 @@
 #endif
 
 int maple_debug_frontier_levels(maple_ctx *ctx, int32_t cap, int64_t *itemsUpdating, int64_t *itemsCached, float *msUpdating,
-                                float *msCached, int32_t *n, int64_t *waveItemsSmall , int64_t *waveItemsBig );
+                                float *msCached, int32_t *n, int64_t *waveItemsSmall , int64_t *waveItemsBig ,
+                                int64_t *waveItemsMid );
+int maple_debug_frontier_wave_classes(maple_ctx *ctx, int32_t level, int64_t cap, int32_t *need, int32_t *needScore, uint8_t *fits,
+                                      int8_t *routed, int64_t *n);
 
 int maple_debug_wave_append_batch(maple_ctx *ctx, int32_t n, const int32_t *parentList, const int32_t *childList,
                                   const uint8_t *isTipC, const double *bLen, double *outLK, float *ms);
diff --git a/maple_amd/csrc/debug_abi.hip b/maple_amd/csrc/debug_abi.hip
--- a/maple_amd/csrc/debug_abi.hip
+++ b/maple_amd/csrc/debug_abi.hip
@@ -197,15 +197,96 @@
 }
 
 extern "C" int maple_debug_frontier_levels(maple_ctx *c, int32_t cap, int64_t *itemsUpdating, int64_t *itemsCached, float *msUpdating,
-                                           float *msCached, int32_t *n, int64_t *waveItemsSmall, int64_t *waveItemsBig)
+                                           float *msCached, int32_t *n, int64_t *waveItemsSmall, int64_t *waveItemsBig, int64_t *waveItemsMid)
 {
     if (!c || cap < 0 || !itemsUpdating || !itemsCached || !msUpdating || !msCached || !n) return MAPLE_ERR_ARG;
     HIPCK(c, hipSetDevice(c->device));
     int nn = 0;
     const int rc = frontier_level_profile(c, cap, (long long *)itemsUpdating, (long long *)itemsCached, msUpdating, msCached, &nn,
-                                          (long long *)waveItemsSmall, (long long *)waveItemsBig);
+                                          (long long *)waveItemsSmall, (long long *)waveItemsBig, (long long *)waveItemsMid);
     *n = nn;
     return rc;
+}
+
+__global__ __launch_bounds__(FR_BLOCK) void k_debug_wave_need(ArenaViewS av, DevTree T, FPools fp, int heavyMin, long long n, int32_t *need,
+                                                              int32_t *needScore, uint8_t *fits)
+{
+    const long long lo = (long long)fp.ctr->loU;
+    heavyMin = fr_level_heavy_min(fp, heavyMin);
+    for (long long i = (long long)blockIdx.x * blockDim.x + threadIdx.x; i < n; i += (long long)gridDim.x * blockDim.x) {
+        const FItem &it = fp.U[lo + i];
+        int nd = -1, ns = -1;
+        if (it.dir != 3 && fvalid(it.hPassed)) {
+            const NodeRec r1 = T.nd[it.t1];
+            const int dir = it.dir, nP = flen(av, fp, it.hPassed);
+            const bool mat = fp.mat && (r1.c0Frame != r1.frameOf || r1.c1Frame != r1.frameOf || r1.upFrame != r1.frameOf);
+            auto len = [&](int listId, int mutId) { return listId < 0 ? 0 : av.n_ent[listId] + ((mat && mutId >= 0) ? 2 * fp.mv.cnt[mutId] : 0); };
+            ns = flen(av, fp, it.hRpr);
+            nd = max(nP, max(len(r1.lower, -1), len(r1.totUp, -1)));
+            if (dir == 0) {
+                if (r1.c0 >= 0) nd = max(nd, len(T.nd[r1.c0].lower, T.nd[r1.c0].mutId));
+                if (r1.c1 >= 0) nd = max(nd, len(T.nd[r1.c1].lower, T.nd[r1.c1].mutId));
+            } else {
+                const int other = dir == 1 ? r1.c1 : r1.c0;
+                if (other >= 0 && T.nd[other].lower >= 0) nd = max(nd, nP + len(T.nd[other].lower, T.nd[other].mutId));
+                if (r1.up >= 0) nd = max(nd, len(r1.whichChild ? T.nd[r1.up].upLeft : T.nd[r1.up].upRight, r1.mutId));
+            }
+        }
+        need[i] = nd; needScore[i] = ns;
+        const int in[5] = {128, 192, 256, 384, 512}, sc[5] = {256, 512, 512, 512, 512};
+        uint8_t f = (heavyMin > 0 && it.dir != 3 && fr_upd_size(av, T, fp, it) >= heavyMin) ? 0x80 : 0;
+        for (int k = 0; k < 5; k++) if (fr_wave_fits(av, T, fp, it, in[k], sc[k])) f |= (uint8_t)(1 << k);
+        fits[i] = f;
+    }
+}
+__global__ __launch_bounds__(FR_BLOCK) void k_debug_wave_routed(FPools fp, long long n, int8_t *routed)
+{
+    const long long nS = (long long)fp.ctr->permHeavy, nM = (long long)fp.ctr->permHeavyM, nB = (long long)fp.ctr->permHeavy2;
+    for (long long k = (long long)blockIdx.x * blockDim.x + threadIdx.x; k < nS + nM + nB; k += (long long)gridDim.x * blockDim.x) {
+        const int cls = k < nS ? 0 : (k < nS + nM ? 1 : 2);
+        const int32_t i = cls == 0 ? fp.perm3[k] : (cls == 1 ? fp.perm5[k - nS] : fp.perm4[k - nS - nM]);
+        if (i >= 0 && i < n) routed[i] = (int8_t)cls;
+    }
+}
+
+extern "C" int maple_debug_frontier_wave_classes(maple_ctx *c, int32_t level, int64_t cap, int32_t *need, int32_t *needScore, uint8_t *fits,
+                                                 int8_t *routed, int64_t *n)
+{
+    if (!c || level < 0 || cap < 0 || !need || !needScore || !fits || !routed || !n) return MAPLE_ERR_ARG;
+    HIPCK(c, hipSetDevice(c->device));
+    FPools fp;
+    int heavyMin = 0, bigMin = 0;
+    std::vector<unsigned long long> ranges;
+    TRY(frontier_last_levels(c, &fp, &heavyMin, &bigMin, &ranges));
+    *n = 0;
+    if ((size_t)level >= ranges.size() / 2) return fail(c, MAPLE_ERR_ARG, "the last frontier search had %zu levels of list-updating items", ranges.size() / 2);
+    const long long lo = (long long)ranges[2 * (size_t)level], cnt = (long long)ranges[2 * (size_t)level + 1] - lo;
+    *n = cnt;
+    if (cnt > cap) return fail(c, MAPLE_ERR_ARG, "%lld items do not fit in %lld", cnt, (long long)cap);
+    if (lo < 0 || lo + cnt > fp.capU) return fail(c, MAPLE_ERR_STATE, "level %d lies outside the pool", level);
+    auto up16 = [](size_t x) { return (x + 255) & ~(size_t)255; };
+    const size_t oCtr = 0, oNeed = up16(sizeof(FCtr)), oScore = up16(oNeed + (size_t)cnt * 4), oFits = up16(oScore + (size_t)cnt * 4),
+                 oRouted = up16(oFits + (size_t)cnt), total = up16(oRouted + (size_t)cnt);
+    DevBuf<uint8_t> own;
+    HIPCK(c, own.reserve_exact(total));
+    FCtr hc;
+    memset(&hc, 0, sizeof hc);
+    hc.loU = (unsigned long long)lo; hc.hiU = (unsigned long long)(lo + cnt);
+    HIPCK(c, hipMemcpyAsync(own.p + oCtr, &hc, sizeof hc, hipMemcpyHostToDevice, c->stream));
+    HIPCK(c, hipMemsetAsync(own.p + oRouted, 0xff, (size_t)cnt, c->stream));
+    fp.ctr = (FCtr *)(own.p + oCtr);
+    const ArenaViewS av{c->d_words, c->d_aux, c->d_ent_off, c->d_aux_off, c->d_n_ent, c->d_n_aux};
+    TRY(frontier_sort_level_again(c, fp, heavyMin, bigMin));
+    hipLaunchKernelGGL(k_debug_wave_need, dim3(grid_for((int)cnt)), dim3(FR_BLOCK), 0, c->stream, av, c->dtree, fp, heavyMin, cnt, (int32_t *)(own.p + oNeed),
+                       (int32_t *)(own.p + oScore), own.p + oFits);
+    hipLaunchKernelGGL(k_debug_wave_routed, dim3(grid_for((int)cnt)), dim3(FR_BLOCK), 0, c->stream, fp, cnt, (int8_t *)(own.p + oRouted));
+    HIPCK(c, hipGetLastError());
+    HIPCK(c, hipMemcpyAsync(need, own.p + oNeed, (size_t)cnt * 4, hipMemcpyDeviceToHost, c->stream));
+    HIPCK(c, hipMemcpyAsync(needScore, own.p + oScore, (size_t)cnt * 4, hipMemcpyDeviceToHost, c->stream));
+    HIPCK(c, hipMemcpyAsync(fits, own.p + oFits, (size_t)cnt, hipMemcpyDeviceToHost, c->stream));
+    HIPCK(c, hipMemcpyAsync(routed, own.p + oRouted, (size_t)cnt, hipMemcpyDeviceToHost, c->stream));
+    HIPCK(c, hipStreamSynchronize(c->stream));
+    return MAPLE_OK;
 }
 
 template <bool RV, bool U, bool SS>
diff --git a/maple_amd/csrc/fr_wave_items_body.inc b/maple_amd/csrc/fr_wave_items_body.inc
--- a/maple_amd/csrc/fr_wave_items_body.inc
+++ b/maple_amd/csrc/fr_wave_items_body.inc
@@ -44,7 +44,7 @@
             const bool fits = fr_wave_fits(av, T, fp, it, Class::wuIn, Class::capW);
             if (!fits) {
 #ifdef MAPLE_SPR_PROFILE
-                profCls += 2;
+                profCls += 3;
 #endif
                 if (lane == 0) fr_upd_item_lane_call(c, av, T, P, fp, budget, laneBase + blockIdx.x, i, &bU);
                 wave_sync();
diff --git a/maple_amd/csrc/frontier.h b/maple_amd/csrc/frontier.h
--- a/maple_amd/csrc/frontier.h
+++ b/maple_amd/csrc/frontier.h
@@ -26,4 +26,4 @@
 __attribute__((visibility("hidden"))) int frontier_export(maple_ctx *c, long long cap, int32_t *q, int32_t *node, long long *n);
 __attribute__((visibility("hidden")))
 int frontier_level_profile(maple_ctx *c, int cap, long long *itemsU, long long *itemsC, float *msU, float *msC, int *n,
-                           long long *waveSmall = nullptr, long long *waveBig = nullptr);
+                           long long *waveSmall = nullptr, long long *waveBig = nullptr, long long *waveMid = nullptr);
diff --git a/maple_amd/csrc/frontier.hip b/maple_amd/csrc/frontier.hip
--- a/maple_amd/csrc/frontier.hip
+++ b/maple_amd/csrc/frontier.hip
@@ -111,7 +111,7 @@
     }
 }
 
-#define FR_LVL 8
+#define FR_LVL 9
 __global__ void k_fr_snap_u(FCtr *ctr, long long capU, long long capR, long long capPassR, unsigned long long *lvl, int maxLevels)
 {
     if (threadIdx.x == 0 && blockIdx.x == 0) {
@@ -120,12 +120,14 @@
         __threadfence();
         atomicExch(&ctr->safeR, min(ctr->usedR, (unsigned long long)capR));
         ctr->bigUsed = 0;
-        const unsigned long long heavySmall = ctr->permHeavy, heavyBig = ctr->permHeavy2;
-        ctr->permDown = ctr->permUp = ctr->permDownB = ctr->permUpB = ctr->permHeavy = ctr->permHeavy2 = 0;
+        const unsigned long long heavySmall = ctr->permHeavy, heavyBig = ctr->permHeavy2, heavyMid = ctr->permHeavyM;
+        ctr->permDown = ctr->permUp = ctr->permDownB = ctr->permUpB = ctr->permHeavy = ctr->permHeavy2 = ctr->permHeavyM = 0;
         if (lvl) {
             const int l = ctr->nLevels++;
-            if (l < maxLevels) { lvl[FR_LVL * l] = ctr->loU; lvl[FR_LVL * l + 1] = ctr->hiU; lvl[FR_LVL * l + 6] = lvl[FR_LVL * l + 7] = 0; }
-            if (l > 0 && l - 1 < maxLevels) { lvl[FR_LVL * (l - 1) + 6] = heavySmall; lvl[FR_LVL * (l - 1) + 7] = heavyBig; }
+            if (l < maxLevels) { lvl[FR_LVL * l] = ctr->loU; lvl[FR_LVL * l + 1] = ctr->hiU; lvl[FR_LVL * l + 6] = lvl[FR_LVL * l + 7] = lvl[FR_LVL * l + 8] = 0; }
+            if (l > 0 && l - 1 < maxLevels) {
+                lvl[FR_LVL * (l - 1) + 6] = heavySmall; lvl[FR_LVL * (l - 1) + 7] = heavyBig; lvl[FR_LVL * (l - 1) + 8] = heavyMid;
+            }
         }
     }
 }
@@ -206,6 +208,9 @@
     }
 }
 
+#ifndef FR_WAVE_MID
+#define FR_WAVE_MID 1
+#endif
 __global__ __launch_bounds__(FR_BLOCK) void k_fr_sort_level(ArenaViewS av, DevTree T, FPools fp, int heavyMin, int bigMin)
 {
     const long long lo = (long long)fp.ctr->loU, hi = (long long)fp.ctr->hiU;
@@ -218,27 +223,29 @@
     for (long long base = (long long)blockIdx.x * blockDim.x; base < n; base += (long long)gridDim.x * blockDim.x) {
         const long long i = base + threadIdx.x;
         int kind = -1;
-        bool small = false;
+        int cls = -1;
         if (i < n) {
             const FItem &it = fp.U[lo + i];
             const int sz = fr_upd_size(av, T, fp, it);
             if (!(heavyMin > 0 && it.dir != 3 && sz >= heavyMin)) kind = (it.dir == 0 ? 0 : 1) + (sz >= bigMin ? 2 : 0);
             else {
-                small = fr_wave_fits(av, T, fp, it, WaveSmall::wuIn, WaveSmall::capW);
-                if (!small && !fr_wave_fits(av, T, fp, it, WaveBig::wuIn, WaveBig::capW)) kind = (it.dir == 0 ? 2 : 3);
+                if (fr_wave_fits(av, T, fp, it, WaveSmall::wuIn, WaveSmall::capW)) cls = 0;
+                else if (FR_WAVE_MID && fr_wave_fits(av, T, fp, it, WaveMid::wuIn, WaveMid::capW)) cls = 1;
+                else if (fr_wave_fits(av, T, fp, it, WaveBig::wuIn, WaveBig::capW)) cls = 2;
+                else kind = (it.dir == 0 ? 2 : 3);
             }
         }
         const unsigned long long below = (1ull << lane) - 1ull;
         {
             const bool hv = i < n && kind == -1;
-            for (int cls = 0; cls < 2; cls++) {
-                const bool mine = hv && (small == (cls == 0));
+            for (int k = 0; k < 3; k++) {
+                const bool mine = hv && cls == k;
                 const unsigned long long mh = __ballot(mine);
                 if (!mh) continue;
                 unsigned long long b0 = 0;
-                if (lane == 0) b0 = atomicAdd(cls == 0 ? &fp.ctr->permHeavy : &fp.ctr->permHeavy2, (unsigned long long)__popcll(mh));
+                if (lane == 0) b0 = atomicAdd(k == 0 ? &fp.ctr->permHeavy : (k == 1 ? &fp.ctr->permHeavyM : &fp.ctr->permHeavy2), (unsigned long long)__popcll(mh));
                 b0 = bc(b0);
-                if (mine) (cls == 0 ? fp.perm3 : fp.perm4)[(long long)(b0 + __popcll(mh & below))] = (int32_t)i;
+                if (mine) (k == 0 ? fp.perm3 : (k == 1 ? fp.perm5 : fp.perm4))[(long long)(b0 + __popcll(mh & below))] = (int32_t)i;
             }
         }
         for (int k = 0; k < 4; k++) {
@@ -961,12 +968,13 @@
     DevBuf<LRec> trec, arec;
     DevBuf<int32_t> nodes, expQ, expNode;
     DevBuf<uint8_t> out, wideBr, tflag, overHint;
-    DevBuf<int32_t> wideRow, wideQ, wideCtr, perm, perm2, perm3, perm4, tot, lsize, lpos, lpar, passList, passListR, deferred;
+    DevBuf<int32_t> wideRow, wideQ, wideCtr, perm, perm2, perm3, perm4, perm5, tot, lsize, lpos, lpar, passList, passListR, deferred;
     DevBuf<uint2> bw2; DevBuf<double> ba2;
     DevBuf<uint8_t> visit;
     DevBuf<unsigned long long> lvl;
     DevBuf<long long> vbase;
     std::vector<unsigned long long> lastLvl;
+    int lastHeavyMin = 0, lastBigMin = 0;
     std::vector<size_t> lastSlotsU, lastSlotsC;
     long long lastU = -1, lastC = -1, lastR = 0;
     plan::FrontierNeeds need;
@@ -977,7 +985,7 @@
         plan::FrontierCaps k;
         k.itemsU = itemsU.cap; k.itemsC = itemsC.cap; k.tw = tw.cap; k.ta = ta.cap; k.trec = trec.cap; k.tflag = tflag.cap; k.arec = arec.cap;
         k.sw = sw.cap; k.sa = sa.cap; k.sais = sais.cap; k.bw = bw.cap; k.bw2 = bw2.cap; k.recs = recs.cap;
-        k.perm = perm.cap; k.perm2 = perm2.cap; k.perm3 = perm3.cap; k.perm4 = perm4.cap; k.visit = visit.cap; k.lsize = lsize.cap;
+        k.perm = perm.cap; k.perm2 = perm2.cap; k.perm3 = perm3.cap; k.perm4 = perm4.cap; k.perm5 = perm5.cap; k.visit = visit.cap; k.lsize = lsize.cap;
         k.lpos = lpos.cap; k.lpar = lpar.cap; k.passList = passList.cap; k.passListR = passListR.cap;
         return k;
     }
@@ -1052,7 +1060,8 @@
     HIPCK(c, F.perm2.reserve_exact(bd.resPerm2));
     HIPCK(c, F.perm3.reserve_exact(bd.resPerm3));
     HIPCK(c, F.perm4.reserve_exact(bd.resPerm4));
-    fp.perm = F.perm.p; fp.perm2 = F.perm2.p; fp.perm3 = F.perm3.p; fp.perm4 = F.perm4.p;
+    HIPCK(c, F.perm5.reserve_exact(bd.resPerm5));
+    fp.perm = F.perm.p; fp.perm2 = F.perm2.p; fp.perm3 = F.perm3.p; fp.perm4 = F.perm4.p; fp.perm5 = F.perm5.p;
     fp.waveAllBelow = pl.waveAllBelow;
     fp.maxLevels = 4096;
     fp.capVisit = bd.capVisit;
@@ -1168,8 +1177,9 @@
         TRY(fr_launch_updating(c, s, pl.gridUpd, av, T, P, fp, budget, pl.heavyMin));
         TRY(stage("k_fr_updating"));
         if (pl.heavyMin > 0) {
-            TRY(fr_launch_updating_wave_small(c, s, pl.gridWaveSmall, av, T, P, fp, budget, pl.heavyMin, pl.scratchLanes + 256));
-            TRY(fr_launch_updating_wave(c, s, pl.gridWave, av, T, P, fp, budget, pl.heavyMin, pl.scratchLanes));
+            TRY(fr_launch_updating_wave_small(c, s, pl.gridWaveSmall, av, T, P, fp, budget, pl.heavyMin, pl.scratchLanes + pl.slabWaveSmall));
+            TRY(fr_launch_updating_wave_mid(c, s, pl.gridWaveMid, av, T, P, fp, budget, pl.heavyMin, pl.scratchLanes + pl.slabWaveMid));
+            TRY(fr_launch_updating_wave(c, s, pl.gridWave, av, T, P, fp, budget, pl.heavyMin, pl.scratchLanes + pl.slabWave));
         }
         TRY(stage("k_fr_updating_wave"));
         HIPCK(c, hipEventRecord(a1, s));
@@ -1192,7 +1202,7 @@
             HIPCK(c, hipEventRecord(F.evFork2, s2));
             HIPCK(c, hipStreamWaitEvent(s3, F.evFork2, 0));
             DISPATCH3(c, k_fr_pass_wave, <<<1024, FR_BLOCK, 0, s3>>>(c->d_model, av, T, fp));
-            DISPATCH3(c, k_fr_pass, <<<256, FR_BLOCK, 0, s3>>>(c->d_model, av, T, fpC, pl.scratchLanes + 2048));
+            DISPATCH3(c, k_fr_pass, <<<256, FR_BLOCK, 0, s3>>>(c->d_model, av, T, fpC, pl.scratchLanes + pl.slabPass));
             HIPCK(c, hipEventRecord(F.evJoin2, s3));
             passQueued = true;
             TRY(stage("k_fr_pass"));
@@ -1329,8 +1339,9 @@
                 hc.dbgC[0], (double)hc.dbgC[5] / hc.dbgC[0], hc.dbgC[1] * 1e-2 / hc.dbgC[0], hc.dbgC[2] * 1e-2 / hc.dbgC[0],
                 (double)hc.dbgC[6] / std::max(1.0, (double)hc.dbgC[5]), (double)hc.dbgC[4] / hc.dbgC[0], hc.dbgC[3] * 1e-2 / hc.dbgC[0]);
     {
-        const char *nm[4] = {"small class", "512 class", "small class, one lane (a list does not fit)", "512 class, one lane (a list does not fit)"};
-        for (int b = 0; b < 4; b++)
+        const char *nm[6] = {"small class", "512 class", "256 class", "small class, one lane (a list does not fit)",
+                             "512 class, one lane (a list does not fit)", "256 class, one lane (a list does not fit)"};
+        for (int b = 0; b < 6; b++)
             if (hc.dbgWCnt[b]) fprintf(stderr, "[maple] wavefront-wide updating items, %s: %llu items, mean %.3f ms, slowest %.3f ms\n", nm[b],
                                        hc.dbgWCnt[b], hc.dbgWT[b] * 1e-5 / hc.dbgWCnt[b], hc.dbgWMax[b] * 1e-5);
     }
@@ -1353,10 +1364,11 @@
         if (nl) HIPCK(c, hipMemcpy(F.lastLvl.data(), fp.lvl, (size_t)nl * FR_LVL * sizeof(unsigned long long), hipMemcpyDeviceToHost));
         for (int l = 0; l < nl; l++) {
             unsigned long long *L = F.lastLvl.data() + (size_t)FR_LVL * l;
-            if (l >= levels) L[0] = L[1] = L[6] = L[7] = 0;
+            if (l >= levels) L[0] = L[1] = L[6] = L[7] = L[8] = 0;
             if (l >= launchesC) L[2] = L[3] = L[4] = L[5] = 0;
         }
         F.lastSlotsU = slotsU; F.lastSlotsC = slotsC;
+        F.lastHeavyMin = pl.heavyMin; F.lastBigMin = pl.bigMin;
     }
     if (hc.overflow) F.lastU = F.lastC = -1;
     if (stats) {
@@ -1387,7 +1399,7 @@
 }
 
 int frontier_level_profile(maple_ctx *c, int cap, long long *itemsU, long long *itemsC, float *msU, float *msC, int *n, long long *waveSmall,
-                           long long *waveBig)
+                           long long *waveBig, long long *waveMid)
 {
     FrontierScratch *F = static_cast<FrontierScratch *>(c->frontier.get());
     if (!F) return fail(c, MAPLE_ERR_STATE, "no frontier search to report on");
@@ -1399,6 +1411,7 @@
         itemsC[l] = (long long)(L[3] - L[2]) + (long long)(L[5] - L[4]);
         if (waveSmall) waveSmall[l] = (long long)L[6];
         if (waveBig) waveBig[l] = (long long)L[7];
+        if (waveMid) waveMid[l] = (long long)L[8];
         msU[l] = msC[l] = 0.f;
         const size_t su = l < (int)F->lastSlotsU.size() ? F->lastSlotsU[l] : (size_t)-1 / 4, sc = l < (int)F->lastSlotsC.size() ? F->lastSlotsC[l] : (size_t)-1 / 4;
         if (2 * su + 1 < c->ev_used) { HIPCK(c, hipEventSynchronize(c->evs[2 * su + 1])); HIPCK(c, hipEventElapsedTime(&msU[l], c->evs[2 * su], c->evs[2 * su + 1])); }
@@ -1406,3 +1419,21 @@
     }
     return MAPLE_OK;
 }
+
+int frontier_last_levels(maple_ctx *c, FPools *fp, int *heavyMin, int *bigMin, std::vector<unsigned long long> *ranges)
+{
+    FrontierScratch *F = static_cast<FrontierScratch *>(c->frontier.get());
+    if (!F || F->lastLvl.empty()) return fail(c, MAPLE_ERR_STATE, "no frontier search to report on");
+    *fp = F->lastPools; *heavyMin = F->lastHeavyMin; *bigMin = F->lastBigMin;
+    ranges->clear();
+    for (size_t l = 0; l < F->lastLvl.size() / FR_LVL && F->lastLvl[FR_LVL * l + 1] > F->lastLvl[FR_LVL * l]; l++) {
+        ranges->push_back(F->lastLvl[FR_LVL * l]); ranges->push_back(F->lastLvl[FR_LVL * l + 1]);
+    }
+    return MAPLE_OK;
+}
+int frontier_sort_level_again(maple_ctx *c, const FPools &fp, int heavyMin, int bigMin)
+{
+    k_fr_sort_level<<<512, FR_BLOCK, 0, c->stream>>>(view(c), c->dtree, fp, heavyMin, bigMin);
+    HIPCK(c, hipGetLastError());
+    return MAPLE_OK;
+}
diff --git a/maple_amd/csrc/frontier_dev.h b/maple_amd/csrc/frontier_dev.h
--- a/maple_amd/csrc/frontier_dev.h
+++ b/maple_amd/csrc/frontier_dev.h
@@ -95,6 +95,7 @@
     alignas(128) unsigned long long permUpB;
     alignas(128) unsigned long long permHeavy;
     alignas(128) unsigned long long permHeavy2;
+    alignas(128) unsigned long long permHeavyM;
     alignas(128) unsigned long long nLists;
     alignas(128) unsigned long long usedW;
     alignas(128) unsigned long long usedA;
@@ -111,7 +112,7 @@
 #ifdef MAPLE_SPR_PROFILE
     unsigned long long dbgCnt[8], dbgT[8], dbgMax[8];
     unsigned long long dbgC[8];
-    unsigned long long dbgWCnt[4], dbgWT[4], dbgWMax[4];
+    unsigned long long dbgWCnt[6], dbgWT[6], dbgWMax[6];
 #endif
 };
 
@@ -130,7 +131,7 @@
     int32_t maxLevels;
     int32_t *tot; long long *vbase;
     int32_t *perm, *perm2;
-    int32_t *perm3, *perm4;
+    int32_t *perm3, *perm4, *perm5;
     int32_t waveAllBelow;
     uint2 *sw; double *sa; double *sais;
     int32_t capE;
@@ -485,6 +486,11 @@
     static constexpr int32_t *FPools::*perm = &FPools::perm3;
     static constexpr unsigned long long FCtr::*count = &FCtr::permHeavy;
 };
+struct WaveMid {
+    static constexpr int wuIn = 256, capW = 512, profCls = 2;
+    static constexpr int32_t *FPools::*perm = &FPools::perm5;
+    static constexpr unsigned long long FCtr::*count = &FCtr::permHeavyM;
+};
 struct WaveBig {
     static constexpr int wuIn = 512, capW = 512, profCls = 1;
     static constexpr int32_t *FPools::*perm = &FPools::perm4;
@@ -498,6 +504,10 @@
 }
 
 }
+
+__attribute__((visibility("hidden")))
+int frontier_last_levels(maple_ctx *c, frt::FPools *fp, int *heavyMin, int *bigMin, std::vector<unsigned long long> *ranges);
+__attribute__((visibility("hidden"))) int frontier_sort_level_again(maple_ctx *c, const frt::FPools &fp, int heavyMin, int bigMin);
 
 __attribute__((visibility("hidden")))
 int fr_launch_updating(maple_ctx *c, hipStream_t s, int grid, const ArenaViewS &av, const DevTree &T, const SearchParams &P, const frt::FPools &fp,
@@ -506,5 +516,8 @@
 int fr_launch_updating_wave(maple_ctx *c, hipStream_t s, int grid, const ArenaViewS &av, const DevTree &T, const SearchParams &P,
                             const frt::FPools &fp, int budget, int heavyMin, long long laneBase);
 __attribute__((visibility("hidden")))
+int fr_launch_updating_wave_mid(maple_ctx *c, hipStream_t s, int grid, const ArenaViewS &av, const DevTree &T, const SearchParams &P,
+                                const frt::FPools &fp, int budget, int heavyMin, long long laneBase);
+__attribute__((visibility("hidden")))
 int fr_launch_updating_wave_small(maple_ctx *c, hipStream_t s, int grid, const ArenaViewS &av, const DevTree &T, const SearchParams &P,
                                   const frt::FPools &fp, int budget, int heavyMin, long long laneBase);
diff --git a/maple_amd/csrc/frontier_upd_wave.h b/maple_amd/csrc/frontier_upd_wave.h
--- a/maple_amd/csrc/frontier_upd_wave.h
+++ b/maple_amd/csrc/frontier_upd_wave.h
@@ -32,6 +32,10 @@
     return (int)id;
 }
 
-static_assert(sizeof(WaveUpdLds<WaveSmall::wuIn>) == 27680 && sizeof(WaveUpdLds<WaveBig::wuIn>) == 110720 && sizeof(Lds) == 160, "LDS per wavefront");
+static_assert(sizeof(WaveUpdLds<WaveSmall::wuIn>) == 27680 && sizeof(WaveUpdLds<WaveMid::wuIn>) == 55360
+              && sizeof(WaveUpdLds<WaveBig::wuIn>) == 110720 && sizeof(Lds) == 160, "LDS per wavefront");
+static_assert(5 * (27680 + 160) <= 160 * 1024 && 2 * (55360 + 160) <= 160 * 1024 && 3 * (55360 + 160) > 160 * 1024, "wavefronts per compute unit");
+static_assert(WaveSmall::wuIn < WaveMid::wuIn && WaveMid::wuIn < WaveBig::wuIn && WaveSmall::capW <= WaveMid::capW && WaveMid::capW <= WaveBig::capW,
+              "k_fr_sort_level tries the classes in this order");
 
 }
diff --git a/maple_amd/csrc/frontier_updw256.hip b/maple_amd/csrc/frontier_updw256.hip
--- /dev/null
+++ b/maple_amd/csrc/frontier_updw256.hip
@@ -0,0 +1,22 @@
+#include "frontier_upd_wave.h"
+
+using namespace frt;
+
+namespace {
+
+template <bool RV, bool U, bool SS>
+__global__ __launch_bounds__(64) void k_fr_updating_wave_m(const DevModel *__restrict__ mp, ArenaViewS av, DevTree T, SearchParams P, FPools fp,
+                                                           int budget, int heavyMin, long long laneBase)
+{
+    using Class = WaveMid;
+#include "fr_wave_items_body.inc"
+}
+}
+
+int fr_launch_updating_wave_mid(maple_ctx *c, hipStream_t s, int grid, const ArenaViewS &av, const DevTree &T, const SearchParams &P,
+                                const FPools &fp, int budget, int heavyMin, long long laneBase)
+{
+    DISPATCH3(c, k_fr_updating_wave_m, <<<grid, 64, 0, s>>>(c->d_model, av, T, P, fp, budget, heavyMin, laneBase));
+    HIPCK(c, hipGetLastError());
+    return MAPLE_OK;
+}
diff --git a/maple_amd/csrc/search_plan.h b/maple_amd/csrc/search_plan.h
--- a/maple_amd/csrc/search_plan.h
+++ b/maple_amd/csrc/search_plan.h
@@ -15,7 +15,7 @@
 
 struct FrontierCaps {
     size_t itemsU = 0, itemsC = 0, tw = 0, ta = 0, trec = 0, tflag = 0, arec = 0, sw = 0, sa = 0, sais = 0, bw = 0, bw2 = 0, recs = 0;
-    size_t perm = 0, perm2 = 0, perm3 = 0, perm4 = 0, visit = 0, lsize = 0, lpos = 0, lpar = 0, passList = 0, passListR = 0;
+    size_t perm = 0, perm2 = 0, perm3 = 0, perm4 = 0, perm5 = 0, visit = 0, lsize = 0, lpos = 0, lpar = 0, passList = 0, passListR = 0;
 };
 
 struct FrontierPlanIn {
@@ -44,7 +44,11 @@
     long long capBig, capBig2, capRecs;
     double room;
     int gridN, gridCached, heavyMin, bigMin, gridWave, gridWaveSmall, groupLevels, gridLayout, waveAllBelow;
-};
+    int gridWaveMid;
+    long long slabWave, slabWaveSmall, slabWaveMid, slabPass;
+};
+
+static inline int wave_grid(int cus, long long ldsPerCu, long long ldsPerWave) { return cus * (int)(ldsPerCu / ldsPerWave); }
 
 static inline size_t grow(size_t want, size_t cap) { return want <= cap ? cap : std::max(want, cap + cap / 2); }
 
@@ -74,7 +78,11 @@
     const int capE = std::max(in.capE, std::max(256, std::min(1024, (6 * (int)meanEnt + 31) / 32 * 32)));
     p.capE = capE;
     long long scratchLanes = m <= 64 ? 16384 : 256ll * 4 * 4 * 64;
-    const long long extraSlabs = 2048 + (in.matTree ? 256ll * in.frBlock : 0);
+    p.gridWave = wave_grid(256, 160 << 10, 110720 + 160); p.gridWaveMid = wave_grid(256, 160 << 10, 55360 + 160);
+    p.gridWaveSmall = wave_grid(256, 160 << 10, 27680 + 160);
+    p.slabWave = 0; p.slabWaveSmall = p.slabWave + p.gridWave; p.slabWaveMid = p.slabWaveSmall + p.gridWaveSmall;
+    p.slabPass = p.slabWaveMid + p.gridWaveMid;
+    const long long extraSlabs = p.slabPass + (in.matTree ? 256ll * in.frBlock : 0);
     while (scratchLanes > 16384 && (double)(scratchLanes + extraSlabs) * capE * 64 > 0.25 * room) scratchLanes /= 2;
     p.scratchLanes = scratchLanes; p.extraSlabs = extraSlabs;
     p.gridUpd = (int)(scratchLanes / in.frBlock);
@@ -122,7 +130,7 @@
     p.resBa2 = (size_t)capBig2 * 5;
     p.gridN = std::max(1, std::min(2048, (m + in.frBlock - 1) / in.frBlock));
     p.gridCached = (int)std::min<long long>(16384, std::max<long long>(512, (long long)m / 12));
-    p.heavyMin = m <= 64 ? 1 : std::max(256, in.heavyMult * (int)meanEnt / 4); p.gridWave = 256; p.gridWaveSmall = 1280;
+    p.heavyMin = m <= 64 ? 1 : std::max(256, in.heavyMult * (int)meanEnt / 4);
     p.bigMin = m <= 64 ? (1 << 30) : in.bigMin;
     p.groupLevels = m <= 64 ? 2 : 8;
     p.gridLayout = (int)std::min<long long>(1024, std::max<long long>(64, (long long)m / 64));
@@ -133,7 +141,7 @@
 struct FrontierBound {
     long long capU, capC, capCC, capW, capA, capL, capBig, capRecs, capVisit;
     bool layoutOK;
-    size_t resPerm, resPerm2, resPerm3, resPerm4, resVisit, resLsize, resLpos, resLpar, resPassList, resPassListR, resDeferred;
+    size_t resPerm, resPerm2, resPerm3, resPerm4, resPerm5, resVisit, resLsize, resLpos, resLpar, resPassList, resPassListR, resDeferred;
 };
 
 static inline FrontierBound bind_frontier(const FrontierPlanIn &in, const FrontierPlan &p, const FrontierCaps &after)
@@ -147,6 +155,7 @@
     b.resPerm2 = std::max(after.perm2, (size_t)b.capU);
     b.resPerm3 = std::max(after.perm3, (size_t)b.capU);
     b.resPerm4 = std::max(after.perm4, (size_t)b.capU);
+    b.resPerm5 = std::max(after.perm5, (size_t)b.capU);
     b.capVisit = b.capU + b.capC;
     b.layoutOK = in.m > 64 && b.capVisit < (1ll << 31) - 64;
     b.resVisit = b.resLsize = b.resLpos = b.resLpar = 0;
diff --git a/maple_amd/runtime.py b/maple_amd/runtime.py
--- a/maple_amd/runtime.py
+++ b/maple_amd/runtime.py
@@ -26,7 +26,7 @@
 
 DEBUG_EXPORTS = ["maple_debug_wave_append_batch", "maple_debug_trace_query", "maple_debug_trace_read", "maple_debug_calib_walk",
                  "maple_debug_calib_write", "maple_debug_gpv_batch", "maple_debug_simplify_batch", "maple_debug_frontier_levels",
-                 "maple_debug_frontier_pass_batch", "maple_debug_live_resources", "maple_debug_score_rows"]
+                 "maple_debug_frontier_wave_classes", "maple_debug_frontier_pass_batch", "maple_debug_live_resources", "maple_debug_score_rows"]
 LIB_PATH_DEBUG = os.path.join(HERE, "libmaple_hip_debug.so")
 
 
@@ -614,13 +614,32 @@
 
     def frontier_levels(self, cap=4096):
         iu, ic = np.zeros(cap, np.int64), np.zeros(cap, np.int64)
-        ws, wb = np.zeros(cap, np.int64), np.zeros(cap, np.int64)
+        ws, wb, wm = np.zeros(cap, np.int64), np.zeros(cap, np.int64), np.zeros(cap, np.int64)
         mu, mc = np.zeros(cap, np.float32), np.zeros(cap, np.float32)
         n = C.c_int32()
-        self._ck(self.lib.maple_debug_frontier_levels(self.h, int(cap), _ptr(iu), _ptr(ic), _ptr(mu), _ptr(mc), C.byref(n), _ptr(ws), _ptr(wb)))
+        self._ck(self.lib.maple_debug_frontier_levels(self.h, int(cap), _ptr(iu), _ptr(ic), _ptr(mu), _ptr(mc), C.byref(n), _ptr(ws), _ptr(wb),
+                                                      _ptr(wm)))
         k = min(cap, n.value)
         self.last_wave_items = (ws[:k], wb[:k])
+        self.last_wave_items_mid = wm[:k]
         return iu[:k], ic[:k], mu[:k], mc[:k]
+
+    def frontier_wave_classes(self, level):
+        n = C.c_int64()
+        cap = 1 << 16
+        while True:
+            need, score = np.zeros(cap, np.int32), np.zeros(cap, np.int32)
+            fits, routed = np.zeros(cap, np.uint8), np.zeros(cap, np.int8)
+            rc = self.lib.maple_debug_frontier_wave_classes(self.h, int(level), C.c_int64(cap), _ptr(need), _ptr(score), _ptr(fits), _ptr(routed),
+                                                            C.byref(n))
+            if rc == MapleError.ERR_ARG and n.value > cap:
+                cap = int(n.value)
+                continue
+            if rc == MapleError.ERR_ARG and n.value == 0:
+                return None
+            self._ck(rc)
+            k = n.value
+            return need[:k], score[:k], fits[:k], routed[:k]
 
     def tree_rebuild_lists(self, root, up, c0, c1, tip, mut, dist, lower, bump_len=0.0):
         n = len(up)
```

After: 41.46 billion. 0.975x the previous value.
